# rug-marl-group2/scopa

Hardware: AMD Instinct MI355X
Metric: MiniScopa infoset-traversals/sec (higher is better)
Workload: dtype f64

## Files before the change

include/scopa.h:

```cpp
#ifndef SCOPA_H
#define SCOPA_H
#include <stddef.h>
#include <stdint.h>

#ifdef __cplusplus
extern "C" {
#endif

#define SCOPA_ABI_VERSION 1

enum {
    SCOPA_OK = 0,
    SCOPA_EINVAL = -1,
    SCOPA_ENODEV = -2,
    SCOPA_EHIP = -3,
    SCOPA_ESTATE = -4,
    SCOPA_ENOMEM = -5,
    SCOPA_ELIMIT = -6,
    SCOPA_ETIMEOUT = -7
};

#define SCOPA_N_CARDS 16
#define SCOPA_N_PLIES 8
#define SCOPA_N_DECISION 1653
#define SCOPA_N_TERMINAL 576
#define SCOPA_N_NODES 2229
#define SCOPA_MAX_ACTIONS 4

#define SCOPA_STEP_CLONED 0x80u
#define SCOPA_STEP_COUNT_MASK 0x7Fu
typedef struct scopa_state {
    uint16_t hand[2];
    uint32_t table;
    uint8_t  nh[2];
    uint8_t  nt;
    uint8_t  step;
    uint8_t  ncap[2];
    uint8_t  scopas[2];
} scopa_state;

typedef struct scopa_ctx scopa_ctx;

int32_t     scopa_abi_version(void);
const char *scopa_strerror(int32_t status);
const char *scopa_last_error(const scopa_ctx *ctx);

int32_t scopa_ctx_create(int32_t device_id, void *hip_stream, scopa_ctx **out);
int32_t scopa_ctx_destroy(scopa_ctx *ctx);
int32_t scopa_ctx_synchronize(scopa_ctx *ctx);

int32_t scopa_deal_py_seed(int64_t seed, uint8_t perm16[16]);
int32_t scopa_state_init(const uint8_t perm16[16], scopa_state *out);
int32_t scopa_state_step(scopa_state *s, int32_t action);
int32_t scopa_state_clone(const scopa_state *s, scopa_state *out);
int32_t scopa_state_is_terminal(const scopa_state *s);
int32_t scopa_state_current_player(const scopa_state *s);
int32_t scopa_state_legal(const scopa_state *s, int32_t player , int32_t out[4], int32_t *n);
int32_t scopa_state_rewards_x2(const scopa_state *s, int32_t r2[2]);
int32_t scopa_state_infoset_key(const scopa_state *s, int32_t player, uint64_t *key);
int32_t scopa_key_to_string(uint64_t key, char *buf, int32_t cap);
int32_t scopa_state_infoset_string(const scopa_state *s, int32_t player, char *buf, int32_t cap);

int32_t scopa_step_batch(scopa_ctx *ctx, scopa_state *d_states, const uint8_t *d_actions, int64_t n);
int32_t scopa_step_batch_host(scopa_ctx *ctx, scopa_state *h_states, const uint8_t *h_actions, int64_t n);

int32_t scopa_set_deal(scopa_ctx *ctx, const uint8_t perm16[16]);
int32_t scopa_tree_counts(scopa_ctx *ctx, int32_t *n_nodes, int32_t *n_decision, int32_t *n_infosets);
int32_t scopa_tree_export(scopa_ctx *ctx, scopa_state *h_states, int32_t *h_infoset, int8_t *h_r2,
                          uint64_t *h_infoset_key, int8_t *h_infoset_nlegal, int8_t *h_infoset_legal);

int32_t scopa_tables_reset(scopa_ctx *ctx);
int32_t scopa_tables_get(scopa_ctx *ctx, double *h_regret, double *h_strategy, double *h_local);
int32_t scopa_tables_set(scopa_ctx *ctx, const double *h_regret, const double *h_strategy, const double *h_local);

int32_t scopa_visited_get(scopa_ctx *ctx, uint32_t *h_seq);

int32_t scopa_cfr_exact_iterate(scopa_ctx *ctx, int32_t n_iters, double *h_root_values);
int32_t scopa_cfr_exact_traverse(scopa_ctx *ctx, int32_t traverser, double *h_value);
int32_t scopa_cfr_exact_mode(scopa_ctx *ctx, int32_t sequential);
int32_t scopa_cfr_exact_last_route(scopa_ctx *ctx, int32_t *route);
int32_t scopa_cfr_exact_traverse_from(scopa_ctx *ctx, int32_t traverser, int32_t depth, const int32_t *path,
                                      double reach_p0, double reach_p1, double *h_value);

int32_t scopa_cfr_sync_iterate(scopa_ctx *ctx, int32_t n_iters);
int32_t scopa_cfr_sync_iterate_weighted(scopa_ctx *ctx, int32_t n_iters, const double *h_w , int32_t alternating);

int32_t scopa_mccfr_replay(scopa_ctx *ctx, int32_t n_iters, const double *h_uniforms, int64_t n_uniforms,
                           int64_t *consumed);

int32_t scopa_mccfr_seed(scopa_ctx *ctx, uint64_t seed);
int32_t scopa_mccfr_iterate(scopa_ctx *ctx, uint32_t batch, uint32_t n_iters);
int32_t scopa_mccfr_traverse(scopa_ctx *ctx, uint32_t iteration, uint32_t b0, uint32_t nb);
int32_t scopa_mccfr_delta_buffer(scopa_ctx *ctx, void **d_delta, size_t *bytes);
int32_t scopa_mccfr_bind_delta(scopa_ctx *ctx, void *d_buf, size_t bytes);
int32_t scopa_mccfr_delta_get(scopa_ctx *ctx, double *h_delta);
int32_t scopa_mccfr_delta_set(scopa_ctx *ctx, const double *h_delta);
int32_t scopa_mccfr_apply(scopa_ctx *ctx);
int32_t scopa_mccfr_iteration_counter(scopa_ctx *ctx, uint32_t *iteration);
int32_t scopa_mccfr_graph_mode(scopa_ctx *ctx, int32_t on);
int32_t scopa_debug_lds_limit(scopa_ctx *ctx, int32_t bytes);

int32_t scopa_sdcfr_frontier_width(int32_t traverser, int32_t ply);
int32_t scopa_sdcfr_features(scopa_ctx *ctx, int32_t ply, int64_t n, const int32_t *d_idx, float *d_feats, float *d_mask);
int32_t scopa_sdcfr_expand(scopa_ctx *ctx, int32_t ply, int32_t traverser, int64_t n, const int32_t *d_idx, const float *d_adv,
                           int32_t *d_child_idx, float *d_pol, const double *d_uniforms, uint32_t iteration, uint32_t b0);
int32_t scopa_sdcfr_terminal_values(scopa_ctx *ctx, int32_t traverser, int64_t n, const int32_t *d_idx, float *d_val);
int32_t scopa_sdcfr_backward(scopa_ctx *ctx, int32_t ply, int32_t traverser, int64_t n, const int32_t *d_idx, const float *d_pol,
                             const float *d_child_val, float *d_val, const float *d_feats, const float *d_mask, float *d_mem_feat,
                             float *d_mem_regret, float *d_mem_mask, int64_t capacity, int64_t write_base);
int32_t scopa_sdcfr_visits(scopa_ctx *ctx, uint64_t *decision_visits);
int32_t scopa_sdcfr_policy_get(scopa_ctx *ctx, float *h_policy, uint64_t *h_thr);
#define SCOPA_SDCFR_IMAGE_FLOATS 13520
int32_t scopa_sdcfr_image_floats(void);
int32_t scopa_sdcfr_pack_weights(scopa_ctx *ctx, int32_t player, const float *d_w1, const float *d_b1, const float *d_w2,
                                 const float *d_b2, const float *d_w3, const float *d_b3, float *d_image);
int32_t scopa_sdcfr_traverse_fused(scopa_ctx *ctx, int32_t traverser, int32_t batch, const float *d_image, float *d_mem_feat,
                                   float *d_mem_regret, float *d_mem_mask, int64_t capacity, int64_t write_base,
                                   float *d_root_values, const double *d_uniforms, uint32_t iteration, uint32_t b0);
int32_t scopa_sdcfr_mode(scopa_ctx *ctx, int32_t forward_per_visit);
int32_t scopa_sdcfr_tuning(scopa_ctx *ctx, int32_t traversals_per_task, int32_t wavefronts_per_task);
int32_t scopa_sdcfr_train_params(void);
int32_t scopa_sdcfr_train_steps(scopa_ctx *ctx, const int64_t *d_rows, int32_t n_rows, int32_t n_steps, const float *d_feat, const float *d_regret, const float *d_mask,
                                int64_t capacity, float *d_w1, float *d_b1, float *d_w2, float *d_b2, float *d_w3, float *d_b3, float *d_state,
                                int32_t first_step, float lr, float *d_loss);
int32_t scopa_sdcfr_train_step(scopa_ctx *ctx, const int64_t *d_rows, int32_t n_rows, const float *d_feat, const float *d_regret, const float *d_mask,
                               int64_t capacity, float *d_w1, float *d_b1, float *d_w2, float *d_b2, float *d_w3, float *d_b3, float *d_state,
                               int32_t step, float lr, float *d_loss);
int32_t scopa_sdcfr_average_policy(scopa_ctx *ctx, int32_t player, int32_t n_snap, const float *d_w1, const float *d_b1, const float *d_w2,
                                   const float *d_b2, const float *d_w3, const float *d_b3, int32_t max_size, const int32_t *d_slots,
                                   const float *d_coef, double *d_policy);
int32_t scopa_features_from_states(scopa_ctx *ctx, const scopa_state *d_states, int64_t n, float *d_feats, float *d_mask);
int32_t scopa_eval_init_states(scopa_ctx *ctx, scopa_state *d_states, int64_t n);
int32_t scopa_eval_step(scopa_ctx *ctx, scopa_state *d_states, int64_t n, const float *d_probs, const int32_t *d_trained_seat,
                        uint32_t stream_id, uint32_t ply_tag);

int32_t scopa_eval_tabular_prepare(scopa_ctx *ctx, const double *d_policy);
int32_t scopa_eval_tabular_step(scopa_ctx *ctx, scopa_state *d_states, int32_t *d_node_idx, int64_t n, int32_t ply,
                                const double *d_policy, const int32_t *d_trained_seat, uint32_t stream_id);
int32_t scopa_eval_tabular_match(scopa_ctx *ctx, int64_t n, int64_t n_seat0, uint32_t stream_id, scopa_state *d_states_out, int32_t *d_node_idx_out,
                                 int64_t h_stats[10]);

int32_t scopa_exploitability(scopa_ctx *ctx, const double *h_policy, double *h_out4, double *h_policy_out);

int32_t scopa_cross_play(scopa_ctx *ctx, int32_t n_pol, const double *d_policies , double *d_out );
int32_t scopa_best_response(scopa_ctx *ctx, int32_t n_pol, const double *d_policies , double *d_br ,
                            double *d_out4 );
int32_t scopa_eval_pair_match(scopa_ctx *ctx, const double *d_policy_a, const double *d_policy_b, int64_t n, int64_t n_seat0, uint32_t stream_id,
                              int32_t *d_node_idx_out, int64_t h_stats[10]);

typedef struct scopa_multi scopa_multi;
int32_t scopa_multi_create(scopa_ctx *ctx, int32_t n_deals, scopa_multi **out);
int32_t scopa_multi_destroy(scopa_multi *m);
int32_t scopa_multi_deal_py_seeds(scopa_multi *m, const int64_t *h_seeds);
int32_t scopa_multi_set_perms(scopa_multi *m, const uint8_t *h_perms );
int32_t scopa_multi_perms_get(scopa_multi *m, uint8_t *h_perms);
int32_t scopa_multi_build(scopa_multi *m, int32_t *h_n_infosets);
int32_t scopa_multi_cfr_exact_iterate(scopa_multi *m, int32_t n_iters);
int32_t scopa_multi_cfr_exact_iterate_lanes(scopa_multi *m, int32_t n_iters);
int32_t scopa_multi_cfr_sync_iterate(scopa_multi *m, int32_t n_iters);
int32_t scopa_multi_cfr_sync_iterate_weighted(scopa_multi *m, int32_t n_iters, const double *h_w, int32_t alternating,
                                              const uint8_t *h_active );
int32_t scopa_multi_mccfr_iterate(scopa_multi *m, uint32_t batch, uint32_t n_iters, uint64_t seed);
int32_t scopa_multi_exploitability(scopa_multi *m, double *h_out4);
int32_t scopa_multi_tables_get(scopa_multi *m, int32_t deal, double *h_regret, double *h_strategy, double *h_local, uint64_t *h_keys);
int32_t scopa_multi_tables_set(scopa_multi *m, int32_t deal, const double *h_regret, const double *h_strategy, const double *h_local);
int32_t scopa_multi_counters(scopa_multi *m, uint64_t *decision_visits, uint64_t *terminal_visits);

typedef struct scopa_chance scopa_chance;
int32_t scopa_chance_create(scopa_multi *m, scopa_chance **out);
int32_t scopa_chance_destroy(scopa_chance *g);
int32_t scopa_chance_counts(scopa_chance *g, int32_t *n_deals, int64_t *n_global, int64_t *n_occurrences);
int32_t scopa_chance_index_get(scopa_chance *g, uint64_t *h_keys , int32_t *h_map );
int32_t scopa_chance_tables_reset(scopa_chance *g);
int32_t scopa_chance_tables_get(scopa_chance *g, double *h_regret, double *h_strategy);
int32_t scopa_chance_tables_set(scopa_chance *g, const double *h_regret, const double *h_strategy);
int32_t scopa_chance_cfr_iterate_weighted(scopa_chance *g, int32_t n_iters, const double *h_w , int32_t alternating);
int32_t scopa_chance_cfr_iterate_sampled(scopa_chance *g, int32_t n_iters, int32_t m, const int32_t *h_deals ,
                                         const double *h_w , int32_t alternating);
int32_t scopa_chance_mccfr_iterate(scopa_chance *g, int32_t n_iters, uint32_t batch, uint64_t seed,
                                   int32_t m, const int32_t *h_deals );
int32_t scopa_chance_mccfr_counters(scopa_chance *g, uint64_t *decision_visits, uint64_t *terminal_visits, uint32_t *iteration);
int32_t scopa_chance_exploitability(scopa_chance *g, const double *h_policy , double *h_out4, double *h_policy_out);
int32_t scopa_chance_policy_for_deal(scopa_chance *g, const double *d_policy_G, int32_t deal, double *d_policy_local );
int32_t scopa_chance_cross_play(scopa_chance *g, int32_t n_pol, const double *d_policies , double *d_per_deal ,
                                double *d_out );
int32_t scopa_chance_best_response(scopa_chance *g, int32_t n_pol, const double *d_policies , double *d_br ,
                                   double *d_out4 );
int32_t scopa_chance_debug_scratch_budget(scopa_chance *g, int64_t bytes);
int32_t scopa_chance_match(scopa_chance *g, const double *d_policy_a, const double *d_policy_b, int64_t n, int64_t n_seat0, uint32_t stream_id,
                           int32_t *d_deal_out , int32_t *d_node_idx_out , int64_t h_stats[10]);
int32_t scopa_chance_sdcfr_traverse(scopa_chance *g, int32_t traverser, int32_t batch, int32_t m, const int32_t *h_deals ,
                                    const float *d_image, float *d_mem_feat, float *d_mem_regret, float *d_mem_mask , int64_t capacity,
                                    int64_t write_base, float *d_root_values , uint32_t iteration, uint32_t b0);
int32_t scopa_chance_sdcfr_visits(scopa_chance *g, uint64_t *decision_visits);
int32_t scopa_chance_sdcfr_average_policy(scopa_chance *g, int32_t player, int32_t n_snap, const float *d_w1, const float *d_b1, const float *d_w2,
                                          const float *d_b2, const float *d_w3, const float *d_b3, int32_t max_size, const int32_t *d_slots,
                                          const float *d_coef, double *d_policy_G );

typedef struct scopa_full_state {
    uint64_t table[2];
    uint64_t cap[2];
    uint32_t hand[2];
    uint32_t game;
    uint8_t  nh[2], nt, deck_pos, round, last_capture , scopas[2];
    uint16_t step;
    uint8_t  terminal;
    int8_t   r2_p0;
    uint8_t  flags;
    uint8_t  pad[7];
} scopa_full_state;
int32_t scopa_full_deal_py_seed(int64_t seed, uint8_t perm40[40]);
int32_t scopa_full_state_init(const uint8_t deck40[40], uint32_t game, scopa_full_state *out);
int32_t scopa_full_state_step(scopa_full_state *s, const uint8_t deck40[40], int32_t action);
int32_t scopa_full_state_legal(const scopa_full_state *s, int32_t player, int32_t out[3], int32_t *n);
int32_t scopa_full_state_infoset_string(const scopa_full_state *s, int32_t player, char *buf, int32_t cap);
int32_t scopa_full_step_batch(scopa_ctx *ctx, scopa_full_state *d_states, const uint8_t *d_actions, const uint8_t *d_decks, int64_t n);
int32_t scopa_full_step_batch_host(scopa_ctx *ctx, scopa_full_state *h_states, const uint8_t *h_actions, const uint8_t *h_decks,
                                   int64_t n_decks, int64_t n);
int32_t scopa_full_random_playouts(scopa_ctx *ctx, const int64_t *h_seeds, int64_t n_games, int8_t *h_r2_p0, int16_t *h_plies);

typedef struct scopa_team_state {
    uint64_t history;
    uint32_t table;
    uint16_t hand[4];
    uint16_t cap[4];
    uint8_t  nh[4];
    uint8_t  scopas[4];
    uint8_t  nt, step, last_capture_team , flags ;
} scopa_team_state;
int32_t scopa_team_state_init(const uint8_t perm16[16], scopa_team_state *out);
int32_t scopa_team_state_step(scopa_team_state *s, int32_t action);
int32_t scopa_team_state_legal(const scopa_team_state *s, int32_t out[4], int32_t *n);
int32_t scopa_team_state_rewards_x2(const scopa_team_state *s, int32_t r2_seat[4]);
int32_t scopa_team_state_infoset_string(const scopa_team_state *s, int32_t team, char *buf, int32_t cap);
int32_t scopa_team_step_batch(scopa_ctx *ctx, scopa_team_state *d_states, const uint8_t *d_actions, int64_t n);
int32_t scopa_team_step_batch_host(scopa_ctx *ctx, scopa_team_state *h_states, const uint8_t *h_actions, int64_t n);
int32_t scopa_team_random_playouts(scopa_ctx *ctx, const int64_t *h_seeds, int64_t n_games, int8_t *h_r2_team0, uint8_t *h_scopas);

#define SCOPA_TEAM_N_CHOICE 321365
#define SCOPA_TEAM_N_LEAVES 331776
#define SCOPA_TEAM_N_INFOSETS 1648469
int32_t scopa_team_set_deal(scopa_ctx *ctx, const uint8_t perm16[16]);
int32_t scopa_team_tree_counts(scopa_ctx *ctx, int32_t *n_choice, int32_t *n_leaves, int32_t *n_infosets);
int32_t scopa_team_tree_leaves(scopa_ctx *ctx, int8_t *h_r2);
int32_t scopa_team_tables_reset(scopa_ctx *ctx);
int32_t scopa_team_tables_get(scopa_ctx *ctx, double *h_regret, double *h_strategy, double *h_local, double *h_leaf_reach_sum);
int32_t scopa_team_tables_set(scopa_ctx *ctx, const double *h_regret, const double *h_strategy, const double *h_local, const double *h_leaf_reach_sum);
int32_t scopa_team_cfr_iterate(scopa_ctx *ctx, int32_t n_iters, const double *h_w , double *h_root_values );
int32_t scopa_team_cfr_traverse(scopa_ctx *ctx, int32_t traverser, double *h_value);
int32_t scopa_team_cfr_launch(scopa_ctx *ctx, int32_t traverser, int32_t part);
int32_t scopa_team_exploitability(scopa_ctx *ctx, const double *d_policy , double *h_out4, double *d_br );
int32_t scopa_team_minimax(scopa_ctx *ctx, double *h_value, double *d_policy_out );
int32_t scopa_team_policy_value(scopa_ctx *ctx, const double *d_policy_a, const double *d_policy_b, double *h_out);
// ... 53 lines not shown
```

scopa_amd/_lib.py:

```python
import ctypes as C
import os

import numpy as np

_HERE = os.path.dirname(os.path.abspath(__file__))
LIB_PATH = os.environ.get("SCOPA_HIP_LIBRARY") or os.path.join(_HERE, "libscopa_hip.so")

SCOPA_OK, SCOPA_EINVAL, SCOPA_ENODEV, SCOPA_EHIP, SCOPA_ESTATE, SCOPA_ENOMEM, SCOPA_ELIMIT, SCOPA_ETIMEOUT = 0, -1, -2, -3, -4, -5, -6, -7
N_NODES, N_DECISION, N_TERMINAL = 2229, 1653, 576
TEAM_N_CHOICE, TEAM_N_LEAVES, TEAM_N_INFOSETS = 321365, 331776, 1648469
TEAM_MCCFR_DRAWS = (49381, 20583)

SYMBOLS = [
    "scopa_abi_version", "scopa_strerror", "scopa_last_error", "scopa_ctx_create", "scopa_ctx_destroy",
    "scopa_ctx_synchronize", "scopa_deal_py_seed", "scopa_state_init", "scopa_state_step", "scopa_state_clone", "scopa_state_is_terminal",
    "scopa_state_current_player", "scopa_state_legal", "scopa_state_rewards_x2", "scopa_state_infoset_key",
    "scopa_key_to_string", "scopa_state_infoset_string", "scopa_step_batch", "scopa_step_batch_host", "scopa_set_deal",
    "scopa_tree_counts", "scopa_tree_export", "scopa_tables_reset", "scopa_tables_get", "scopa_tables_set",
    "scopa_visited_get", "scopa_cfr_exact_iterate", "scopa_cfr_exact_traverse", "scopa_cfr_exact_mode", "scopa_cfr_exact_last_route", "scopa_cfr_exact_traverse_from", "scopa_mccfr_replay", "scopa_mccfr_seed",
    "scopa_mccfr_iterate", "scopa_mccfr_traverse", "scopa_mccfr_delta_buffer", "scopa_mccfr_bind_delta", "scopa_mccfr_delta_get", "scopa_mccfr_delta_set", "scopa_mccfr_apply",
    "scopa_mccfr_iteration_counter", "scopa_mccfr_graph_mode", "scopa_debug_lds_limit", "scopa_sdcfr_frontier_width", "scopa_sdcfr_features", "scopa_sdcfr_expand",
    "scopa_sdcfr_terminal_values", "scopa_sdcfr_backward", "scopa_sdcfr_visits", "scopa_sdcfr_policy_get", "scopa_sdcfr_traverse_fused", "scopa_sdcfr_image_floats", "scopa_sdcfr_pack_weights", "scopa_sdcfr_tuning", "scopa_sdcfr_mode", "scopa_sdcfr_train_params", "scopa_sdcfr_train_step", "scopa_sdcfr_train_steps", "scopa_sdcfr_average_policy", "scopa_features_from_states",
    "scopa_eval_init_states", "scopa_eval_step", "scopa_eval_tabular_step", "scopa_eval_tabular_prepare", "scopa_eval_tabular_match", "scopa_cfr_sync_iterate", "scopa_cfr_sync_iterate_weighted", "scopa_multi_create", "scopa_multi_destroy",
    "scopa_multi_deal_py_seeds", "scopa_multi_set_perms", "scopa_multi_perms_get", "scopa_multi_build", "scopa_multi_cfr_exact_iterate",
    "scopa_multi_cfr_exact_iterate_lanes", "scopa_multi_cfr_sync_iterate", "scopa_multi_cfr_sync_iterate_weighted", "scopa_multi_mccfr_iterate", "scopa_multi_exploitability", "scopa_multi_tables_get", "scopa_multi_tables_set", "scopa_multi_counters",
    "scopa_chance_create", "scopa_chance_destroy", "scopa_chance_counts", "scopa_chance_index_get", "scopa_chance_tables_reset", "scopa_chance_tables_get", "scopa_chance_tables_set",
    "scopa_chance_cfr_iterate_weighted", "scopa_chance_cfr_iterate_sampled", "scopa_chance_mccfr_iterate", "scopa_chance_mccfr_counters", "scopa_chance_exploitability", "scopa_chance_policy_for_deal",
    "scopa_chance_cross_play", "scopa_chance_best_response", "scopa_chance_debug_scratch_budget", "scopa_chance_match",
    "scopa_chance_sdcfr_traverse", "scopa_chance_sdcfr_visits", "scopa_chance_sdcfr_average_policy", "scopa_full_deal_py_seed",
    "scopa_full_state_init", "scopa_full_state_step", "scopa_full_state_legal", "scopa_full_state_infoset_string",
    "scopa_full_step_batch", "scopa_full_step_batch_host", "scopa_full_random_playouts",
    "scopa_team_state_init", "scopa_team_state_step", "scopa_team_state_legal", "scopa_team_state_rewards_x2", "scopa_team_state_infoset_string",
    "scopa_team_step_batch", "scopa_team_step_batch_host", "scopa_team_random_playouts",
    "scopa_team_set_deal", "scopa_team_tree_counts", "scopa_team_tree_leaves", "scopa_team_tables_reset", "scopa_team_tables_get", "scopa_team_tables_set",
    "scopa_team_cfr_iterate", "scopa_team_cfr_traverse", "scopa_team_cfr_launch", "scopa_team_exploitability", "scopa_team_minimax", "scopa_team_policy_value",
    "scopa_team_chance_create", "scopa_team_chance_destroy", "scopa_team_chance_debug_image_budget", "scopa_team_chance_counts", "scopa_team_chance_index_get",
    "scopa_team_chance_tables_reset", "scopa_team_chance_tables_get", "scopa_team_chance_tables_set", "scopa_team_chance_sigma_get", "scopa_team_chance_cfr_iterate", "scopa_team_chance_cfr_launch",
    "scopa_team_chance_exploitability", "scopa_team_chance_policy_for_deal",
    "scopa_team_chance_mccfr_traverse", "scopa_team_chance_mccfr_apply", "scopa_team_chance_mccfr_walk", "scopa_team_chance_mccfr_iterate", "scopa_team_chance_mccfr_counters", "scopa_team_chance_mccfr_delta_get",
    "scopa_team_mccfr_replay", "scopa_team_mccfr_traverse", "scopa_team_mccfr_apply", "scopa_team_mccfr_iterate", "scopa_team_mccfr_counters", "scopa_team_mccfr_delta_get", "scopa_team_mccfr_visits_get",
    "scopa_mccfr_iterate_sharded", "scopa_p2p_create", "scopa_p2p_connect", "scopa_p2p_allreduce_delta", "scopa_p2p_set_form", "scopa_p2p_set_budget", "scopa_p2p_status", "scopa_p2p_destroy", "scopa_exploitability", "scopa_cross_play", "scopa_best_response", "scopa_eval_pair_match", "scopa_counters", "scopa_prof_enable", "scopa_prof_read", "scopa_prof_device", "scopa_prof_phases", "scopa_prof_spread",
]


class ScopaError(RuntimeError):
    def __init__(self, status, where, detail=""):
        self.status = status
        msg = f"{where}: status {status}"
        try:
            msg += f" ({lib().scopa_strerror(status).decode()})"
        except Exception:
            pass
        if detail:
            msg += f": {detail}"
        super().__init__(msg)


class State16(C.Structure):
    _fields_ = [("hand", C.c_uint16 * 2), ("table", C.c_uint32), ("nh", C.c_uint8 * 2), ("nt", C.c_uint8),
                ("step", C.c_uint8), ("ncap", C.c_uint8 * 2), ("scopas", C.c_uint8 * 2)]


STEP_CLONED, STEP_COUNT_MASK = 0x80, 0x7F
STATE_DTYPE = np.dtype([("hand", "<u2", (2,)), ("table", "<u4"), ("nh", "u1", (2,)), ("nt", "u1"), ("step", "u1"),
                        ("ncap", "u1", (2,)), ("scopas", "u1", (2,))])
assert STATE_DTYPE.itemsize == 16 and C.sizeof(State16) == 16

_lib = None


def lib():
    global _lib
    if _lib is not None:
        return _lib
    try:
        import torch
    except ImportError:
        pass
    if not os.path.exists(LIB_PATH):
        raise OSError(f"{LIB_PATH} is missing: build it with `python __graft_entry__.py` or `python scopa_amd/build.py` "
                      "(the MiniScopa solver path has no fallback)")
    L = C.CDLL(LIB_PATH)
    vp, i32, i64, u32, u64 = C.c_void_p, C.c_int32, C.c_int64, C.c_uint32, C.c_uint64
    sig = {
        "scopa_abi_version": (i32, []),
        "scopa_strerror": (C.c_char_p, [i32]),
        "scopa_last_error": (C.c_char_p, [vp]),
        "scopa_ctx_create": (i32, [i32, vp, C.POINTER(vp)]),
        "scopa_ctx_destroy": (i32, [vp]),
        "scopa_ctx_synchronize": (i32, [vp]),
        "scopa_deal_py_seed": (i32, [i64, vp]),
        "scopa_state_init": (i32, [vp, C.POINTER(State16)]),
        "scopa_state_step": (i32, [C.POINTER(State16), i32]),
        "scopa_state_clone": (i32, [C.POINTER(State16), C.POINTER(State16)]),
        "scopa_state_is_terminal": (i32, [C.POINTER(State16)]),
        "scopa_state_current_player": (i32, [C.POINTER(State16)]),
        "scopa_state_legal": (i32, [C.POINTER(State16), i32, C.POINTER(i32 * 4), C.POINTER(i32)]),
        "scopa_state_rewards_x2": (i32, [C.POINTER(State16), C.POINTER(i32 * 2)]),
        "scopa_state_infoset_key": (i32, [C.POINTER(State16), i32, C.POINTER(u64)]),
        "scopa_key_to_string": (i32, [u64, C.c_char_p, i32]),
        "scopa_state_infoset_string": (i32, [C.POINTER(State16), i32, C.c_char_p, i32]),
        "scopa_step_batch": (i32, [vp, vp, vp, i64]),
        "scopa_step_batch_host": (i32, [vp, vp, vp, i64]),
        "scopa_set_deal": (i32, [vp, vp]),
        "scopa_tree_counts": (i32, [vp, C.POINTER(i32), C.POINTER(i32), C.POINTER(i32)]),
        "scopa_tree_export": (i32, [vp, vp, vp, vp, vp, vp, vp]),
        "scopa_tables_reset": (i32, [vp]),
        "scopa_tables_get": (i32, [vp, vp, vp, vp]),
        "scopa_tables_set": (i32, [vp, vp, vp, vp]),
        "scopa_cfr_exact_iterate": (i32, [vp, i32, vp]),
        "scopa_cfr_exact_traverse": (i32, [vp, i32, C.POINTER(C.c_double)]),
        "scopa_cfr_exact_mode": (i32, [vp, i32]),
        "scopa_cfr_exact_last_route": (i32, [vp, C.POINTER(i32)]),
        "scopa_cfr_exact_traverse_from": (i32, [vp, i32, i32, vp, C.c_double, C.c_double, C.POINTER(C.c_double)]),
        "scopa_visited_get": (i32, [vp, vp]),
        "scopa_mccfr_replay": (i32, [vp, i32, vp, i64, C.POINTER(i64)]),
        "scopa_mccfr_seed": (i32, [vp, u64]),
        "scopa_mccfr_iterate": (i32, [vp, u32, u32]),
        "scopa_mccfr_traverse": (i32, [vp, u32, u32, u32]),
        "scopa_mccfr_delta_buffer": (i32, [vp, C.POINTER(vp), C.POINTER(C.c_size_t)]),
        "scopa_mccfr_bind_delta": (i32, [vp, vp, C.c_size_t]),
        "scopa_mccfr_delta_get": (i32, [vp, vp]),
        "scopa_mccfr_delta_set": (i32, [vp, vp]),
        "scopa_mccfr_apply": (i32, [vp]),
        "scopa_mccfr_iteration_counter": (i32, [vp, C.POINTER(u32)]),
        "scopa_mccfr_graph_mode": (i32, [vp, i32]),
        "scopa_debug_lds_limit": (i32, [vp, i32]),
        "scopa_exploitability": (i32, [vp, vp, vp, vp]),
        "scopa_sdcfr_frontier_width": (i32, [i32, i32]),
        "scopa_sdcfr_features": (i32, [vp, i32, i64, vp, vp, vp]),
        "scopa_sdcfr_expand": (i32, [vp, i32, i32, i64, vp, vp, vp, vp, vp, u32, u32]),
        "scopa_sdcfr_terminal_values": (i32, [vp, i32, i64, vp, vp]),
        "scopa_sdcfr_backward": (i32, [vp, i32, i32, i64, vp, vp, vp, vp, vp, vp, vp, vp, vp, i64, i64]),
        "scopa_sdcfr_visits": (i32, [vp, C.POINTER(u64)]),
        "scopa_sdcfr_policy_get": (i32, [vp, vp, vp]),
        "scopa_sdcfr_traverse_fused": (i32, [vp, i32, i32, vp, vp, vp, vp, i64, i64, vp, vp, u32, u32]),
        "scopa_sdcfr_image_floats": (i32, []),
        "scopa_sdcfr_pack_weights": (i32, [vp, i32, vp, vp, vp, vp, vp, vp, vp]),
        "scopa_sdcfr_tuning": (i32, [vp, i32, i32]),
        "scopa_sdcfr_train_params": (i32, []),
        "scopa_sdcfr_train_step": (i32, [vp, vp, i32, vp, vp, vp, i64, vp, vp, vp, vp, vp, vp, vp, i32, C.c_float, vp]),
        "scopa_sdcfr_train_steps": (i32, [vp, vp, i32, i32, vp, vp, vp, i64, vp, vp, vp, vp, vp, vp, vp, i32, C.c_float, vp]),
        "scopa_sdcfr_mode": (i32, [vp, i32]),
        "scopa_sdcfr_average_policy": (i32, [vp, i32, i32, vp, vp, vp, vp, vp, vp, i32, vp, vp, vp]),
        "scopa_features_from_states": (i32, [vp, vp, i64, vp, vp]),
        "scopa_eval_init_states": (i32, [vp, vp, i64]),
        "scopa_eval_step": (i32, [vp, vp, i64, vp, vp, u32, u32]),
        "scopa_eval_tabular_step": (i32, [vp, vp, vp, i64, i32, vp, vp, u32]),
        "scopa_eval_tabular_prepare": (i32, [vp, vp]),
        "scopa_eval_tabular_match": (i32, [vp, i64, i64, u32, vp, vp, vp]),
        "scopa_cross_play": (i32, [vp, i32, vp, vp]),
        "scopa_best_response": (i32, [vp, i32, vp, vp, vp]),
        "scopa_eval_pair_match": (i32, [vp, vp, vp, i64, i64, u32, vp, vp]),
        "scopa_cfr_sync_iterate": (i32, [vp, i32]),
        "scopa_cfr_sync_iterate_weighted": (i32, [vp, i32, vp, i32]),
        "scopa_multi_create": (i32, [vp, i32, C.POINTER(vp)]),
        "scopa_multi_destroy": (i32, [vp]),
        "scopa_multi_deal_py_seeds": (i32, [vp, vp]),
        "scopa_multi_set_perms": (i32, [vp, vp]),
        "scopa_multi_perms_get": (i32, [vp, vp]),
        "scopa_multi_build": (i32, [vp, vp]),
        "scopa_multi_cfr_exact_iterate": (i32, [vp, i32]),
        "scopa_multi_cfr_sync_iterate": (i32, [vp, i32]),
        "scopa_multi_cfr_sync_iterate_weighted": (i32, [vp, i32, vp, i32, vp]),
        "scopa_multi_cfr_exact_iterate_lanes": (i32, [vp, i32]),
        "scopa_multi_exploitability": (i32, [vp, vp]),
        "scopa_multi_mccfr_iterate": (i32, [vp, u32, u32, u64]),
        "scopa_multi_tables_get": (i32, [vp, i32, vp, vp, vp, vp]),
        "scopa_multi_tables_set": (i32, [vp, i32, vp, vp, vp]),
        "scopa_multi_counters": (i32, [vp, C.POINTER(u64), C.POINTER(u64)]),
        "scopa_chance_create": (i32, [vp, C.POINTER(vp)]),
        "scopa_chance_destroy": (i32, [vp]),
        "scopa_chance_counts": (i32, [vp, C.POINTER(i32), C.POINTER(i64), C.POINTER(i64)]),
        "scopa_chance_index_get": (i32, [vp, vp, vp]),
        "scopa_chance_tables_reset": (i32, [vp]),
        "scopa_chance_tables_get": (i32, [vp, vp, vp]),
        "scopa_chance_tables_set": (i32, [vp, vp, vp]),
        "scopa_chance_cfr_iterate_weighted": (i32, [vp, i32, vp, i32]),
        "scopa_chance_cfr_iterate_sampled": (i32, [vp, i32, i32, vp, vp, i32]),
        "scopa_chance_mccfr_iterate": (i32, [vp, i32, u32, u64, i32, vp]),
        "scopa_chance_mccfr_counters": (i32, [vp, C.POINTER(u64), C.POINTER(u64), C.POINTER(u32)]),
        "scopa_chance_exploitability": (i32, [vp, vp, vp, vp]),
        "scopa_chance_policy_for_deal": (i32, [vp, vp, i32, vp]),
        "scopa_chance_cross_play": (i32, [vp, i32, vp, vp, vp]),
        "scopa_chance_best_response": (i32, [vp, i32, vp, vp, vp]),
        "scopa_chance_debug_scratch_budget": (i32, [vp, i64]),
        "scopa_chance_match": (i32, [vp, vp, vp, i64, i64, u32, vp, vp, vp]),
        "scopa_chance_sdcfr_traverse": (i32, [vp, i32, i32, i32, vp, vp, vp, vp, vp, i64, i64, vp, u32, u32]),
        "scopa_chance_sdcfr_visits": (i32, [vp, C.POINTER(u64)]),
        "scopa_chance_sdcfr_average_policy": (i32, [vp, i32, i32, vp, vp, vp, vp, vp, vp, i32, vp, vp, vp]),
        "scopa_full_deal_py_seed": (i32, [i64, vp]),
        "scopa_full_state_init": (i32, [vp, u32, vp]),
        "scopa_full_state_step": (i32, [vp, vp, i32]),
        "scopa_full_state_legal": (i32, [vp, i32, C.POINTER(i32 * 3), C.POINTER(i32)]),
        "scopa_full_state_infoset_string": (i32, [vp, i32, C.c_char_p, i32]),
        "scopa_full_step_batch": (i32, [vp, vp, vp, vp, i64]),
        "scopa_full_step_batch_host": (i32, [vp, vp, vp, vp, i64, i64]),
        "scopa_full_random_playouts": (i32, [vp, vp, i64, vp, vp]),
        "scopa_mccfr_iterate_sharded": (i32, [vp, u32, u32, u32]),
        "scopa_p2p_create": (i32, [vp, i32, i32, vp]),
        "scopa_p2p_connect": (i32, [vp, vp]),
        "scopa_p2p_allreduce_delta": (i32, [vp]),
        "scopa_p2p_set_form": (i32, [vp, i32]),
        "scopa_p2p_set_budget": (i32, [vp, C.c_double]),
        "scopa_p2p_status": (i32, [vp, C.POINTER(i32), C.POINTER(u64)]),
        "scopa_p2p_destroy": (i32, [vp]),
        "scopa_team_state_init": (i32, [vp, vp]),
        "scopa_team_state_step": (i32, [vp, i32]),
        "scopa_team_state_legal": (i32, [vp, C.POINTER(i32 * 4), C.POINTER(i32)]),
        "scopa_team_state_rewards_x2": (i32, [vp, C.POINTER(i32 * 4)]),
        "scopa_team_state_infoset_string": (i32, [vp, i32, C.c_char_p, i32]),
        "scopa_team_step_batch": (i32, [vp, vp, vp, i64]),
        "scopa_team_step_batch_host": (i32, [vp, vp, vp, i64]),
        "scopa_team_random_playouts": (i32, [vp, vp, i64, vp, vp]),
        "scopa_team_set_deal": (i32, [vp, vp]),
        "scopa_team_tree_counts": (i32, [vp, C.POINTER(i32), C.POINTER(i32), C.POINTER(i32)]),
        "scopa_team_tree_leaves": (i32, [vp, vp]),
        "scopa_team_tables_reset": (i32, [vp]),
        "scopa_team_tables_get": (i32, [vp, vp, vp, vp, vp]),
        "scopa_team_tables_set": (i32, [vp, vp, vp, vp, vp]),
        "scopa_team_cfr_iterate": (i32, [vp, i32, vp, vp]),
        "scopa_team_cfr_traverse": (i32, [vp, i32, C.POINTER(C.c_double)]),
        "scopa_team_cfr_launch": (i32, [vp, i32, i32]),
        "scopa_team_exploitability": (i32, [vp, vp, C.POINTER(C.c_double * 4), vp]),
        "scopa_team_minimax": (i32, [vp, C.POINTER(C.c_double), vp]),
        "scopa_team_policy_value": (i32, [vp, vp, vp, C.POINTER(C.c_double)]),
        "scopa_team_chance_create": (i32, [vp, i32, vp, C.POINTER(vp)]),
        "scopa_team_chance_destroy": (i32, [vp]),
        "scopa_team_chance_debug_image_budget": (i32, [vp, i64]),
        "scopa_team_chance_counts": (i32, [vp, C.POINTER(i32), C.POINTER(i64), C.POINTER(i64)]),
        "scopa_team_chance_index_get": (i32, [vp, vp, vp]),
        "scopa_team_chance_tables_reset": (i32, [vp]),
        "scopa_team_chance_tables_get": (i32, [vp, vp, vp]),
        "scopa_team_chance_tables_set": (i32, [vp, vp, vp]),
        "scopa_team_chance_sigma_get": (i32, [vp, vp]),
        "scopa_team_chance_cfr_iterate": (i32, [vp, i32, vp, vp]),
        "scopa_team_chance_cfr_launch": (i32, [vp, i32, i32]),
        "scopa_team_chance_exploitability": (i32, [vp, vp, C.POINTER(C.c_double * 4), vp, vp]),
        "scopa_team_chance_policy_for_deal": (i32, [vp, vp, i32, vp]),
        "scopa_team_chance_mccfr_traverse": (i32, [vp, C.c_uint32, i32, C.c_uint32, C.c_uint32]),
        "scopa_team_chance_mccfr_apply": (i32, [vp]),
        "scopa_team_chance_mccfr_walk": (i32, [vp, C.c_uint32, C.c_uint32, i32, vp]),
        "scopa_team_chance_mccfr_iterate": (i32, [vp, i32, C.c_uint32, i32, vp]),
        "scopa_team_chance_mccfr_counters": (i32, [vp, C.POINTER(C.c_uint64), C.POINTER(C.c_uint64), C.POINTER(C.c_uint32)]),
        "scopa_team_chance_mccfr_delta_get": (i32, [vp, vp]),
        "scopa_team_mccfr_replay": (i32, [vp, i32, vp, i64, C.POINTER(i64)]),
        "scopa_team_mccfr_traverse": (i32, [vp, C.c_uint32, C.c_uint32, C.c_uint32]),
        "scopa_team_mccfr_apply": (i32, [vp]),
        "scopa_team_mccfr_iterate": (i32, [vp, C.c_uint32, C.c_uint32]),
        "scopa_team_mccfr_counters": (i32, [vp, C.POINTER(C.c_uint64), C.POINTER(C.c_uint64), C.POINTER(C.c_uint32)]),
        "scopa_team_mccfr_delta_get": (i32, [vp, vp]),
        "scopa_team_mccfr_visits_get": (i32, [vp, vp, vp]),
        "scopa_counters": (i32, [vp, C.POINTER(u64), C.POINTER(u64)]),
        "scopa_prof_enable": (i32, [vp, i32]),
        "scopa_prof_read": (i32, [vp, C.POINTER(i64), C.POINTER(C.c_double)]),
        "scopa_prof_device": (i32, [vp, C.POINTER(i64), C.POINTER(C.c_double)]),
        "scopa_prof_phases": (i32, [vp, C.POINTER(C.c_double * 3)]),
        "scopa_prof_spread": (i32, [vp, C.POINTER(C.c_double * 3)]),
    }
    lenient = bool(os.environ.get("SCOPA_HIP_LIBRARY")) and os.environ.get("SCOPA_AB_OLD_LIBRARY") == "1"
    for name, (res, args) in sig.items():
        if lenient and not hasattr(L, name):
            continue
        fn = getattr(L, name)
        fn.restype, fn.argtypes = res, args
    if L.scopa_abi_version() != 1:
        raise OSError("libscopa_hip.so ABI version mismatch")
    _lib = L
    return L


def _ptr(a):
    return a.ctypes.data_as(C.c_void_p) if a is not None else None


def _weights(weights):
    w = np.ascontiguousarray(weights, np.float64).reshape(-1, 3)
    return (w if w.size else np.ones((1, 3))), w.shape[0]


# ... 20 lines not shown
        self._L = lib()
        rc = self._L.scopa_ctx_create(int(device), C.c_void_p(stream) if stream else None, C.byref(self._h))
        if rc:
            self._h = None
            raise ScopaError(rc, "scopa_ctx_create", "a GPU is required: the solver path has no CPU fallback")
        self.device = device
        self.stream = stream
        self.n_infosets = 0
        self._children = []

    def close(self):
        if getattr(self, "_h", None):
            for ref in getattr(self, "_children", []):
                child = ref()
                if child is not None:
                    child.close()
            self._L.scopa_ctx_destroy(self._h)
            self._h = None

    def __del__(self):
        try:
            self.close()
        except Exception:
            pass

    def _ck(self, rc, where):
        if rc:
            raise ScopaError(rc, where, self._L.scopa_last_error(self._h).decode())

    def synchronize(self):
        self._ck(self._L.scopa_ctx_synchronize(self._h), "scopa_ctx_synchronize")

    def step_batch_host(self, states, actions):
        assert states.dtype == STATE_DTYPE and states.flags.c_contiguous
        actions = np.ascontiguousarray(actions, np.uint8)
        assert actions.size == states.size
        self._ck(self._L.scopa_step_batch_host(self._h, _ptr(states), _ptr(actions), states.size), "scopa_step_batch_host")
        return states

    def step_batch(self, d_states_ptr, d_actions_ptr, n):
        self._ck(self._L.scopa_step_batch(self._h, C.c_void_p(d_states_ptr), C.c_void_p(d_actions_ptr), int(n)), "scopa_step_batch")

    def set_deal(self, perm16):
        perm = np.ascontiguousarray(perm16, np.uint8)
        assert perm.size == 16
        self._ck(self._L.scopa_set_deal(self._h, _ptr(perm)), "scopa_set_deal")
        a, b, c = C.c_int32(), C.c_int32(), C.c_int32()
        self._ck(self._L.scopa_tree_counts(self._h, C.byref(a), C.byref(b), C.byref(c)), "scopa_tree_counts")
        self.n_infosets = c.value
        self.perm = perm
        return self.n_infosets

    def tree_export(self):
        I = self.n_infosets
        out = dict(states=np.zeros(N_NODES, STATE_DTYPE), infoset=np.zeros(N_NODES, np.int32), r2=np.zeros((N_NODES, 2), np.int8),
                   infoset_key=np.zeros(I, np.uint64), infoset_nlegal=np.zeros(I, np.int8), infoset_legal=np.zeros((I, 4), np.int8))
        self._ck(self._L.scopa_tree_export(self._h, _ptr(out["states"]), _ptr(out["infoset"]), _ptr(out["r2"]),
                                           _ptr(out["infoset_key"]), _ptr(out["infoset_nlegal"]), _ptr(out["infoset_legal"])),
                 "scopa_tree_export")
        return out

    def tables_reset(self):
        self._ck(self._L.scopa_tables_reset(self._h), "scopa_tables_reset")

    def tables_get(self, regret=True, strategy=True, local=True):
        I = self.n_infosets
        R = np.zeros((I, 4)) if regret else None
        S = np.zeros((I, 4)) if strategy else None
        Lc = np.zeros((I, 4)) if local else None
        self._ck(self._L.scopa_tables_get(self._h, _ptr(R), _ptr(S), _ptr(Lc)), "scopa_tables_get")
        return R, S, Lc

    def tables_set(self, regret=None, strategy=None, local=None):
        arrs = []
        for a in (regret, strategy, local):
            if a is not None:
                a = np.ascontiguousarray(a, np.float64)
                assert a.shape == (self.n_infosets, 4)
            arrs.append(a)
        self._ck(self._L.scopa_tables_set(self._h, _ptr(arrs[0]), _ptr(arrs[1]), _ptr(arrs[2])), "scopa_tables_set")

    def cfr_exact_iterate(self, n_iters):
        rv = np.zeros((max(int(n_iters), 0), 2))
        self._ck(self._L.scopa_cfr_exact_iterate(self._h, int(n_iters), _ptr(rv)), "scopa_cfr_exact_iterate")
        return rv

    def cfr_exact_mode(self, sequential):
        self._ck(self._L.scopa_cfr_exact_mode(self._h, 1 if sequential else 0), "scopa_cfr_exact_mode")

    def cfr_exact_last_route(self):
        r = C.c_int32()
        self._ck(self._L.scopa_cfr_exact_last_route(self._h, C.byref(r)), "scopa_cfr_exact_last_route")
        return r.value

    def cfr_exact_traverse(self, traverser):
        v = C.c_double()
        self._ck(self._L.scopa_cfr_exact_traverse(self._h, int(traverser), C.byref(v)), "scopa_cfr_exact_traverse")
        return v.value

    def cfr_exact_traverse_from(self, traverser, path, reach_p0=1.0, reach_p1=1.0):
        pa = np.ascontiguousarray(path, np.int32)
        v = C.c_double()
        self._ck(self._L.scopa_cfr_exact_traverse_from(self._h, int(traverser), pa.size, _ptr(pa), float(reach_p0), float(reach_p1),
                                                       C.byref(v)), "scopa_cfr_exact_traverse_from")
        return v.value

    def visited_get(self):
        seq = np.zeros(self.n_infosets, np.uint32)
        self._ck(self._L.scopa_visited_get(self._h, _ptr(seq)), "scopa_visited_get")
        return seq

    def mccfr_replay(self, n_iters, uniforms):
        u = np.ascontiguousarray(uniforms, np.float64)
        used = C.c_int64()
        self._ck(self._L.scopa_mccfr_replay(self._h, int(n_iters), _ptr(u), u.size, C.byref(used)), "scopa_mccfr_replay")
        return used.value

    def mccfr_seed(self, seed):
        self._ck(self._L.scopa_mccfr_seed(self._h, int(seed)), "scopa_mccfr_seed")

    def mccfr_iterate(self, batch, n_iters):
        self._ck(self._L.scopa_mccfr_iterate(self._h, int(batch), int(n_iters)), "scopa_mccfr_iterate")

    def mccfr_traverse(self, iteration, b0, nb):
        self._ck(self._L.scopa_mccfr_traverse(self._h, int(iteration), int(b0), int(nb)), "scopa_mccfr_traverse")

    def mccfr_delta_buffer(self):
        p, n = C.c_void_p(), C.c_size_t()
        self._ck(self._L.scopa_mccfr_delta_buffer(self._h, C.byref(p), C.byref(n)), "scopa_mccfr_delta_buffer")
        return p.value, n.value

    def mccfr_bind_delta(self, d_ptr, nbytes):
        self._ck(self._L.scopa_mccfr_bind_delta(self._h, C.c_void_p(d_ptr) if d_ptr else None, int(nbytes)), "scopa_mccfr_bind_delta")

    def mccfr_delta_get(self):
        d = np.zeros((self.n_infosets, 5))
        self._ck(self._L.scopa_mccfr_delta_get(self._h, _ptr(d)), "scopa_mccfr_delta_get")
        return d

    def mccfr_delta_set(self, d):
        d = np.ascontiguousarray(d, np.float64)
        assert d.shape == (self.n_infosets, 5)
        self._ck(self._L.scopa_mccfr_delta_set(self._h, _ptr(d)), "scopa_mccfr_delta_set")

    def mccfr_apply(self):
        self._ck(self._L.scopa_mccfr_apply(self._h), "scopa_mccfr_apply")

    def mccfr_graph_mode(self, on):
        self._ck(self._L.scopa_mccfr_graph_mode(self._h, 1 if on else 0), "scopa_mccfr_graph_mode")

    def debug_lds_limit(self, nbytes):
        self._ck(self._L.scopa_debug_lds_limit(self._h, int(nbytes)), "scopa_debug_lds_limit")

    def mccfr_iteration(self):
        v = C.c_uint32()
        self._ck(self._L.scopa_mccfr_iteration_counter(self._h, C.byref(v)), "scopa_mccfr_iteration_counter")
        return v.value

    def exploitability(self, policy=None, return_policy=False):
        pin = None if policy is None else np.ascontiguousarray(policy, np.float64)
        out = np.zeros(4)
        pout = np.zeros((self.n_infosets, 4)) if return_policy else None
        self._ck(self._L.scopa_exploitability(self._h, _ptr(pin), _ptr(out), _ptr(pout)), "scopa_exploitability")
        res = dict(exploitability=out[0], br0=out[1], br1=out[2], value_p0=out[3])
        if return_policy:
            res["policy"] = pout
        return res

    def sdcfr_features(self, ply, n, idx_ptr, feats_ptr, mask_ptr):
        self._ck(self._L.scopa_sdcfr_features(self._h, ply, n, C.c_void_p(idx_ptr), C.c_void_p(feats_ptr), C.c_void_p(mask_ptr)), "scopa_sdcfr_features")

    def sdcfr_expand(self, ply, traverser, n, idx_ptr, adv_ptr, child_ptr, pol_ptr, uniforms_ptr, iteration, b0):
        self._ck(self._L.scopa_sdcfr_expand(self._h, ply, traverser, n, C.c_void_p(idx_ptr), C.c_void_p(adv_ptr), C.c_void_p(child_ptr),
                                            C.c_void_p(pol_ptr), C.c_void_p(uniforms_ptr) if uniforms_ptr else None, iteration, b0), "scopa_sdcfr_expand")

    def sdcfr_terminal_values(self, traverser, n, idx_ptr, val_ptr):
        self._ck(self._L.scopa_sdcfr_terminal_values(self._h, traverser, n, C.c_void_p(idx_ptr), C.c_void_p(val_ptr)), "scopa_sdcfr_terminal_values")

    def sdcfr_backward(self, ply, traverser, n, idx_ptr, pol_ptr, child_val_ptr, val_ptr, feats_ptr, mask_ptr, mem_feat_ptr, mem_regret_ptr,
                       mem_mask_ptr, capacity, write_base):
        vp = lambda x: C.c_void_p(x) if x else None
        self._ck(self._L.scopa_sdcfr_backward(self._h, ply, traverser, n, vp(idx_ptr), vp(pol_ptr), vp(child_val_ptr), vp(val_ptr), vp(feats_ptr),
                                              vp(mask_ptr), vp(mem_feat_ptr), vp(mem_regret_ptr), vp(mem_mask_ptr), capacity, write_base),
                 "scopa_sdcfr_backward")

    def sdcfr_pack_weights(self, player, w1_ptr, b1_ptr, w2_ptr, b2_ptr, w3_ptr, b3_ptr, image_ptr):
        self._ck(self._L.scopa_sdcfr_pack_weights(self._h, player, *(C.c_void_p(x) for x in (w1_ptr, b1_ptr, w2_ptr, b2_ptr, w3_ptr, b3_ptr, image_ptr))),
                 "scopa_sdcfr_pack_weights")

    def sdcfr_mode(self, forward_per_visit):
        self._ck(self._L.scopa_sdcfr_mode(self._h, 1 if forward_per_visit else 0), "scopa_sdcfr_mode")

    def sdcfr_tuning(self, traversals_per_task=0, wavefronts_per_task=0):
        self._ck(self._L.scopa_sdcfr_tuning(self._h, traversals_per_task, wavefronts_per_task), "scopa_sdcfr_tuning")

    def sdcfr_train_steps(self, rows_ptr, n_rows, n_steps, feat_ptr, regret_ptr, mask_ptr, capacity, param_ptrs, state_ptr, first_step, lr, loss_ptr):
        self._ck(self._L.scopa_sdcfr_train_steps(self._h, C.c_void_p(rows_ptr), int(n_rows), int(n_steps), C.c_void_p(feat_ptr), C.c_void_p(regret_ptr), C.c_void_p(mask_ptr),
                                                 int(capacity), *(C.c_void_p(p) for p in param_ptrs), C.c_void_p(state_ptr), int(first_step), float(lr),
                                                 C.c_void_p(loss_ptr)), "scopa_sdcfr_train_steps")

    def sdcfr_train_step(self, rows_ptr, n_rows, feat_ptr, regret_ptr, mask_ptr, capacity, param_ptrs, state_ptr, step, lr, loss_ptr):
        self._ck(self._L.scopa_sdcfr_train_step(self._h, C.c_void_p(rows_ptr), int(n_rows), C.c_void_p(feat_ptr), C.c_void_p(regret_ptr), C.c_void_p(mask_ptr),
                                                int(capacity), *(C.c_void_p(p) for p in param_ptrs), C.c_void_p(state_ptr), int(step), float(lr),
                                                C.c_void_p(loss_ptr)), "scopa_sdcfr_train_step")

    def sdcfr_traverse_fused(self, traverser, batch, weights_ptr, mem_feat_ptr, mem_regret_ptr, mem_mask_ptr, capacity, write_base,
                             root_values_ptr, uniforms_ptr, iteration, b0):
        self._ck(self._L.scopa_sdcfr_traverse_fused(self._h, traverser, batch, C.c_void_p(weights_ptr), C.c_void_p(mem_feat_ptr),
                                                    C.c_void_p(mem_regret_ptr), C.c_void_p(mem_mask_ptr), capacity, write_base,
                                                    C.c_void_p(root_values_ptr), C.c_void_p(uniforms_ptr) if uniforms_ptr else None,
                                                    iteration, b0), "scopa_sdcfr_traverse_fused")

    def sdcfr_average_policy(self, player, n_snap, param_ptrs, max_size, slots_ptr, coef_ptr, policy_ptr):
        vp = lambda x: C.c_void_p(x) if x else None
        self._ck(self._L.scopa_sdcfr_average_policy(self._h, int(player), int(n_snap), *(vp(p) for p in param_ptrs), int(max_size), vp(slots_ptr),
                                                    vp(coef_ptr), vp(policy_ptr)), "scopa_sdcfr_average_policy")

    def sdcfr_visits(self):
        v = C.c_uint64()
        self._ck(self._L.scopa_sdcfr_visits(self._h, C.byref(v)), "scopa_sdcfr_visits")
        return v.value

    def sdcfr_policy_get(self):
        pol, thr = np.zeros((N_DECISION, 4), np.float32), np.zeros((N_DECISION, 3), np.uint64)
        self._ck(self._L.scopa_sdcfr_policy_get(self._h, _ptr(pol), _ptr(thr)), "scopa_sdcfr_policy_get")
        return pol, thr

    def features_from_states(self, states_ptr, n, feats_ptr, mask_ptr):
        self._ck(self._L.scopa_features_from_states(self._h, C.c_void_p(states_ptr), n, C.c_void_p(feats_ptr), C.c_void_p(mask_ptr)), "scopa_features_from_states")

    def eval_init_states(self, states_ptr, n):
        self._ck(self._L.scopa_eval_init_states(self._h, C.c_void_p(states_ptr), n), "scopa_eval_init_states")

    def eval_step(self, states_ptr, n, probs_ptr, seat_ptr, stream_id, ply_tag):
        self._ck(self._L.scopa_eval_step(self._h, C.c_void_p(states_ptr), n, C.c_void_p(probs_ptr) if probs_ptr else None, C.c_void_p(seat_ptr),
                                         stream_id, ply_tag), "scopa_eval_step")

    def eval_tabular_prepare(self, policy_ptr):
        self._ck(self._L.scopa_eval_tabular_prepare(self._h, C.c_void_p(policy_ptr)), "scopa_eval_tabular_prepare")

    def eval_tabular_step(self, states_ptr, idx_ptr, n, ply, policy_ptr, seat_ptr, stream_id):
        self._ck(self._L.scopa_eval_tabular_step(self._h, C.c_void_p(states_ptr), C.c_void_p(idx_ptr), n, ply, C.c_void_p(policy_ptr) if policy_ptr else None,
                                                 C.c_void_p(seat_ptr), stream_id), "scopa_eval_tabular_step")

    def eval_tabular_match(self, n, n_seat0, stream_id, states_ptr=0, idx_ptr=0):
        st = np.zeros((2, 5), np.int64)
        self._ck(self._L.scopa_eval_tabular_match(self._h, int(n), int(n_seat0), stream_id, C.c_void_p(states_ptr) if states_ptr else None,
                                                  C.c_void_p(idx_ptr) if idx_ptr else None, _ptr(st)), "scopa_eval_tabular_match")
        return st

    def cross_play(self, n_pol, policies_ptr, out_ptr):
        self._ck(self._L.scopa_cross_play(self._h, int(n_pol), C.c_void_p(policies_ptr) if policies_ptr else None, C.c_void_p(out_ptr) if out_ptr else None),
                 "scopa_cross_play")

    def best_response(self, n_pol, policies_ptr, br_ptr, out4_ptr):
        self._ck(self._L.scopa_best_response(self._h, int(n_pol), C.c_void_p(policies_ptr) if policies_ptr else None, C.c_void_p(br_ptr) if br_ptr else None,
                                             C.c_void_p(out4_ptr) if out4_ptr else None), "scopa_best_response")

    def eval_pair_match(self, policy_a_ptr, policy_b_ptr, n, n_seat0, stream_id, idx_ptr=0):
        st = np.zeros((2, 5), np.int64)
        self._ck(self._L.scopa_eval_pair_match(self._h, C.c_void_p(policy_a_ptr) if policy_a_ptr else None, C.c_void_p(policy_b_ptr) if policy_b_ptr else None,
                                               int(n), int(n_seat0), stream_id, C.c_void_p(idx_ptr) if idx_ptr else None, _ptr(st)), "scopa_eval_pair_match")
        return st

    def cfr_sync_iterate(self, n_iters):
        self._ck(self._L.scopa_cfr_sync_iterate(self._h, int(n_iters)), "scopa_cfr_sync_iterate")

    def cfr_sync_iterate_weighted(self, weights, alternating=False):
        w, n = _weights(weights)
        self._ck(self._L.scopa_cfr_sync_iterate_weighted(self._h, n, _ptr(w), int(alternating)), "scopa_cfr_sync_iterate_weighted")

    def full_step_batch_host(self, states, actions, decks):
        assert states.dtype == FULL_STATE_DTYPE
        actions = np.ascontiguousarray(actions, np.uint8)
        decks = np.ascontiguousarray(decks, np.uint8).reshape(-1, 40)
        self._ck(self._L.scopa_full_step_batch_host(self._h, _ptr(states), _ptr(actions), _ptr(decks), decks.shape[0], states.size),
                 "scopa_full_step_batch_host")
        return states

    def full_step_batch(self, states_ptr, actions_ptr, decks_ptr, n):
        self._ck(self._L.scopa_full_step_batch(self._h, C.c_void_p(states_ptr), C.c_void_p(actions_ptr), C.c_void_p(decks_ptr), int(n)), "scopa_full_step_batch")

    def full_random_playouts(self, seeds):
        seeds = np.ascontiguousarray(seeds, np.int64)
        r2, plies = np.zeros(seeds.size, np.int8), np.zeros(seeds.size, np.int16)
        self._ck(self._L.scopa_full_random_playouts(self._h, _ptr(seeds), seeds.size, _ptr(r2), _ptr(plies)), "scopa_full_random_playouts")
        return r2, plies

    def p2p_create(self, rank, world):
        h = np.zeros(64, np.uint8)
        self._ck(self._L.scopa_p2p_create(self._h, int(rank), int(world), _ptr(h)), "scopa_p2p_create")
        return h

    def p2p_connect(self, handles):
        handles = np.ascontiguousarray(handles, np.uint8).reshape(-1, 64)
        self._ck(self._L.scopa_p2p_connect(self._h, _ptr(handles)), "scopa_p2p_connect")

    def p2p_allreduce_delta(self):
        self._ck(self._L.scopa_p2p_allreduce_delta(self._h), "scopa_p2p_allreduce_delta")

    def mccfr_iterate_sharded(self, b0, nb, n_iters=1):
        self._ck(self._L.scopa_mccfr_iterate_sharded(self._h, int(b0), int(nb), int(n_iters)), "scopa_mccfr_iterate_sharded")

    def p2p_status(self):
        t, n = C.c_int32(), C.c_uint64()
        self._ck(self._L.scopa_p2p_status(self._h, C.byref(t), C.byref(n)), "scopa_p2p_status")
# ... 664 lines not shown
```

scopa_amd/csrc/scopa_ctx.h:

```cpp
#pragma once
#include <hip/hip_runtime.h>
#include <stdint.h>
#include <stdio.h>

#include <vector>

#include "../../include/scopa.h"
#include "scopa_rules.h"

struct scopa_p2p;
struct scopa_team_solver;

struct scopa_ctx {
    int device = -1;
    hipStream_t stream = nullptr;
    bool own_stream = false;
    char err[512] = {0};

    bool has_deal = false;
    uint8_t perm[16] = {0};
    int n_infosets = 0;

    scopa_state *d_states = nullptr;
    uint16_t *d_infoset = nullptr;
    int8_t *d_payoff = nullptr;
    uint64_t *d_key = nullptr;
    int32_t *d_meta = nullptr;
    uint32_t *d_visit = nullptr;

    double *d_regret = nullptr, *d_strat = nullptr, *d_local = nullptr;
    double *d_delta = nullptr;
    double *d_delta_own = nullptr;
    double *d_scratch = nullptr;
    double *d_sigcdf = nullptr;
    bool sigcdf_valid = false;
    bool mccfr_all_seen = false;
    uint32_t mccfr_seen_wait = 0;
    double *d_groups = nullptr;
    unsigned long long *d_clock = nullptr;
    uint16_t clock_grid[2048] = {0};
    double prof_phase_us[3] = {0.0, 0.0, 0.0};
    double prof_spread_us[3] = {0.0, 0.0, 0.0};
    size_t scratch_bytes = 0;

    unsigned long long *d_counters = nullptr;

    uint64_t seed = 0x5C09A;
    uint64_t sdcfr_visits = 0;
    void *d_sdnode = nullptr;
    bool sdnode_valid = false;
    void *d_eval_thr = nullptr;
    bool eval_thr_valid = false;
    void *d_pair_thr = nullptr;
    void *d_train_partial = nullptr;
    void *d_sdpol = nullptr;
    bool sdpol_valid = false;
    void *d_sdavg = nullptr;
    size_t sdavg_bytes = 0;
    int sdcfr_mode = 0;
    uint32_t iteration = 0;

    bool prof_on = false;
    int prof_stride = 1;
    long long prof_tick = 0;
    std::vector<hipEvent_t> ev_pool;
    size_t ev_used = 0;
    int64_t prof_launches = 0;
    double prof_ms = 0.0;

    uint32_t *d_lane_tab = nullptr;
    uint16_t *d_sched = nullptr;
    int sched_steps = 0;
    bool sched_valid = false;
    int exact_last_route = -1;
    bool exact_sequential = false;

    scopa_p2p *p2p = nullptr;
    scopa_team_solver *team = nullptr;

    struct GraphEntry { uint32_t batch, k, track; void *exec; };
    std::vector<GraphEntry> mccfr_graphs;
    bool mccfr_graph_mode = false;

    int lds_limit = 160 * 1024;
    int n_cus = 256;
    uint32_t lds_attr_done = 0;
    long long team_chance_budget = 0;
};

namespace scopa {

#ifndef SCOPA_GROUPS
#define SCOPA_GROUPS 16
#endif
#ifndef SCOPA_GROUP_PERM
#define SCOPA_GROUP_PERM 0
#endif
constexpr int kDeltaGroups = SCOPA_GROUPS;
constexpr int kGroupRows = 1664;
constexpr size_t kDeltaTable = (size_t)kGroupRows * 5;
__host__ __device__ inline size_t group_cell(int k, int r) {
#if SCOPA_GROUP_PERM == 1
    return (size_t)k * kGroupRows + (size_t)((r & 63) * 26 + (r >> 6));
#elif SCOPA_GROUP_PERM == 2
    return (size_t)k * kGroupRows + (size_t)((r & 7) * 208 + (r >> 3));
#else
    return (size_t)k * kGroupRows + (size_t)r;
#endif
}
constexpr int kClockSamples = 2048, kClockStride = 2048;

inline int32_t fail(scopa_ctx *ctx, int32_t code, const char *what, hipError_t e = hipSuccess) {
    if (ctx) {
        if (e != hipSuccess) snprintf(ctx->err, sizeof ctx->err, "%s: %s", what, hipGetErrorString(e));
        else snprintf(ctx->err, sizeof ctx->err, "%s", what);
    }
    return code;
}

#define SC_HIP(ctx, call)                                                         \
    do {                                                                          \
        hipError_t e__ = (call);                                                  \
        if (e__ != hipSuccess) return scopa::fail((ctx), SCOPA_EHIP, #call, e__); \
    } while (0)

#define SC_REQUIRE(ctx, cond, code, msg)                        \
    do {                                                        \
        if (!(cond)) return scopa::fail((ctx), (code), (msg)); \
    } while (0)

int32_t ensure_scratch(scopa_ctx *ctx, size_t bytes);

void range_push(const char *name);
void range_pop();
struct Range { explicit Range(const char *n) { range_push(n); } ~Range() { range_pop(); } };

enum LdsAttrKernel : uint32_t { kLdsTraverse = 1u, kLdsReplay = 8u, kLdsCfrExact = 16u, kLdsCfrSched = 512u, kLdsExploit = 32u, kLdsCfrSync = 64u, kLdsSdcfr = 128u, kLdsMulti = 256u, kLdsSdcfrReplay = 1024u, kLdsSdPolicy = 2048u, kLdsSdWalk0 = 4096u, kLdsSdWalk1 = 8192u, kLdsCfrSyncW = 16384u, kLdsCrossPlay = 32768u, kLdsBestResponse = 65536u, kLdsMccfrChance = 131072u, kLdsChanceSdWalk0 = 262144u, kLdsChanceSdWalk1 = 524288u, kLdsChanceCrossPlay = 1048576u, kLdsTeamCfr = 2097152u, kLdsTeamChance = 4194304u };
inline bool cfr_weights_ok(const double *h_w, int32_t n_iters) {
    for (size_t k = 0; k < (size_t)n_iters * 3; k++) if (!(h_w[k] >= 0.0 && h_w[k] <= 1.0)) return false;
    return true;
}
inline int32_t ensure_lds_attr(scopa_ctx *ctx, uint32_t kernel_bit, const void *fn, int bytes) {
    if (ctx->lds_attr_done & kernel_bit) return SCOPA_OK;
    SC_HIP(ctx, hipFuncSetAttribute(fn, hipFuncAttributeMaxDynamicSharedMemorySize, bytes));
    ctx->lds_attr_done |= kernel_bit;
    return SCOPA_OK;
}
#define SC_LDS_ATTR(ctx, bit, kernel, bytes)                                                                     \
    do {                                                                                                         \
        const int32_t rc__ = scopa::ensure_lds_attr((ctx), (bit), reinterpret_cast<const void *>(kernel), (bytes)); \
        if (rc__ != SCOPA_OK) return rc__;                                                                       \
    } while (0)
bool prof_events(scopa_ctx *ctx, hipEvent_t *start, hipEvent_t *stop);
void p2p_release(scopa_ctx *ctx);
void team_release(scopa_ctx *ctx);
void mccfr_graphs_clear(scopa_ctx *ctx);

}
```

scopa_amd/csrc/scopa_host.hip:

```cpp
#include <string.h>

#include <new>

#include "scopa_ctx.h"

using namespace scopa;

namespace scopa {

int32_t ensure_scratch(scopa_ctx *ctx, size_t bytes) {
    if (bytes <= ctx->scratch_bytes) return SCOPA_OK;
    if (ctx->d_scratch) SC_HIP(ctx, hipFree(ctx->d_scratch));
    ctx->d_scratch = nullptr;
    ctx->scratch_bytes = 0;
    SC_HIP(ctx, hipMalloc(&ctx->d_scratch, bytes));
    ctx->scratch_bytes = bytes;
    return SCOPA_OK;
}

static void prof_pool_fill(scopa_ctx *ctx) {
    while (ctx->ev_pool.size() < 4096) {
        hipEvent_t e;
        if (hipEventCreate(&e) != hipSuccess) break;
        ctx->ev_pool.push_back(e);
    }
}

bool prof_events(scopa_ctx *ctx, hipEvent_t *start, hipEvent_t *stop) {
    if (!ctx->prof_on) return false;
    if ((ctx->prof_tick++ % ctx->prof_stride) != 0) return false;
    if (ctx->ev_used + 2 > ctx->ev_pool.size()) {
        if (ctx->ev_used) {
            (void)hipEventSynchronize(ctx->ev_pool[ctx->ev_used - 1]);
            for (size_t i = 0; i + 1 < ctx->ev_used; i += 2) {
                float ms = 0.f;
                if (hipEventElapsedTime(&ms, ctx->ev_pool[i], ctx->ev_pool[i + 1]) == hipSuccess) ctx->prof_ms += ms;
            }
            ctx->ev_used = 0;
        }
        if (ctx->ev_pool.empty()) prof_pool_fill(ctx);
    }
    if (ctx->ev_used + 2 > ctx->ev_pool.size()) return false;
    *start = ctx->ev_pool[ctx->ev_used];
    *stop = ctx->ev_pool[ctx->ev_used + 1];
    ctx->ev_used += 2;
    ctx->prof_launches++;
    return true;
}

}

#include <dlfcn.h>
namespace scopa {
namespace {
int (*g_roctx_push)(const char *) = nullptr;
int (*g_roctx_pop)() = nullptr;
int g_roctx_state = 0;
void roctx_resolve() {
    g_roctx_state = -1;
    const char *on = getenv("SCOPA_ROCTX");
    if (!on || on[0] != '1') return;
    for (const char *lib : {"librocprofiler-sdk-roctx.so", "libroctx64.so"}) {
        void *h = dlopen(lib, RTLD_NOW | RTLD_GLOBAL);
        if (!h) continue;
        g_roctx_push = reinterpret_cast<int (*)(const char *)>(dlsym(h, "roctxRangePushA"));
        g_roctx_pop = reinterpret_cast<int (*)()>(dlsym(h, "roctxRangePop"));
        if (g_roctx_push && g_roctx_pop) { g_roctx_state = 1; return; }
    }
}
}
void range_push(const char *name) {
    if (g_roctx_state == 0) roctx_resolve();
    if (g_roctx_state == 1) (void)g_roctx_push(name);
}
void range_pop() {
    if (g_roctx_state == 1) (void)g_roctx_pop();
}
}

extern "C" {

int32_t scopa_abi_version(void) { return SCOPA_ABI_VERSION; }

const char *scopa_strerror(int32_t status) {
    switch (status) {
        case SCOPA_OK: return "ok";
        case SCOPA_EINVAL: return "invalid argument";
        case SCOPA_ENODEV: return "no usable HIP device (the solver path has no CPU fallback)";
        case SCOPA_EHIP: return "HIP runtime error";
        case SCOPA_ESTATE: return "call order violated";
        case SCOPA_ENOMEM: return "out of memory";
        case SCOPA_ELIMIT: return "problem exceeds a compiled-in capacity";
        case SCOPA_ETIMEOUT: return "a peer did not answer within the wait budget";
        default: return "unknown status";
    }
}

const char *scopa_last_error(const scopa_ctx *ctx) { return ctx ? ctx->err : "null context"; }

int32_t scopa_ctx_create(int32_t device_id, void *hip_stream, scopa_ctx **out) {
    if (!out || device_id < 0) return SCOPA_EINVAL;
    *out = nullptr;
    int count = 0;
    if (hipGetDeviceCount(&count) != hipSuccess || count <= 0) return SCOPA_ENODEV;
    if (device_id >= count) return SCOPA_ENODEV;
    scopa_ctx *ctx = new (std::nothrow) scopa_ctx();
    if (!ctx) return SCOPA_ENOMEM;
    ctx->device = device_id;
    hipError_t e = hipSetDevice(device_id);
    if (e != hipSuccess) { delete ctx; return SCOPA_ENODEV; }
    hipDeviceProp_t prop;
    if (hipGetDeviceProperties(&prop, device_id) == hipSuccess) {
        ctx->n_cus = prop.multiProcessorCount;
        ctx->lds_limit = (int)prop.sharedMemPerBlock;
    }
    if (hip_stream) ctx->stream = (hipStream_t)hip_stream;
    else {
        e = hipStreamCreateWithFlags(&ctx->stream, hipStreamNonBlocking);
        if (e != hipSuccess) { delete ctx; return SCOPA_EHIP; }
        ctx->own_stream = true;
    }
    const size_t rows = (size_t)kDecision;
    bool ok = hipMalloc(&ctx->d_states, sizeof(scopa_state) * kNodes) == hipSuccess &&
              hipMalloc(&ctx->d_infoset, sizeof(uint16_t) * kDecision) == hipSuccess &&
              hipMalloc(&ctx->d_payoff, kTerminal) == hipSuccess &&
              hipMalloc(&ctx->d_key, sizeof(uint64_t) * kDecision) == hipSuccess &&
              hipMalloc(&ctx->d_meta, sizeof(int32_t) * 8) == hipSuccess &&
              hipMalloc(&ctx->d_visit, sizeof(uint32_t) * kDecision) == hipSuccess &&
              hipMalloc(&ctx->d_sigcdf, (size_t)kDecision * 6 * sizeof(double)) == hipSuccess &&
              hipMalloc(&ctx->d_groups, scopa::kDeltaGroups * scopa::kDeltaTable * sizeof(double)) == hipSuccess &&
              hipMalloc(&ctx->d_regret, rows * 4 * sizeof(double)) == hipSuccess &&
              hipMalloc(&ctx->d_strat, rows * 4 * sizeof(double)) == hipSuccess &&
              hipMalloc(&ctx->d_local, rows * 4 * sizeof(double)) == hipSuccess &&
              hipMalloc(&ctx->d_delta_own, rows * 5 * sizeof(double)) == hipSuccess &&
              hipMalloc(&ctx->d_counters, (8 + 2 * 1024) * sizeof(unsigned long long)) == hipSuccess;
    ctx->d_delta = ctx->d_delta_own;
    if (ok) ok = hipMemsetAsync(ctx->d_counters, 0, (8 + 2 * 1024) * sizeof(unsigned long long), ctx->stream) == hipSuccess &&
                 hipMemsetAsync(ctx->d_delta, 0, rows * 5 * sizeof(double), ctx->stream) == hipSuccess &&
                 hipMemsetAsync(ctx->d_groups, 0, scopa::kDeltaGroups * scopa::kDeltaTable * sizeof(double), ctx->stream) == hipSuccess;
    if (!ok) { scopa_ctx_destroy(ctx); return SCOPA_ENOMEM; }
    *out = ctx;
    return SCOPA_OK;
}

int32_t scopa_ctx_destroy(scopa_ctx *ctx) {
    if (!ctx) return SCOPA_EINVAL;
    (void)hipSetDevice(ctx->device);
    (void)hipStreamSynchronize(ctx->stream);
    scopa::p2p_release(ctx);
    scopa::team_release(ctx);
    scopa::mccfr_graphs_clear(ctx);
    for (hipEvent_t e : ctx->ev_pool) (void)hipEventDestroy(e);
    void *bufs[] = {ctx->d_states, ctx->d_infoset, ctx->d_payoff, ctx->d_key, ctx->d_meta, ctx->d_regret, ctx->d_strat,
                    ctx->d_local, ctx->d_delta_own, ctx->d_scratch, ctx->d_counters, ctx->d_visit, ctx->d_sigcdf, ctx->d_groups, ctx->d_clock, ctx->d_sched, ctx->d_lane_tab, ctx->d_sdnode, ctx->d_sdpol, ctx->d_train_partial, ctx->d_eval_thr, ctx->d_pair_thr, ctx->d_sdavg};
    for (void *b : bufs) if (b) (void)hipFree(b);
    if (ctx->own_stream) (void)hipStreamDestroy(ctx->stream);
    delete ctx;
    return SCOPA_OK;
}

int32_t scopa_debug_lds_limit(scopa_ctx *ctx, int32_t bytes) {
    if (!ctx || bytes < 0) return SCOPA_EINVAL;
    hipDeviceProp_t prop;
    SC_HIP(ctx, hipGetDeviceProperties(&prop, ctx->device));
    SC_REQUIRE(ctx, bytes == 0 || (bytes >= 64 * 1024 && (size_t)bytes <= prop.sharedMemPerBlock), SCOPA_EINVAL, "scopa_debug_lds_limit: 0 or 64 KB .. the device's limit");
    ctx->lds_limit = bytes ? bytes : (int)prop.sharedMemPerBlock;
    ctx->lds_attr_done = 0;
    scopa::mccfr_graphs_clear(ctx);
    return SCOPA_OK;
}

int32_t scopa_ctx_synchronize(scopa_ctx *ctx) {
    if (!ctx) return SCOPA_EINVAL;
    SC_HIP(ctx, hipStreamSynchronize(ctx->stream));
    return SCOPA_OK;
}

namespace {
struct Mt19937 {
    uint32_t mt[624];
    int at = 624;
    void seed_u32(uint32_t s) {
        mt[0] = s;
        for (int i = 1; i < 624; i++) mt[i] = 1812433253u * (mt[i - 1] ^ (mt[i - 1] >> 30)) + (uint32_t)i;
        at = 624;
    }
    void seed_array(const uint32_t *key, int n) {
        seed_u32(19650218u);
        int i = 1, j = 0;
        for (int k = n > 624 ? n : 624; k > 0; k--) {
            mt[i] = (mt[i] ^ ((mt[i - 1] ^ (mt[i - 1] >> 30)) * 1664525u)) + key[j] + (uint32_t)j;
            if (++i >= 624) { mt[0] = mt[623]; i = 1; }
            if (++j >= n) j = 0;
        }
        for (int k = 623; k > 0; k--) {
            mt[i] = (mt[i] ^ ((mt[i - 1] ^ (mt[i - 1] >> 30)) * 1566083941u)) - (uint32_t)i;
            if (++i >= 624) { mt[0] = mt[623]; i = 1; }
        }
        mt[0] = 0x80000000u;
    }
    void refill() {
        for (int k = 0; k < 624; k++) {
            const uint32_t y = (mt[k] & 0x80000000u) | (mt[(k + 1) % 624] & 0x7fffffffu);
            mt[k] = mt[(k + 397) % 624] ^ (y >> 1) ^ ((y & 1u) ? 0x9908b0dfu : 0u);
        }
        at = 0;
    }
    uint32_t next() {
        if (at >= 624) refill();
        uint32_t y = mt[at++];
        y ^= y >> 11;
        y ^= (y << 7) & 0x9d2c5680u;
        y ^= (y << 15) & 0xefc60000u;
        y ^= y >> 18;
        return y;
    }
    uint32_t below(uint32_t n) {
        int bits = 32 - __builtin_clz(n);
        uint32_t r;
        do r = next() >> (32 - bits); while (r >= n);
        return r;
    }
};
}

int32_t scopa_deal_py_seed(int64_t seed, uint8_t perm16[16]) {
    if (!perm16) return SCOPA_EINVAL;
    const uint64_t a = seed < 0 ? (uint64_t)0 - (uint64_t)seed : (uint64_t)seed;
    const uint32_t key[2] = {(uint32_t)a, (uint32_t)(a >> 32)};
    Mt19937 g;
    g.seed_array(key, key[1] ? 2 : 1);
    for (int i = 0; i < 16; i++) perm16[i] = (uint8_t)i;
    for (uint32_t i = 15; i >= 1; i--) {
        const uint32_t j = g.below(i + 1);
        const uint8_t t = perm16[i]; perm16[i] = perm16[j]; perm16[j] = t;
    }
    return SCOPA_OK;
}

static bool perm_ok(const uint8_t *p) {
    uint32_t seen = 0;
    for (int i = 0; i < 16; i++) { if (p[i] > 15) return false; seen |= 1u << p[i]; }
    return seen == 0xFFFFu;
}

int32_t scopa_state_init(const uint8_t perm16[16], scopa_state *out) {
    if (!perm16 || !out || !perm_ok(perm16)) return SCOPA_EINVAL;
    state_init(*out, perm16);
    return SCOPA_OK;
}

int32_t scopa_state_step(scopa_state *s, int32_t action) {
    if (!s || action < 0 || action > 15) return SCOPA_EINVAL;
    step(*s, action);
    return SCOPA_OK;
}

int32_t scopa_state_clone(const scopa_state *s, scopa_state *out) {
    if (!s || !out) return SCOPA_EINVAL;
    scopa_state c = *s;
    if (!is_terminal(c)) c.step = (uint8_t)(c.step | SCOPA_STEP_CLONED);
    *out = c;
    return SCOPA_OK;
}

int32_t scopa_state_is_terminal(const scopa_state *s) { return s ? (is_terminal(*s) ? 1 : 0) : SCOPA_EINVAL; }

int32_t scopa_state_current_player(const scopa_state *s) { return s ? current_player(*s) : SCOPA_EINVAL; }

int32_t scopa_state_legal(const scopa_state *s, int32_t player, int32_t out[4], int32_t *n) {
    if (!s || !out || !n || player > 1) return SCOPA_EINVAL;
    int tmp[4];
    *n = legal(*s, player, tmp);
    for (int i = 0; i < *n; i++) out[i] = tmp[i];
    return SCOPA_OK;
}

int32_t scopa_state_rewards_x2(const scopa_state *s, int32_t r2[2]) {
    if (!s || !r2) return SCOPA_EINVAL;
    int a, b;
    rewards_x2(*s, a, b);
    r2[0] = a; r2[1] = b;
    return SCOPA_OK;
}

int32_t scopa_state_infoset_key(const scopa_state *s, int32_t player, uint64_t *key) {
    if (!s || !key || player > 1) return SCOPA_EINVAL;
    if (player < 0) player = s->step & 1;
    *key = infoset_key(*s, player);
    return SCOPA_OK;
}

int32_t scopa_key_to_string(uint64_t key, char *buf, int32_t cap) {
    if (!buf || cap < 64) return SCOPA_EINVAL;
    static const char suit[4] = {'c', 'f', 'p', 'b'};
    const int player = (int)(key & 1), nh = (int)((key >> 1) & 7), nt = (int)((key >> 20) & 15);
    const uint32_t hand = (uint32_t)((key >> 4) & 0xFFFF), table = (uint32_t)(key >> 24);
    char *w = buf;
    w += sprintf(w, "P%d:H[", player);
    for (int i = 0; i < nh; i++) w += sprintf(w, "%s%d%c", i ? "-" : "", card_rank(nib(hand, i)), suit[nib(hand, i) >> 2]);
    w += sprintf(w, "]_T[");
    for (int i = 0; i < nt; i++) w += sprintf(w, "%s%d%c", i ? "-" : "", card_rank(nib(table, i)), suit[nib(table, i) >> 2]);
    w += sprintf(w, "]");
    return (int32_t)(w - buf);
}

int32_t scopa_state_infoset_string(const scopa_state *s, int32_t player, char *buf, int32_t cap) {
    if (!s || !buf || cap < 64 || player > 1) return SCOPA_EINVAL;
    if (player < 0) player = current_player(*s);
    if (is_terminal(*s) || player < 0) return (int32_t)sprintf(buf, "TERMINAL");
    return scopa_key_to_string(infoset_key(*s, player), buf, cap);
}

int32_t scopa_tables_get(scopa_ctx *ctx, double *h_regret, double *h_strategy, double *h_local) {
    if (!ctx) return SCOPA_EINVAL;
    SC_REQUIRE(ctx, ctx->has_deal, SCOPA_ESTATE, "scopa_tables_get: no deal set");
    const size_t bytes = (size_t)ctx->n_infosets * 4 * sizeof(double);
    if (h_regret) SC_HIP(ctx, hipMemcpyAsync(h_regret, ctx->d_regret, bytes, hipMemcpyDeviceToHost, ctx->stream));
    if (h_strategy) SC_HIP(ctx, hipMemcpyAsync(h_strategy, ctx->d_strat, bytes, hipMemcpyDeviceToHost, ctx->stream));
    if (h_local) SC_HIP(ctx, hipMemcpyAsync(h_local, ctx->d_local, bytes, hipMemcpyDeviceToHost, ctx->stream));
    SC_HIP(ctx, hipStreamSynchronize(ctx->stream));
// ... 140 lines not shown
```

scopa_amd/csrc/scopa_mccfr.hip:

```cpp
#include <hip/hip_ext.h>

#include "scopa_ctx.h"
#include "scopa_mccfr_sigma.h"
#include "scopa_p2p.h"
#include "scopa_philox.h"

using namespace scopa;

namespace {


__device__ __forceinline__ void choice_cdf(const double *sigma, int n, uint32_t *thr) {
    double cdf[4];
    double c = sigma[0];
    cdf[0] = c;
#pragma unroll
    for (int i = 1; i < 4; i++) { if (i < n) c += sigma[i]; cdf[i] = c; }
    const double last = c;
#pragma unroll
    for (int i = 0; i < 4; i++) thr[i] = i < n ? (uint32_t)ceil((cdf[i] / last) * 2147483648.0) : 0xFFFFFFFFu;
}
__device__ __forceinline__ void row_store(double *__restrict__ row, const double *sg, const uint32_t *thr) {
    double2 *out = reinterpret_cast<double2 *>(row);
    out[0] = make_double2(sg[0], sg[1]);
    out[1] = make_double2(sg[2], sg[3]);
    out[2] = make_double2(__longlong_as_double((long long)(((unsigned long long)thr[1] << 32) | thr[0])),
                          __longlong_as_double((long long)(((unsigned long long)thr[3] << 32) | thr[2])));
}
__device__ __forceinline__ void choice_cdf_f64(const double *sigma, int n, double *cdf) {
    double c = sigma[0];
    cdf[0] = c;
    for (int i = 1; i < n; i++) { c += sigma[i]; cdf[i] = c; }
    const double last = cdf[n - 1];
    for (int i = 0; i < 4; i++) cdf[i] = i < n ? cdf[i] / last : 2.0;
}

__host__ __device__ constexpr int ntl_at(int trav, int d) { return trav == 0 ? (d + 1) >> 1 : d >> 1; }
__host__ __device__ constexpr int task_nodes(int trav, int d) {
    return ntl_at(trav, d) == 0 ? 1 : ntl_at(trav, d) == 1 ? 5 : ntl_at(trav, d) == 2 ? 20 : 60;
}

constexpr int kRow = 6;
constexpr int kUpd = 26;
constexpr unsigned int kPairDecisionVisits = (1 + 5 + 5 + 20 + 20 + 60 + 60 + 120) + (1 + 1 + 5 + 5 + 20 + 20 + 60 + 60), kPairTerminalVisits = 120 + 120;
static_assert(kPairDecisionVisits == 463, "291 + 172");

}

__global__ void __launch_bounds__(256)
k_mccfr_prepare(const uint64_t *__restrict__ g_key, const double *__restrict__ g_regret, double *__restrict__ g_sigcdf, int n_infosets) {
    const int r = blockIdx.x * blockDim.x + threadIdx.x;
    if (r >= n_infosets) return;
    const int n = (int)((g_key[r] >> 1) & 7);
    double R[4], sg[4];
    uint32_t thr[4];
    for (int c = 0; c < 4; c++) R[c] = g_regret[r * 4 + c];
    mc_sigma(R, n, sg);
    choice_cdf(sg, n, thr);
    row_store(g_sigcdf + r * kRow, sg, thr);
}

constexpr int kIdentSlot = 166;
struct WaveScratch {
    uint32_t npk[168];
    int8_t p6[128];
    uint32_t kdraw[64][4];
};
static_assert(sizeof(WaveScratch) % 16 == 0, "WaveScratch must keep 16-byte alignment");

__device__ __forceinline__ void wave_lds_sync() {
    __builtin_amdgcn_fence(__ATOMIC_RELEASE, "wavefront");
    __builtin_amdgcn_s_waitcnt(0xc07f);
    __builtin_amdgcn_wave_barrier();
    __builtin_amdgcn_fence(__ATOMIC_ACQUIRE, "wavefront");
}

__device__ __forceinline__ uint32_t lds_addr(const void *p) { return (uint32_t)(uintptr_t)(__attribute__((address_space(3))) const void *)p; }
__device__ __forceinline__ uint32_t lds_read_u32(uint32_t a) { return *(__attribute__((address_space(3))) const uint32_t *)(uintptr_t)a; }
__device__ __forceinline__ int lds_read_i8(uint32_t a) { return *(__attribute__((address_space(3))) const int8_t *)(uintptr_t)a; }
__device__ __forceinline__ double lds_read_f64(uint32_t a) { return *(__attribute__((address_space(3))) const double *)(uintptr_t)a; }
typedef uint32_t u32x4 __attribute__((ext_vector_type(4)));
__device__ __forceinline__ uint4 lds_read_u4(uint32_t a) {
    const u32x4 v = *(__attribute__((address_space(3))) const u32x4 *)(uintptr_t)a;
    return make_uint4(v.x, v.y, v.z, v.w);
}
__device__ __forceinline__ void lds_write_u4(uint32_t a, uint32_t x, uint32_t y, uint32_t z, uint32_t w) {
    *(__attribute__((address_space(3))) u32x4 *)(uintptr_t)a = u32x4{x, y, z, w};
}

constexpr int kLaneSlotVecs = 15;
constexpr int kStaticLds = 64 + kLaneSlotVecs * 1024;
constexpr int kStaticLdsMulti = kStaticLds;

template <int NP>
__device__ __forceinline__ void draw_pairs(uint32_t wsb, int lane, const uint32_t (&b)[NP], uint32_t iteration, uint32_t seed_lo, uint32_t seed_hi) {
    const int trav = lane < 44 ? 0 : 1, p = trav ? lane - 44 : lane;
    philox_out x[NP];
#pragma unroll
    for (int i = 0; i < NP; i++) x[i] = philox4x32_10((uint32_t)p, b[i], iteration, (uint32_t)trav, seed_lo, seed_hi);
#pragma unroll
    for (int i = 0; i < NP; i++)
        lds_write_u4(wsb + (uint32_t)(i * sizeof(WaveScratch) + offsetof(WaveScratch, kdraw)) + 16u * (uint32_t)lane, x[i].x0 >> 1, x[i].x1 >> 1, x[i].x2 >> 1, x[i].x3 >> 1);
    wave_lds_sync();
}

struct NodeRegs {
    uint32_t pk;
};

__host__ __device__ constexpr int npk_offset(int d) { return d == 0 ? 0 : d == 1 ? 2 : d == 2 ? 8 : d == 3 ? 18 : d == 4 ? 43 : 86; }
__host__ __device__ constexpr int npk_slot(int trav, int d, int j) { return npk_offset(d) + (trav ? task_nodes(0, d) : 0) + j; }
static_assert(npk_offset(1) == task_nodes(0, 0) + task_nodes(1, 0) && npk_offset(2) == npk_offset(1) + task_nodes(0, 1) + task_nodes(1, 1) &&
              npk_offset(3) == npk_offset(2) + task_nodes(0, 2) + task_nodes(1, 2) && npk_offset(4) == npk_offset(3) + task_nodes(0, 3) + task_nodes(1, 3) &&
              npk_offset(4) + task_nodes(0, 4) + task_nodes(1, 4) <= npk_offset(5) && npk_offset(5) + task_nodes(0, 5) + task_nodes(1, 5) == kIdentSlot,
              "record slots of plies 0..5 tile WaveScratch::npk");

constexpr int kLvLeaf = 7, kLvUpd = 9;
struct LaneTabRow { uint4 v[kLaneSlotVecs]; };

template <int D, int ROUND>
__device__ __forceinline__ void lane_slot_build(LaneTabRow &row, int lane) {
    constexpr int S = D + ROUND;
    constexpr int c0 = task_nodes(0, D), c1 = task_nodes(1, D);
    const int t = lane + 64 * ROUND;
    const bool valid = t < c0 + c1;
    const int trav = t < c0 ? 0 : 1;
    const int j = valid ? (trav ? t - c0 : t) : 0;
    const bool is_trav = (D & 1) == trav;
    const int ntl = trav == 0 ? (D + 1) >> 1 : D >> 1;
    uint32_t plane4 = 0u, amask = valid ? ~0u : 0u, aforce = 0u;
    if constexpr (D > 0) {
        constexpr int pd = D > 0 ? D - 1 : 0, pn = 4 - (pd >> 1);
        const bool p_trav = (pd & 1) == trav;
        int pj = j, br = 0;
        if (p_trav) { pj = j / (pn + 1); br = j - pj * (pn + 1); }
        if (valid) plane4 = 4u * (uint32_t)((trav ? task_nodes(0, pd) : 0) + pj);
        if (valid && p_trav && br > 0) { amask = 0u; aforce = (uint32_t)(br - 1); }
    }
    const int blk = (ntl == 0 ? 0 : ntl == 1 ? 1 : ntl == 2 ? 4 : 14) + (j >> 1);
    const uint32_t kword = valid ? (uint32_t)(offsetof(WaveScratch, kdraw) + 16 * ((trav ? 44 : 0) + blk) + 4 * ((j & 1) * 2 + (is_trav ? 1 : 0)))
                                 : (uint32_t)offsetof(WaveScratch, kdraw);
    row.v[S] = make_uint4(plane4, amask, aforce, kword);
}

__device__ __forceinline__ void upd_build(LaneTabRow &row, int x) {
    const uint32_t ident = (uint32_t)(offsetof(WaveScratch, npk) + 4 * kIdentSlot);
    uint32_t rec[5] = {ident, ident, ident, ident, ident}, am[5] = {24u, 24u, 24u, 24u, 24u}, af[5] = {0u, 0u, 0u, 0u, 0u};
    uint32_t own = ident, nX = 1u, p6o[4] = {(uint32_t)offsetof(WaveScratch, p6), (uint32_t)offsetof(WaveScratch, p6), (uint32_t)offsetof(WaveScratch, p6), (uint32_t)offsetof(WaveScratch, p6)};
    if (x < 2 * kUpd) {
        const int trav = x < kUpd ? 0 : 1, xx = trav ? x - kUpd : x;
        const int m = xx == 0 ? 0 : xx < 6 ? 1 : 2;
        int j = xx - (m == 0 ? 0 : m == 1 ? 1 : 6);
        const int d = 2 * m + trav;
        nX = (uint32_t)(4 - m);
        const int stride = m == 0 ? 12 : m == 1 ? 3 : 1;
        const int base = m == 0 ? 0 : m == 1 ? j * 12 : j * 3;
        for (int c = 0; c < 4; c++) p6o[c] = (uint32_t)(offsetof(WaveScratch, p6) + trav * 60 + base + ((c < (int)nX ? c : (int)nX - 1) + 1) * stride);
        own = (uint32_t)(offsetof(WaveScratch, npk) + 4 * npk_slot(trav, d, j));
        for (int c = d; c > 0; c--) {
            const int pd = c - 1, pn = 4 - (pd >> 1);
            int forced = 0;
            if ((pd & 1) == trav) { const int pj = j / (pn + 1), br = j - pj * (pn + 1); forced = br; j = pj; }
            rec[pd] = (uint32_t)(offsetof(WaveScratch, npk) + 4 * npk_slot(trav, pd, j));
            if (forced) { am[pd] = 0u; af[pd] = 8u * (uint32_t)(forced - 1); }
        }
    }
    row.v[kLvUpd + 0] = make_uint4(rec[0], rec[1], rec[2], rec[3]);
    row.v[kLvUpd + 1] = make_uint4(rec[4], own, nX, 0u);
    row.v[kLvUpd + 2] = make_uint4(p6o[0], p6o[1], p6o[2], p6o[3]);
    row.v[kLvUpd + 3] = make_uint4(am[0], am[1], am[2], am[3]);
    row.v[kLvUpd + 4] = make_uint4(am[4], af[0], af[1], af[2]);
    row.v[kLvUpd + 5] = make_uint4(af[3], af[4], 0u, 0u);
}

struct WalkEnv {
    uint32_t wsb;
    uint32_t tab;
    const uint16_t *s_inf;
    const int8_t *s_pay;
    const double *s_sigcdf;
    double *s_dR;
    uint8_t *s_seen;
    unsigned int *s_cnt;
};

template <int D, int NP>
__device__ __forceinline__ void ply_step(const WalkEnv &e, int lane, NodeRegs (&st)[NP]) {
    constexpr int n = 4 - (D >> 1);
    constexpr int c0 = task_nodes(0, D), c1 = task_nodes(1, D);
    constexpr int NR = c0 + c1 > 64 ? 2 : 1;
    struct Pre {
        int idx, In;
        uint32_t k, thr0, thr1, thr2;
    };
    Pre g[NP][NR];
    uint4 sl[NR];
#pragma unroll
    for (int r = 0; r < NR; r++) sl[r] = lds_read_u4(e.tab + 1024u * (uint32_t)(D + r));
#pragma unroll
    for (int i = 0; i < NP; i++)
#pragma unroll
        for (int r = 0; r < NR; r++) {
            Pre &q = g[i][r];
            q.idx = 0;
            if constexpr (D > 0) {
                constexpr int pn = 4 - ((D > 0 ? D - 1 : 0) >> 1);
                const uint32_t ppk = (uint32_t)__builtin_amdgcn_ds_bpermute((int)sl[r].x, (int)st[i].pk);
                const uint32_t act = ((ppk >> 21) & sl[r].y) | sl[r].z;
                q.idx = (int)((ppk & 1023u) * pn + act);
            }
            q.In = e.s_inf[level_offset(D) + q.idx];
            q.k = lds_read_u32(e.wsb + sl[r].w + (uint32_t)(i * sizeof(WaveScratch)));
            const uint32_t *thr = reinterpret_cast<const uint32_t *>(e.s_sigcdf + q.In * kRow + 4);
            q.thr0 = thr[0];
            q.thr1 = n > 2 ? thr[1] : 0xFFFFFFFFu;
            q.thr2 = n > 3 ? thr[2] : 0xFFFFFFFFu;
        }
#pragma unroll
    for (int i = 0; i < NP; i++)
#pragma unroll
        for (int r = 0; r < NR; r++) {
            const Pre &q = g[i][r];
            const int t = 64 * r + lane;
            if (t < c0 + c1) {
                const int a = (q.thr0 <= q.k) + (q.thr1 <= q.k) + (q.thr2 <= q.k);
                if ((D & 1) == (t < c0 ? 0 : 1)) atomicAdd(&e.s_cnt[q.In], 1u);
                else if (e.s_seen) e.s_seen[q.In] = 1;
                const uint32_t pk = (uint32_t)q.idx | ((uint32_t)q.In << 10) | ((uint32_t)a << 21);
                *(__attribute__((address_space(3))) uint32_t *)(uintptr_t)(e.wsb + (uint32_t)(i * sizeof(WaveScratch) + offsetof(WaveScratch, npk) + 4 * npk_offset(D)) + 4u * (uint32_t)t) = pk;
                if constexpr (D < 5) st[i].pk = pk;
            }
        }
    if constexpr (D == 5) wave_lds_sync();
}

#ifdef SCOPA_WALK_STAMPS
__device__ unsigned long long g_walk_stamps[16];
__device__ unsigned long long g_wave_clocks[3 * 16];
__device__ unsigned long long g_wave_phases[4 * 16];
#define WALK_STAMP(i) do { const unsigned long long now_ = clock64(); if (blockIdx.x == 0 && threadIdx.x == 0) { g_walk_stamps[i] += now_ - t_prev_; } t_prev_ = now_; } while (0)
#else
#define WALK_STAMP(i) do { } while (0)
#endif

template <int NP>
__device__ __forceinline__ void walk_pairs(const WalkEnv &e, int lane, const uint32_t (&b)[NP], uint32_t iteration, uint32_t seed_lo,
                                           uint32_t seed_hi, unsigned int &my_pairs) {
#ifdef SCOPA_WALK_STAMPS
    const unsigned long long w_start_ = wall_clock64();
    unsigned long long t_prev_ = clock64();
#endif
    draw_pairs<NP>(e.wsb, lane, b, iteration, seed_lo, seed_hi);
    WALK_STAMP(0);
    NodeRegs st[NP];
#pragma unroll
    for (int i = 0; i < NP; i++) st[i].pk = 0u;
    ply_step<0, NP>(e, lane, st); WALK_STAMP(1);
    ply_step<1, NP>(e, lane, st); WALK_STAMP(2);
    ply_step<2, NP>(e, lane, st); WALK_STAMP(3);
    ply_step<3, NP>(e, lane, st); WALK_STAMP(4);
    ply_step<4, NP>(e, lane, st); WALK_STAMP(5);
    ply_step<5, NP>(e, lane, st); WALK_STAMP(6);
    my_pairs += NP;
    {
        uint4 lf[2];
#pragma unroll
        for (int q = 0; q < 2; q++) lf[q] = lds_read_u4(e.tab + 1024u * (uint32_t)(kLvLeaf + q));
        uint32_t ppk[NP][2];
#pragma unroll
        for (int i = 0; i < NP; i++)
#pragma unroll
            for (int q = 0; q < 2; q++) ppk[i][q] = lds_read_u32(e.wsb + lf[q].x + (uint32_t)(i * sizeof(WaveScratch)));
        int I6[NP][2], I7[NP][2], pay[NP][2];
#pragma unroll
        for (int i = 0; i < NP; i++)
#pragma unroll
            for (int q = 0; q < 2; q++) {
                const uint32_t act = ((ppk[i][q] >> 21) & lf[q].y) | lf[q].z;
                const int idx6 = (int)((ppk[i][q] & 1023u) * 2 + act);
                I6[i][q] = e.s_inf[level_offset(6) + idx6];
                I7[i][q] = e.s_inf[level_offset(7) + idx6];
                pay[i][q] = e.s_pay[idx6];
            }
#pragma unroll
        for (int i = 0; i < NP; i++)
#pragma unroll
            for (int q = 0; q < 2; q++) {
                const int t = lane + 64 * q;
                if (t < 2 * 60) {
                    const int trv = t < 60 ? 0 : 1;
                    if (e.s_seen) e.s_seen[trv == 0 ? I7[i][q] : I6[i][q]] = 1;
                    atomicAdd(&e.s_cnt[trv == 0 ? I6[i][q] : I7[i][q]], 1u);
                    *(__attribute__((address_space(3))) int8_t *)(uintptr_t)(e.wsb + (uint32_t)(i * sizeof(WaveScratch) + offsetof(WaveScratch, p6)) + (uint32_t)t) =
                        (int8_t)(trv == 0 ? pay[i][q] : -pay[i][q]);
                }
            }
    }
    wave_lds_sync();
    WALK_STAMP(7);
    if (lane < 2 * kUpd) {
        const bool trav1 = lane >= kUpd;
        uint4 u[6];
#pragma unroll
        for (int q = 0; q < 6; q++) u[q] = lds_read_u4(e.tab + 1024u * (uint32_t)(kLvUpd + q));
        const uint32_t ro[5] = {u[0].x, u[0].y, u[0].z, u[0].w, u[1].x}, own = u[1].y;
        const int nX = (int)u[1].z;
        const uint32_t p6o[4] = {u[2].x, u[2].y, u[2].z, u[2].w};
        const uint32_t am[5] = {u[3].x, u[3].y, u[3].z, u[3].w, u[4].x}, af[5] = {u[4].y, u[4].z, u[4].w, u[5].x, u[5].y};
        uint32_t rec[NP][5];
        int IX[NP], pv[NP][4];
#pragma unroll
        for (int i = 0; i < NP; i++) {
            const uint32_t wi = e.wsb + (uint32_t)(i * sizeof(WaveScratch));
#pragma unroll
            for (int q = 0; q < 5; q++) rec[i][q] = lds_read_u32(wi + ro[q]);
            IX[i] = (int)((lds_read_u32(wi + own) >> 10) & 2047u);
#pragma unroll
            for (int c = 0; c < 4; c++) pv[i][c] = lds_read_i8(wi + p6o[c]);
        }
        double fq[NP][5], sg[NP][4];
        const uint32_t sig = lds_addr(e.s_sigcdf);
#pragma unroll
        for (int i = 0; i < NP; i++) {
#pragma unroll
            for (int q = 0; q < 5; q++)
                fq[i][q] = lds_read_f64(sig + ((rec[i][q] >> 10) & 2047u) * (uint32_t)(kRow * 8) + (((rec[i][q] >> 18) & am[q]) | af[q]));
            const double2 s01 = *reinterpret_cast<const double2 *>(e.s_sigcdf + IX[i] * kRow), s23 = *reinterpret_cast<const double2 *>(e.s_sigcdf + IX[i] * kRow + 2);
            sg[i][0] = s01.x; sg[i][1] = s01.y; sg[i][2] = s23.x; sg[i][3] = s23.y;
        }
#pragma unroll
        for (int i = 0; i < NP; i++) {
            const double even = (fq[i][0] * fq[i][2]) * fq[i][4], odd = fq[i][1] * fq[i][3];
            const double sX = trav1 ? odd : even, rX = trav1 ? even : odd;
            const double w = sX > 0.0 ? rX / sX : 0.0;
            double cfv[4], v = 0.0;
#pragma unroll
            for (int c = 0; c < 4; c++) {
                cfv[c] = 0.5 * (double)pv[i][c];
                const double t = fma(sg[i][c], cfv[c], v);
                v = c < nX ? t : v;
            }
#pragma unroll
            for (int c = 0; c < 4; c++) {
                const double delta = w * (cfv[c] - v);
                if (c < nX && delta != 0.0) atomicAdd(&e.s_dR[IX[i] * 4 + c], delta);
            }
        }
    }
    wave_lds_sync();
    WALK_STAMP(8);
#ifdef SCOPA_WALK_STAMPS
    if (blockIdx.x == 0 && threadIdx.x == 0) { g_walk_stamps[15] += NP; g_walk_stamps[14] += wall_clock64() - w_start_; }
#endif
}

__global__ void __launch_bounds__(64) k_lane_table(uint4 *__restrict__ g_tab) {
    const int lane = threadIdx.x;
    LaneTabRow row;
    for (int i = 0; i < kLaneSlotVecs; i++) row.v[i] = make_uint4(0u, 0u, 0u, 0u);
    lane_slot_build<0, 0>(row, lane);
    lane_slot_build<1, 0>(row, lane);
    lane_slot_build<2, 0>(row, lane);
    lane_slot_build<3, 0>(row, lane);
    lane_slot_build<4, 0>(row, lane);
    lane_slot_build<5, 0>(row, lane);
    lane_slot_build<5, 1>(row, lane);
    for (int q = 0; q < 2; q++) {
        const int t = lane + 64 * q;
        const bool on = t < 2 * 60;
        const int tt = on ? t : 0, trv = tt < 60 ? 0 : 1, j = trv ? tt - 60 : tt;
        int pj = j, kk = 0;
        if (trv == 1) { pj = j / 3; kk = j - pj * 3; }
        row.v[kLvLeaf + q] = make_uint4((uint32_t)(offsetof(WaveScratch, npk) + 4 * (npk_offset(5) + (trv ? 60 : 0) + pj)),
                                        (trv == 1 && kk > 0) ? 0u : ~0u, (trv == 1 && kk > 0) ? (uint32_t)(kk - 1) : 0u, 0u);
    }
    upd_build(row, lane);
    for (int i = 0; i < kLaneSlotVecs; i++) g_tab[i * 64 + lane] = row.v[i];
}

__device__ __forceinline__ void wave_scratch_init(WaveScratch *ws, int n_scratch, int lane, int n_infosets) {
    if (lane == 0)
        for (int i = 0; i < n_scratch; i++) ws[i].npk[kIdentSlot] = (uint32_t)n_infosets << 10;
}

__device__ __forceinline__ int group_of(unsigned int b) { return (int)((b >> 3) % kDeltaGroups); }

__global__ void __launch_bounds__(1024)
k_mccfr_traverse(const uint16_t *__restrict__ g_infoset, const int8_t *__restrict__ g_payoff,
                 const double *__restrict__ g_sigcdf, double *__restrict__ g_groups,
                 int n_infosets, uint32_t seed_lo, uint32_t seed_hi, uint32_t iteration, uint32_t b0, uint32_t nb,
                 unsigned long long *__restrict__ g_wg_counts, uint32_t *__restrict__ g_visit, unsigned long long *__restrict__ g_clock,
                 const uint4 *__restrict__ g_lane_tab, const uint32_t *__restrict__ g_iter, uint32_t track_seen) {
    extern __shared__ __align__(16) unsigned char smem[];
    __shared__ unsigned int s_vis[2];
    if (g_iter) iteration = *g_iter;
    __shared__ uint32_t s_next[1];
    __shared__ uint32_t s_slice[1];
    __shared__ uint4 s_lane_tab[kLaneSlotVecs * 64];
    const unsigned long long t_start = wall_clock64();
#ifdef SCOPA_WALK_STAMPS
    const unsigned long long c_entry_ = clock64();
#endif
    const int I = n_infosets;
    double *s_sigcdf = reinterpret_cast<double *>(smem);
    double *s_dR = s_sigcdf + (size_t)(I + 1) * kRow;
    WaveScratch *s_wave = reinterpret_cast<WaveScratch *>(s_dR + (size_t)I * 4);
    unsigned int *s_cnt = reinterpret_cast<unsigned int *>(s_wave + 2 * (blockDim.x >> 6));
    uint16_t *s_inf = reinterpret_cast<uint16_t *>(reinterpret_cast<unsigned char *>(s_cnt) + (((size_t)I * 4 + 15) & ~(size_t)15));
    int8_t *s_pay = reinterpret_cast<int8_t *>(s_inf + 1656);
    uint8_t *s_seen = reinterpret_cast<uint8_t *>(s_pay + kTerminal);

    const int tid = threadIdx.x, lane = tid & 63, wave = tid >> 6, n_waves = blockDim.x >> 6, nthr = blockDim.x;
    if (tid < 2) s_vis[tid] = 0u;
    const uint4 lane_piece = tid < kLaneSlotVecs * 64 ? g_lane_tab[tid] : make_uint4(0u, 0u, 0u, 0u);
    if (tid == 0) {
        s_slice[0] = 0u;
        const uint32_t per_wg = (nb + gridDim.x - 1) / gridDim.x, W = blockDim.x >> 6;
        const uint32_t first = blockIdx.x * per_wg, count = first < nb ? (nb - first < per_wg ? nb - first : per_wg) : 0u;
        s_next[0] = count >= 2 * W ? 2 * W : W;
    }
    const uint32_t *gi = reinterpret_cast<const uint32_t *>(g_infoset), *gp = reinterpret_cast<const uint32_t *>(g_payoff);
    {
        constexpr int kSig = 5;
        const double2 *g2 = reinterpret_cast<const double2 *>(g_sigcdf);
        double2 *s2 = reinterpret_cast<double2 *>(s_sigcdf);
        double2 v[kSig];
#pragma unroll
        for (int j = 0; j < kSig; j++) {
            const int idx = tid + j * nthr;
            v[j] = idx < I * 3 ? g2[idx] : make_double2(0.0, 0.0);
        }
        const uint32_t wi = tid < kDecision / 2 ? gi[tid] : 0u;
        const uint32_t wp = tid < kTerminal / 4 ? gp[tid] : 0u;
        const uint16_t last_inf = g_infoset[kDecision - 1];
        for (int i = tid; i < I * 2; i += nthr) reinterpret_cast<double2 *>(s_dR)[i] = make_double2(0.0, 0.0);
        for (int r = tid; r < I; r += nthr) s_cnt[r] = 0u;
        if (track_seen) for (int r = tid; r < I; r += nthr) s_seen[r] = 0;
        if (tid < 4) s_sigcdf[(size_t)I * kRow + tid] = 1.0;
#pragma unroll
        for (int j = 0; j < kSig; j++) {
            const int idx = tid + j * nthr;
            if (idx < I * 3) s2[idx] = v[j];
        }
        for (int idx = tid + kSig * nthr; idx < I * 3; idx += nthr) s2[idx] = g2[idx];
        if (tid < kLaneSlotVecs * 64) s_lane_tab[tid] = lane_piece;
        if (tid < kDecision / 2) reinterpret_cast<uint32_t *>(s_inf)[tid] = wi;
        if (tid == 0) s_inf[kDecision - 1] = last_inf;
        if (tid < kTerminal / 4) reinterpret_cast<uint32_t *>(s_pay)[tid] = wp;
    }
    for (int i = tid + nthr; i < kLaneSlotVecs * 64; i += nthr) s_lane_tab[i] = g_lane_tab[i];
    for (int i = tid + nthr; i < kDecision / 2; i += nthr) reinterpret_cast<uint32_t *>(s_inf)[i] = gi[i];
    for (int i = tid + nthr; i < kTerminal / 4; i += nthr) reinterpret_cast<uint32_t *>(s_pay)[i] = gp[i];
    __syncthreads();
    const unsigned long long t_pro = wall_clock64();
#ifdef SCOPA_WALK_STAMPS
    const unsigned long long c_barrier_ = clock64();
    unsigned long long c_loop0_ = 0, c_loop1_ = 0;
#endif

    WaveScratch *ws = s_wave + 2 * wave;
    wave_scratch_init(ws, 2, lane, I);
    WalkEnv env;
    env.wsb = lds_addr(ws); env.tab = lds_addr(s_lane_tab) + 16u * (uint32_t)lane;
    env.s_inf = s_inf; env.s_pay = s_pay; env.s_sigcdf = s_sigcdf; env.s_dR = s_dR; env.s_seen = track_seen ? s_seen : nullptr; env.s_cnt = s_cnt;
    unsigned int my_pairs = 0;
    {
#ifdef SCOPA_WALK_STAMPS
        const unsigned long long loop_start_ = clock64();
        c_loop0_ = loop_start_;
#endif
        const uint32_t per_wg = (nb + gridDim.x - 1) / gridDim.x;
        const uint32_t first = blockIdx.x * per_wg, count = first < nb ? (nb - first < per_wg ? nb - first : per_wg) : 0u;
        const uint32_t W = (uint32_t)n_waves;
        const bool start_two = count >= 2 * W;
        uint32_t c = start_two ? 2 * (uint32_t)wave : (uint32_t)wave, g = start_two ? 2u : 1u;
        for (;;) {
            if (g == 2 && c + 1 < count) {
                const uint32_t two[2] = {b0 + first + c, b0 + first + c + 1};
                walk_pairs<2>(env, lane, two, iteration, seed_lo, seed_hi, my_pairs);
            } else if (c < count) {
                const uint32_t one[1] = {b0 + first + c};
                walk_pairs<1>(env, lane, one, iteration, seed_lo, seed_hi, my_pairs);
            }
            if (count <= W || c + g >= count) break;
            g = count - c > 4 * W ? 2u : 1u;
            uint32_t got = 0;
            if (lane == 0) got = atomicAdd(s_next, g);
            c = (uint32_t)__builtin_amdgcn_readfirstlane((int)got);
            if (c >= count) break;
        }
#ifdef SCOPA_WALK_STAMPS
        c_loop1_ = clock64();
        if (lane == 0 && (blockIdx.x == 0 || blockIdx.x == 100)) g_wave_clocks[(blockIdx.x == 0 ? 0 : 16) + wave] += c_loop1_ - loop_start_;
        if (lane == 0 && blockIdx.x == 0) { unsigned int hw; asm volatile("s_getreg_b32 %0, hwreg(HW_REG_HW_ID)" : "=s"(hw)); g_wave_clocks[32 + wave] = hw; }
#endif
    }
    {
        uint32_t sl = 0;
        if (lane == 0) sl = atomicAdd(s_slice, 1u);
        sl = (uint32_t)__builtin_amdgcn_readfirstlane((int)sl);
        const int W = n_waves;
        if ((int)sl < W - W / 4) {
            const int per = (I + W - 1) / W, r0 = (W - 1 - (int)sl) * per, r1 = r0 + per < I ? r0 + per : I;
            double *tab = g_groups + (size_t)group_of(blockIdx.x) * kDeltaTable;
            for (int r = r0 + lane; r < r1; r += 64) {
#pragma unroll
                for (int k = 0; k < 4; k++) {
                    const double v = __longlong_as_double((long long)atomicExch(reinterpret_cast<unsigned long long *>(&s_dR[r * 4 + k]), 0ull));
                    if (v != 0.0) atomicAdd(&tab[group_cell(k, r)], v);
                }
                const unsigned int c = atomicExch(&s_cnt[r], 0u);
                if (c != 0u) { atomicAdd(&tab[group_cell(4, r)], (double)c); if (track_seen) s_seen[r] = 1; }
            }
        }
    }
    __syncthreads();

    const unsigned long long t_walk = wall_clock64();
    {
        const bool first0 = track_seen && tid < I && (s_seen[tid] || s_cnt[tid]) && g_visit[tid] == 0u;
        const bool first1 = track_seen && tid + nthr < I && (s_seen[tid + nthr] || s_cnt[tid + nthr]) && g_visit[tid + nthr] == 0u;
        double *tab = g_groups + (size_t)group_of(blockIdx.x) * kDeltaTable;
        for (int r = tid; r < I; r += nthr) {
            const double2 a = reinterpret_cast<const double2 *>(s_dR)[r * 2], b = reinterpret_cast<const double2 *>(s_dR)[r * 2 + 1];
            const unsigned int c = s_cnt[r];
            if (a.x != 0.0) atomicAdd(&tab[group_cell(0, r)], a.x);
            if (a.y != 0.0) atomicAdd(&tab[group_cell(1, r)], a.y);
            if (b.x != 0.0) atomicAdd(&tab[group_cell(2, r)], b.x);
            if (b.y != 0.0) atomicAdd(&tab[group_cell(3, r)], b.y);
            if (c != 0u) atomicAdd(&tab[group_cell(4, r)], (double)c);
        }
        if (first0) g_visit[tid] = 0x40000000u + (uint32_t)tid;
        if (first1) g_visit[tid + nthr] = 0x40000000u + (uint32_t)(tid + nthr);
        if (track_seen)
            for (int r = tid + 2 * nthr; r < I; r += nthr)
                if ((s_seen[r] || s_cnt[r]) && g_visit[r] == 0u) g_visit[r] = 0x40000000u + (uint32_t)r;
    }
    if (lane == 0) { atomicAdd(&s_vis[0], my_pairs * kPairDecisionVisits); atomicAdd(&s_vis[1], my_pairs * kPairTerminalVisits); }
    __syncthreads();
    if (tid < 2) atomicAdd(&g_wg_counts[blockIdx.x * 2 + tid], (unsigned long long)s_vis[tid]);
#ifdef SCOPA_WALK_STAMPS
    if (blockIdx.x == 0 && (tid & 63) == 0) {
        g_wave_phases[(tid >> 6)] += c_barrier_ - c_entry_; g_wave_phases[16 + (tid >> 6)] += c_loop0_ - c_barrier_;
        g_wave_phases[32 + (tid >> 6)] += c_loop1_ - c_loop0_; g_wave_phases[48 + (tid >> 6)] += clock64() - c_loop1_;
    }
#endif
    if (g_clock && tid == 0) {
        g_clock[blockIdx.x * 4] = t_start; g_clock[blockIdx.x * 4 + 1] = t_pro; g_clock[blockIdx.x * 4 + 2] = t_walk; g_clock[blockIdx.x * 4 + 3] = wall_clock64();
    }
}

__global__ void __launch_bounds__(1024)
k_mccfr_multi(const uint16_t *__restrict__ g_infoset, const int8_t *__restrict__ g_payoff, const uint64_t *__restrict__ g_key,
              double *__restrict__ g_regret, double *__restrict__ g_strat, const int32_t *__restrict__ g_meta, uint32_t *__restrict__ g_visit,
              unsigned long long *__restrict__ g_counters, uint32_t seed_lo, uint32_t seed_hi, uint32_t iter0, uint32_t n_iters,
              uint32_t batch, const uint4 *__restrict__ g_lane_tab) {
    extern __shared__ __align__(16) unsigned char smem[];
    __shared__ unsigned long long s_pairs;
    __shared__ uint4 s_lane_tab[kLaneSlotVecs * 64];
    for (int i = threadIdx.x; i < kLaneSlotVecs * 64; i += blockDim.x) s_lane_tab[i] = g_lane_tab[i];
    {
        const size_t deal = blockIdx.x;
        g_infoset += deal * kDecision; g_payoff += deal * kTerminal; g_key += deal * kDecision; g_regret += deal * kDecision * 4;
        g_strat += deal * kDecision * 4; g_meta += deal * 8; g_visit += deal * kDecision; g_counters += deal * 8;
    }
    const int I = g_meta[0];
    double *s_sigcdf = reinterpret_cast<double *>(smem);
    double *s_R = s_sigcdf + (size_t)(I + 1) * kRow;
    WaveScratch *s_wave = reinterpret_cast<WaveScratch *>(s_R + (size_t)I * 4);
    unsigned int *s_cnt = reinterpret_cast<unsigned int *>(s_wave + (blockDim.x >> 6));
    uint16_t *s_inf = reinterpret_cast<uint16_t *>(reinterpret_cast<unsigned char *>(s_cnt) + (((size_t)I * 4 + 15) & ~(size_t)15));
    int8_t *s_pay = reinterpret_cast<int8_t *>(s_inf + 1656);
    uint8_t *s_seen = reinterpret_cast<uint8_t *>(s_pay + kTerminal);
    const int tid = threadIdx.x, lane = tid & 63, wave = tid >> 6, n_waves = blockDim.x >> 6;
    if (tid == 0) s_pairs = 0ull;
    for (int i = tid; i < I * 4; i += blockDim.x) s_R[i] = g_regret[i];
    for (int r = tid; r < I; r += blockDim.x) { s_cnt[r] = 0u; s_seen[r] = 0; }
    for (int i = tid; i < kDecision; i += blockDim.x) s_inf[i] = g_infoset[i];
    for (int i = tid; i < kTerminal; i += blockDim.x) s_pay[i] = g_payoff[i];
    if (tid < 4) s_sigcdf[(size_t)I * kRow + tid] = 1.0;
    __syncthreads();
    WaveScratch *ws = s_wave + wave;
    wave_scratch_init(ws, 1, lane, I);
    WalkEnv env;
    env.wsb = lds_addr(ws); env.tab = lds_addr(s_lane_tab) + 16u * (uint32_t)lane;
    env.s_inf = s_inf; env.s_pay = s_pay; env.s_sigcdf = s_sigcdf; env.s_dR = s_R; env.s_seen = s_seen; env.s_cnt = s_cnt;
    unsigned int my_pairs = 0;
    unsigned long long my_total = 0ull;
    for (uint32_t it = 0; it < n_iters; it++) {
        for (int r = tid; r < I; r += blockDim.x) {
            const int n = (int)((g_key[r] >> 1) & 7);
            double sg[4];
            uint32_t thr[4];
            mc_sigma(s_R + r * 4, n, sg);
            choice_cdf(sg, n, thr);
            for (int c = 0; c < 4; c++) { s_sigcdf[r * kRow + c] = sg[c]; reinterpret_cast<uint32_t *>(s_sigcdf + r * kRow + 4)[c] = thr[c]; }
        }
        __syncthreads();
        for (uint32_t pg = (uint32_t)wave; pg < batch; pg += (uint32_t)n_waves) {
            const uint32_t one[1] = {pg};
            walk_pairs<1>(env, lane, one, iter0 + it, seed_lo, seed_hi, my_pairs);
        }
        my_total += my_pairs;
        my_pairs = 0u;
        __syncthreads();
        for (int r = tid; r < I; r += blockDim.x) {
            const unsigned int c = s_cnt[r];
            if (c) {
                s_seen[r] = 1;
                const int n = (int)((g_key[r] >> 1) & 7);
                for (int k = 0; k < n; k++) g_strat[r * 4 + k] += (double)c * s_sigcdf[r * kRow + k];
                s_cnt[r] = 0u;
            }
        }
        __syncthreads();
    }
    for (int i = tid; i < I * 4; i += blockDim.x) g_regret[i] = s_R[i];
    for (int r = tid; r < I; r += blockDim.x) if (s_seen[r] && g_visit[r] == 0u) g_visit[r] = 0x40000000u + (uint32_t)r;
    if (lane == 0) atomicAdd(&s_pairs, my_total);
    __syncthreads();
    if (tid < 2) g_counters[tid] += s_pairs * (tid == 0 ? kPairDecisionVisits : kPairTerminalVisits);
}

__global__ void __launch_bounds__(1024)
k_mccfr_chance(const uint16_t *__restrict__ g_infoset, const int8_t *__restrict__ g_payoff, const uint64_t *__restrict__ g_key,
               const int32_t *__restrict__ g_map, const int32_t *__restrict__ g_meta, const double *__restrict__ g_R ,
               double *__restrict__ g_delta , const int32_t *__restrict__ list ,
               long long *__restrict__ stamp , long long serial, unsigned long long *__restrict__ g_counters ,
               uint32_t seed_lo, uint32_t seed_hi, uint32_t iteration, uint32_t batch, const uint4 *__restrict__ g_lane_tab) {
    extern __shared__ __align__(16) unsigned char smem[];
    __shared__ unsigned int s_vis[2];
    __shared__ uint4 s_lane_tab[kLaneSlotVecs * 64];
    for (int i = threadIdx.x; i < kLaneSlotVecs * 64; i += blockDim.x) s_lane_tab[i] = g_lane_tab[i];
    const size_t slot = blockIdx.x, deal = list ? (size_t)list[slot] : slot;
    g_infoset += deal * kDecision; g_payoff += deal * kTerminal; g_key += deal * kDecision; g_map += deal * kDecision; g_meta += deal * 8;
    g_delta += slot * kDecision * 8; g_counters += deal * 2;
    const int I = g_meta[0];
    double *s_sigcdf = reinterpret_cast<double *>(smem);
    double *s_dR = s_sigcdf + (size_t)(I + 1) * kRow;
    WaveScratch *s_wave = reinterpret_cast<WaveScratch *>(s_dR + (size_t)I * 4);
    unsigned int *s_cnt = reinterpret_cast<unsigned int *>(s_wave + (blockDim.x >> 6));
    uint16_t *s_inf = reinterpret_cast<uint16_t *>(reinterpret_cast<unsigned char *>(s_cnt) + (((size_t)I * 4 + 15) & ~(size_t)15));
    int8_t *s_pay = reinterpret_cast<int8_t *>(s_inf + 1656);
    const int tid = threadIdx.x, lane = tid & 63, wave = tid >> 6, n_waves = blockDim.x >> 6;
    if (tid < 2) s_vis[tid] = 0u;
    if (tid == 0) stamp[deal] = (serial << 20) | (long long)slot;
    for (int r = tid; r < I; r += blockDim.x) {
        const int n = (int)((g_key[r] >> 1) & 7);
        const double *Rg = g_R + (size_t)g_map[r] * 4;
        const double R[4] = {Rg[0], Rg[1], Rg[2], Rg[3]};
        double sg[4];
        uint32_t thr[4];
        mc_sigma(R, n, sg);
        choice_cdf(sg, n, thr);
        for (int c = 0; c < 4; c++) { s_sigcdf[r * kRow + c] = sg[c]; reinterpret_cast<uint32_t *>(s_sigcdf + r * kRow + 4)[c] = thr[c]; }
        s_cnt[r] = 0u;
    }
    for (int i = tid; i < I * 4; i += blockDim.x) s_dR[i] = 0.0;
    for (int i = tid; i < kDecision; i += blockDim.x) s_inf[i] = g_infoset[i];
    for (int i = tid; i < kTerminal; i += blockDim.x) s_pay[i] = g_payoff[i];
    if (tid < 4) s_sigcdf[(size_t)I * kRow + tid] = 1.0;
    __syncthreads();
    WaveScratch *ws = s_wave + wave;
    wave_scratch_init(ws, 1, lane, I);
    WalkEnv env;
    env.wsb = lds_addr(ws); env.tab = lds_addr(s_lane_tab) + 16u * (uint32_t)lane;
    env.s_inf = s_inf; env.s_pay = s_pay; env.s_sigcdf = s_sigcdf; env.s_dR = s_dR; env.s_seen = nullptr; env.s_cnt = s_cnt;
    unsigned int my_pairs = 0;
    const uint32_t id0 = (uint32_t)deal * batch;
    for (uint32_t pg = (uint32_t)wave; pg < batch; pg += (uint32_t)n_waves) {
        const uint32_t one[1] = {id0 + pg};
        walk_pairs<1>(env, lane, one, iteration, seed_lo, seed_hi, my_pairs);
    }
    __syncthreads();
    for (int i = tid; i < I * 8; i += blockDim.x) {
        const int r = i >> 3, k = i & 7;
        g_delta[i] = k < 4 ? s_dR[r * 4 + k] : k == 4 ? (double)s_cnt[r] : 0.0;
    }
    if (lane == 0) atomicAdd(&s_vis[0], my_pairs);
    __syncthreads();
    if (tid < 2) g_counters[tid] += (unsigned long long)s_vis[0] * (tid == 0 ? kPairDecisionVisits : kPairTerminalVisits);
}

__global__ void __launch_bounds__(256)
k_mccfr_fold(double *__restrict__ g_groups, double *__restrict__ g_delta, int n_infosets) {
    const int r = blockIdx.x * blockDim.x + threadIdx.x;
    if (r >= n_infosets) return;
    double d[5] = {0.0, 0.0, 0.0, 0.0, 0.0};
    for (int g = 0; g < kDeltaGroups; g++)
        for (int k = 0; k < 5; k++) {
            double *q = g_groups + (size_t)g * kDeltaTable + group_cell(k, r);
            d[k] += *q;
            *q = 0.0;
        }
    for (int k = 0; k < 5; k++) g_delta[r * 5 + k] += d[k];
}

struct ApplyRow { double R[4], S[4], sg[4]; int n; };

__device__ __forceinline__ ApplyRow apply_row_load(int r, const uint64_t *__restrict__ g_key, const double *__restrict__ g_regret,
                                                   const double *__restrict__ g_strat, const double *__restrict__ g_sigcdf) {
    ApplyRow a;
    const double2 r0 = *reinterpret_cast<const double2 *>(g_regret + r * 4), r1 = *reinterpret_cast<const double2 *>(g_regret + r * 4 + 2);
    const double2 s0 = *reinterpret_cast<const double2 *>(g_strat + r * 4), s1 = *reinterpret_cast<const double2 *>(g_strat + r * 4 + 2);
    const double2 g0 = *reinterpret_cast<const double2 *>(g_sigcdf + r * kRow), g1 = *reinterpret_cast<const double2 *>(g_sigcdf + r * kRow + 2);
    a.n = (int)((g_key[r] >> 1) & 7);
    a.R[0] = r0.x; a.R[1] = r0.y; a.R[2] = r1.x; a.R[3] = r1.y;
    a.S[0] = s0.x; a.S[1] = s0.y; a.S[2] = s1.x; a.S[3] = s1.y;
    a.sg[0] = g0.x; a.sg[1] = g0.y; a.sg[2] = g1.x; a.sg[3] = g1.y;
    return a;
}

__device__ __forceinline__ void apply_row_store(int r, ApplyRow &a, const double (&d)[5], double *__restrict__ g_regret,
                                                double *__restrict__ g_strat, double *__restrict__ g_sigcdf) {
#pragma unroll
    for (int c = 0; c < 4; c++)
        if (c < a.n) { a.R[c] += d[c]; a.S[c] += d[4] * a.sg[c]; }
    *reinterpret_cast<double2 *>(g_regret + r * 4) = make_double2(a.R[0], a.R[1]);
    *reinterpret_cast<double2 *>(g_regret + r * 4 + 2) = make_double2(a.R[2], a.R[3]);
    *reinterpret_cast<double2 *>(g_strat + r * 4) = make_double2(a.S[0], a.S[1]);
    *reinterpret_cast<double2 *>(g_strat + r * 4 + 2) = make_double2(a.S[2], a.S[3]);
    double sg[4];
    uint32_t thr[4];
    mc_sigma(a.R, a.n, sg);
    choice_cdf(sg, a.n, thr);
    row_store(g_sigcdf + r * kRow, sg, thr);
}

__device__ __forceinline__ double groups_cell_take(double *__restrict__ g_groups, int r, int k) {
    double v[kDeltaGroups];
#pragma unroll
    for (int g = 0; g < kDeltaGroups; g++) v[g] = g_groups[(size_t)g * kDeltaTable + group_cell(k, r)];
    double d = 0.0;
#pragma unroll
    for (int g = 0; g < kDeltaGroups; g++) {
        d += v[g];
        if (v[g] != 0.0) g_groups[(size_t)g * kDeltaTable + group_cell(k, r)] = 0.0;
    }
    return d;
}

constexpr int kApplyLanes = 8, kApplyThreads = 64;

__global__ void __launch_bounds__(kApplyThreads)
k_mccfr_apply_groups(const uint64_t *__restrict__ g_key, double *__restrict__ g_regret, double *__restrict__ g_strat,
                     double *__restrict__ g_groups, int n_infosets, double *__restrict__ g_sigcdf, uint32_t *__restrict__ g_iter) {
    if (g_iter && blockIdx.x == 0 && threadIdx.x == 0) *g_iter += 1u;
    const int lane = threadIdx.x & 63, k = lane & (kApplyLanes - 1);
    const int r = (int)(blockIdx.x * blockDim.x + threadIdx.x) / kApplyLanes;
    const bool valid = r < n_infosets;
    ApplyRow a{};
    if (valid && k == 0) a = apply_row_load(r, g_key, g_regret, g_strat, g_sigcdf);
    const double mine = (valid && k < 5) ? groups_cell_take(g_groups, r, k) : 0.0;
    double d[5];
#pragma unroll
    for (int j = 0; j < 5; j++) d[j] = __shfl(mine, (lane & ~(kApplyLanes - 1)) + j);
    if (valid && k == 0) apply_row_store(r, a, d, g_regret, g_strat, g_sigcdf);
}

__global__ void __launch_bounds__(64)
k_mccfr_apply(const uint64_t *__restrict__ g_key, double *__restrict__ g_regret, double *__restrict__ g_strat,
              double *__restrict__ g_delta, int n_infosets, double *__restrict__ g_sigcdf) {
    const int r = blockIdx.x * blockDim.x + threadIdx.x;
    if (r >= n_infosets) return;
    double d[5];
    for (int k = 0; k < 5; k++) d[k] = g_delta[r * 5 + k];
    ApplyRow a = apply_row_load(r, g_key, g_regret, g_strat, g_sigcdf);
    for (int k = 0; k < 5; k++) g_delta[r * 5 + k] = 0.0;
    apply_row_store(r, a, d, g_regret, g_strat, g_sigcdf);
}

__global__ void __launch_bounds__(64)
k_mccfr_exchange_apply(scopa::P2PArgs xa, double *__restrict__ g_groups, const uint64_t *__restrict__ g_key, double *__restrict__ g_regret,
                       double *__restrict__ g_strat, double *__restrict__ g_sigcdf, int n_infosets) {
    __shared__ double xch[4][scopa::kP2PMaxWorld][5];
    const int rl = threadIdx.x >> 4, q = threadIdx.x & 15;
    const int r = blockIdx.x * 4 + rl;
    const bool valid = r < n_infosets;
    const double mine = (valid && q < 5) ? groups_cell_take(g_groups, r, q) : 0.0;
    double d[5];
#pragma unroll
    for (int j = 0; j < 5; j++) d[j] = __shfl(mine, (int)(threadIdx.x & ~15u) + j);
    ApplyRow a{};
    if (valid && q == 0) a = apply_row_load(r, g_key, g_regret, g_strat, g_sigcdf);
    scopa::p2p_exchange_wave4(xa, r, valid, q, d, xch[rl]);
    if (valid && q == 0) apply_row_store(r, a, d, g_regret, g_strat, g_sigcdf);
}

namespace {
struct ReplayWalk {
    double *R, *S;
    const uint16_t *inf;
    const int8_t *pay;
    uint32_t *visit;
    const double *uniforms;
    long long upos, n_uniforms;
    uint32_t seq;
    unsigned long long dvis, tvis;
};

template <int D, int TRAV>
__device__ __forceinline__ double replay_rec(ReplayWalk &w, int idx, double reach_opp, double samp_trav) {
    if constexpr (D == kPlies) {
        w.tvis++;
        const int p0 = w.pay[idx];
        return 0.5 * (double)(TRAV == 0 ? p0 : -p0);
    } else {
        constexpr int n = 4 - (D >> 1);
        constexpr bool is_trav = (D & 1) == TRAV;
        w.dvis++;
        const int I = w.inf[level_offset(D) + idx];
        if (w.visit[I] == 0u) w.visit[I] = ++w.seq;
        double R[4], sigma[4], cdf[4];
        for (int c = 0; c < 4; c++) R[c] = w.R[I * 4 + c];
        mc_sigma(R, n, sigma);
        choice_cdf_f64(sigma, n, cdf);
        const double u = w.upos < w.n_uniforms ? w.uniforms[w.upos] : 0.0;
        w.upos++;
        int a = (cdf[0] <= u) + (cdf[1] <= u) + (cdf[2] <= u) + (cdf[3] <= u);
        a = a < n - 1 ? a : n - 1;
        double sa = sigma[0];
        for (int i = 1; i < n; i++) sa = a == i ? sigma[i] : sa;
        if constexpr (!is_trav) {
            return replay_rec<D + 1, TRAV>(w, idx * n + a, reach_opp * sa, samp_trav);
        } else {
            const double util = replay_rec<D + 1, TRAV>(w, idx * n + a, reach_opp, samp_trav * sa);
            double cfv[4] = {0.0, 0.0, 0.0, 0.0};
#pragma unroll 1
            for (int i = 0; i < n; i++)
                cfv[i] = replay_rec<D + 1, TRAV>(w, idx * n + i, reach_opp, samp_trav * sigma[i]);
            double v = 0.0;
            for (int i = 0; i < n; i++) v = fma(sigma[i], cfv[i], v);
            const double wt = samp_trav > 0.0 ? reach_opp / samp_trav : 0.0;
            for (int i = 0; i < n; i++) {
                w.R[I * 4 + i] += wt * (cfv[i] - v);
                w.S[I * 4 + i] += 1.0 * sigma[i];
            }
            return util;
        }
    }
}
}

__global__ void __launch_bounds__(256)
k_mccfr_replay(const uint16_t *__restrict__ g_infoset, const int8_t *__restrict__ g_payoff, const uint64_t *__restrict__ g_key,
               double *__restrict__ g_regret, double *__restrict__ g_strat, const double *__restrict__ uniforms,
               long long n_uniforms, int n_iters, unsigned long long *__restrict__ g_counters, long long *__restrict__ consumed,
               uint32_t *__restrict__ g_visit, int32_t *__restrict__ g_meta) {
    extern __shared__ __align__(16) unsigned char smem[];
    __shared__ uint16_t s_inf[1656];
    __shared__ int8_t s_pay[kTerminal];
    __shared__ uint32_t s_visit[kDecision];
    const int tid = threadIdx.x, I = g_meta[0], cells = I * 4;
    double *R = reinterpret_cast<double *>(smem), *S = R + cells;
    for (int i = tid; i < cells; i += blockDim.x) { R[i] = g_regret[i]; S[i] = g_strat[i]; }
    for (int i = tid; i < kDecision; i += blockDim.x) s_inf[i] = g_infoset[i];
    for (int i = tid; i < kTerminal; i += blockDim.x) s_pay[i] = g_payoff[i];
    for (int i = tid; i < I; i += blockDim.x) s_visit[i] = g_visit[i];
    __syncthreads();
    if (tid == 0) {
        ReplayWalk w;
        w.R = R; w.S = S; w.inf = s_inf; w.pay = s_pay; w.visit = s_visit; w.uniforms = uniforms; w.upos = 0; w.n_uniforms = n_uniforms;
        w.seq = (uint32_t)g_meta[1]; w.dvis = 0; w.tvis = 0;
#pragma unroll 1
        for (int it = 0; it < n_iters; it++) {
            replay_rec<0, 0>(w, 0, 1.0, 1.0);
            replay_rec<0, 1>(w, 0, 1.0, 1.0);
        }
        g_counters[0] += w.dvis;
        g_counters[1] += w.tvis;
        g_meta[1] = (int32_t)w.seq;
        *consumed = w.upos;
    }
    __syncthreads();
    for (int i = tid; i < cells; i += blockDim.x) { g_regret[i] = R[i]; g_strat[i] = S[i]; }
    for (int i = tid; i < I; i += blockDim.x) g_visit[i] = s_visit[i];
}


static size_t traverse_lds_bytes(int n_infosets, int waves) {
    size_t b = ((size_t)(n_infosets + 1) * kRow + (size_t)n_infosets * 4) * sizeof(double);
    b += (size_t)waves * 2 * sizeof(WaveScratch);
    b += (((size_t)n_infosets * 4 + 15) & ~(size_t)15);
    b += 1656 * 2 + 576;
    b += (size_t)n_infosets;
    return (b + 15) & ~(size_t)15;
}

static int32_t ensure_lane_table(scopa_ctx *ctx) {
    if (ctx->d_lane_tab) return SCOPA_OK;
    SC_HIP(ctx, hipMalloc(&ctx->d_lane_tab, (size_t)kLaneSlotVecs * 64 * sizeof(uint4)));
    hipLaunchKernelGGL(k_lane_table, dim3(1), dim3(64), 0, ctx->stream, (uint4 *)ctx->d_lane_tab);
    SC_HIP(ctx, hipGetLastError());
    return SCOPA_OK;
}

struct TraverseGeom { int threads; size_t lds; uint32_t grid; };

static int32_t refresh_all_seen(scopa_ctx *ctx, bool now) {
    if (ctx->mccfr_all_seen) return SCOPA_OK;
    if (!now && ++ctx->mccfr_seen_wait < 16u) return SCOPA_OK;
    ctx->mccfr_seen_wait = 0;
    uint32_t h[kDecision];
    SC_HIP(ctx, hipMemcpyAsync(h, ctx->d_visit, (size_t)ctx->n_infosets * sizeof(uint32_t), hipMemcpyDeviceToHost, ctx->stream));
    SC_HIP(ctx, hipStreamSynchronize(ctx->stream));
    bool all = true;
    for (int r = 0; r < ctx->n_infosets; r++) all = all && h[r] != 0u;
    ctx->mccfr_all_seen = all;
    return SCOPA_OK;
}

static int32_t prepare_traverse(scopa_ctx *ctx, uint32_t nb, TraverseGeom *g) {
    int waves = 16;
    while (waves > 1 && traverse_lds_bytes(ctx->n_infosets, waves) + kStaticLds > (size_t)ctx->lds_limit) waves = waves > 2 ? waves - 2 : 1;
    g->threads = waves * 64;
    g->lds = traverse_lds_bytes(ctx->n_infosets, waves);
    SC_REQUIRE(ctx, g->lds + kStaticLds <= (size_t)ctx->lds_limit, SCOPA_ELIMIT, "mccfr traverse: infoset tables do not fit in LDS");
    SC_LDS_ATTR(ctx, scopa::kLdsTraverse, k_mccfr_traverse, ctx->lds_limit - kStaticLds);
    const uint32_t n_passes = (nb + waves - 1) / waves;
    g->grid = n_passes < (uint32_t)ctx->n_cus ? n_passes : (uint32_t)ctx->n_cus;
    SC_REQUIRE(ctx, g->grid <= 1024u, SCOPA_ELIMIT, "mccfr traverse: more than 1024 compute units");
    static_assert(kClockStride >= 4 * 512, "clock sample stride");
    if (int32_t rc = ensure_lane_table(ctx)) return rc;
    if (int32_t rc = refresh_all_seen(ctx, false)) return rc;
    if (!ctx->sigcdf_valid) {
        hipLaunchKernelGGL(k_mccfr_prepare, dim3((ctx->n_infosets + 255) / 256), dim3(256), 0, ctx->stream, ctx->d_key,
                           ctx->d_regret, ctx->d_sigcdf, ctx->n_infosets);
        SC_HIP(ctx, hipGetLastError());
        ctx->sigcdf_valid = true;
    }
    return SCOPA_OK;
}

static int32_t launch_traverse(scopa_ctx *ctx, uint32_t iteration, uint32_t b0, uint32_t nb) {
    TraverseGeom g;
    if (int32_t rc = prepare_traverse(ctx, nb, &g)) return rc;
    const int threads = g.threads;
    const size_t lds = g.lds;
    const uint32_t grid = g.grid;
    hipEvent_t ev0 = nullptr, ev1 = nullptr;
    const bool sampled = prof_events(ctx, &ev0, &ev1);
    unsigned long long *clock = sampled && ctx->d_clock && grid <= 512u ? ctx->d_clock + (size_t)((ctx->prof_launches - 1) % kClockSamples) * kClockStride : nullptr;
    if (sampled) ctx->clock_grid[(ctx->prof_launches - 1) % kClockSamples] = clock ? (uint16_t)grid : (uint16_t)0;
    if (sampled)
        hipExtLaunchKernelGGL(k_mccfr_traverse, dim3(grid), dim3(threads), lds, ctx->stream, ev0, ev1, 0, ctx->d_infoset, ctx->d_payoff,
                              ctx->d_sigcdf, ctx->d_groups, ctx->n_infosets, (uint32_t)ctx->seed, (uint32_t)(ctx->seed >> 32),
                              iteration, b0, nb, ctx->d_counters + 8, ctx->d_visit, clock, (const uint4 *)ctx->d_lane_tab, (const uint32_t *)nullptr,
                              ctx->mccfr_all_seen ? 0u : 1u);
    else
        hipLaunchKernelGGL(k_mccfr_traverse, dim3(grid), dim3(threads), lds, ctx->stream, ctx->d_infoset, ctx->d_payoff,
                           ctx->d_sigcdf, ctx->d_groups, ctx->n_infosets, (uint32_t)ctx->seed, (uint32_t)(ctx->seed >> 32),
                           iteration, b0, nb, ctx->d_counters + 8, ctx->d_visit, clock, (const uint4 *)ctx->d_lane_tab, (const uint32_t *)nullptr,
                           ctx->mccfr_all_seen ? 0u : 1u);
    SC_HIP(ctx, hipGetLastError());
    return SCOPA_OK;
}

void scopa::mccfr_graphs_clear(scopa_ctx *ctx) {
    for (auto &e : ctx->mccfr_graphs) (void)hipGraphExecDestroy((hipGraphExec_t)e.exec);
    ctx->mccfr_graphs.clear();
}

static int32_t graph_for(scopa_ctx *ctx, uint32_t batch, uint32_t k, hipGraphExec_t *out) {
    const uint32_t track = ctx->mccfr_all_seen ? 0u : 1u;
    for (auto &e : ctx->mccfr_graphs)
        if (e.batch == batch && e.k == k && e.track == track) { *out = (hipGraphExec_t)e.exec; return SCOPA_OK; }
    TraverseGeom g;
    if (int32_t rc = prepare_traverse(ctx, batch, &g)) return rc;
    uint32_t *d_iter = reinterpret_cast<uint32_t *>(ctx->d_meta + 2);
    hipGraph_t graph = nullptr;
    SC_HIP(ctx, hipStreamBeginCapture(ctx->stream, hipStreamCaptureModeThreadLocal));
    for (uint32_t i = 0; i < k; i++) {
        hipLaunchKernelGGL(k_mccfr_traverse, dim3(g.grid), dim3(g.threads), g.lds, ctx->stream, ctx->d_infoset, ctx->d_payoff,
                           ctx->d_sigcdf, ctx->d_groups, ctx->n_infosets, (uint32_t)ctx->seed, (uint32_t)(ctx->seed >> 32),
                           0u, 0u, batch, ctx->d_counters + 8, ctx->d_visit, (unsigned long long *)nullptr, (const uint4 *)ctx->d_lane_tab, (const uint32_t *)d_iter, track);
        hipLaunchKernelGGL(k_mccfr_apply_groups, dim3((ctx->n_infosets * kApplyLanes + kApplyThreads - 1) / kApplyThreads), dim3(kApplyThreads), 0, ctx->stream, ctx->d_key,
                           ctx->d_regret, ctx->d_strat, ctx->d_groups, ctx->n_infosets, ctx->d_sigcdf, d_iter);
    }
    const hipError_t e_end = hipStreamEndCapture(ctx->stream, &graph);
    if (e_end != hipSuccess || !graph) return scopa::fail(ctx, SCOPA_EHIP, "mccfr graph: stream capture", e_end);
    hipGraphExec_t exec = nullptr;
    const hipError_t e_inst = hipGraphInstantiate(&exec, graph, nullptr, nullptr, 0);
    (void)hipGraphDestroy(graph);
    if (e_inst != hipSuccess) return scopa::fail(ctx, SCOPA_EHIP, "mccfr graph: instantiate", e_inst);
    if (ctx->mccfr_graphs.size() >= 16) { (void)hipGraphExecDestroy((hipGraphExec_t)ctx->mccfr_graphs.front().exec); ctx->mccfr_graphs.erase(ctx->mccfr_graphs.begin()); }
    ctx->mccfr_graphs.push_back({batch, k, track, (void *)exec});
    *out = exec;
    return SCOPA_OK;
}

static size_t multi_lds_bytes(int max_infosets, int waves) {
    size_t b = ((size_t)(max_infosets + 1) * kRow + (size_t)max_infosets * 4) * sizeof(double) + (size_t)waves * sizeof(WaveScratch);
    b += (((size_t)max_infosets * 4 + 15) & ~(size_t)15) + 1656 * 2 + 576 + (size_t)max_infosets;
    return (b + 15) & ~(size_t)15;
}

namespace scopa {
int32_t launch_mccfr_multi(scopa_ctx *ctx, int n_deals, int max_infosets, const uint16_t *d_infoset, const int8_t *d_payoff,
                           const uint64_t *d_key, double *d_regret, double *d_strat, const int32_t *d_meta, uint32_t *d_visit,
                           unsigned long long *d_counters, uint64_t seed, uint32_t iter0, uint32_t n_iters, uint32_t batch) {
    int waves = 16;
    while (waves > 2 && multi_lds_bytes(max_infosets, waves) + kStaticLdsMulti > (size_t)ctx->lds_limit) waves -= 2;
    SC_REQUIRE(ctx, multi_lds_bytes(max_infosets, waves) + kStaticLdsMulti <= (size_t)ctx->lds_limit, SCOPA_ELIMIT, "mccfr multi: infoset tables do not fit in LDS");
    SC_LDS_ATTR(ctx, scopa::kLdsMulti, k_mccfr_multi, ctx->lds_limit - kStaticLdsMulti);
    if (int32_t rc = ensure_lane_table(ctx)) return rc;
    hipLaunchKernelGGL(k_mccfr_multi, dim3(n_deals), dim3(waves * 64), multi_lds_bytes(max_infosets, waves), ctx->stream, d_infoset, d_payoff, d_key, d_regret, d_strat,
                       d_meta, d_visit, d_counters, (uint32_t)seed, (uint32_t)(seed >> 32), iter0, n_iters, batch, (const uint4 *)ctx->d_lane_tab);
    SC_HIP(ctx, hipGetLastError());
    return SCOPA_OK;
}

int32_t launch_mccfr_chance(scopa_ctx *ctx, int n_slots, int max_infosets, const uint16_t *d_infoset, const int8_t *d_payoff, const uint64_t *d_key,
                            const int32_t *d_map, const int32_t *d_meta, const double *d_R, double *d_delta, const int32_t *d_list, long long *d_stamp,
                            long long serial, unsigned long long *d_counters, uint64_t seed, uint32_t iteration, uint32_t batch) {
    int waves = 16;
    while (waves > 2 && multi_lds_bytes(max_infosets, waves) + kStaticLdsMulti > (size_t)ctx->lds_limit) waves -= 2;
    SC_REQUIRE(ctx, multi_lds_bytes(max_infosets, waves) + kStaticLdsMulti <= (size_t)ctx->lds_limit, SCOPA_ELIMIT, "mccfr chance: infoset tables do not fit in LDS");
    SC_LDS_ATTR(ctx, scopa::kLdsMccfrChance, k_mccfr_chance, ctx->lds_limit - kStaticLdsMulti);
    if (int32_t rc = ensure_lane_table(ctx)) return rc;
    hipLaunchKernelGGL(k_mccfr_chance, dim3(n_slots), dim3(waves * 64), multi_lds_bytes(max_infosets, waves), ctx->stream, d_infoset, d_payoff, d_key, d_map,
                       d_meta, d_R, d_delta, d_list, d_stamp, serial, d_counters, (uint32_t)seed, (uint32_t)(seed >> 32), iteration, batch,
                       (const uint4 *)ctx->d_lane_tab);
    SC_HIP(ctx, hipGetLastError());
    return SCOPA_OK;
}
}

extern "C" {

int32_t scopa_mccfr_seed(scopa_ctx *ctx, uint64_t seed) {
    if (!ctx) return SCOPA_EINVAL;
    if (seed != ctx->seed) scopa::mccfr_graphs_clear(ctx);
    ctx->seed = seed;
    return SCOPA_OK;
}

int32_t scopa_mccfr_traverse(scopa_ctx *ctx, uint32_t iteration, uint32_t b0, uint32_t nb) {
    if (!ctx) return SCOPA_EINVAL;
    SC_REQUIRE(ctx, ctx->has_deal, SCOPA_ESTATE, "scopa_mccfr_traverse: no deal set");
    SC_REQUIRE(ctx, nb <= (1u << 30), SCOPA_EINVAL, "scopa_mccfr_traverse: batch too large");
    if (nb == 0) return SCOPA_OK;
    SC_HIP(ctx, hipSetDevice(ctx->device));
    scopa::Range r("scopa mccfr traverse (split path)");
    const int32_t rc = launch_traverse(ctx, iteration, b0, nb);
    if (rc != SCOPA_OK) return rc;
    hipLaunchKernelGGL(k_mccfr_fold, dim3((ctx->n_infosets + 255) / 256), dim3(256), 0, ctx->stream, ctx->d_groups, ctx->d_delta, ctx->n_infosets);
    SC_HIP(ctx, hipGetLastError());
    return SCOPA_OK;
}

int32_t scopa_mccfr_delta_buffer(scopa_ctx *ctx, void **d_delta, size_t *bytes) {
    if (!ctx || !d_delta || !bytes) return SCOPA_EINVAL;
    SC_REQUIRE(ctx, ctx->has_deal, SCOPA_ESTATE, "scopa_mccfr_delta_buffer: no deal set");
    *d_delta = ctx->d_delta;
    *bytes = (size_t)ctx->n_infosets * 5 * sizeof(double);
    return SCOPA_OK;
}

int32_t scopa_mccfr_bind_delta(scopa_ctx *ctx, void *d_buf, size_t bytes) {
    if (!ctx) return SCOPA_EINVAL;
    SC_REQUIRE(ctx, ctx->has_deal, SCOPA_ESTATE, "scopa_mccfr_bind_delta: no deal set");
    const size_t need = (size_t)ctx->n_infosets * 5 * sizeof(double);
    if (d_buf) {
        SC_REQUIRE(ctx, bytes >= need, SCOPA_EINVAL, "scopa_mccfr_bind_delta: buffer smaller than n_infosets*5 float64");
        SC_REQUIRE(ctx, ((uintptr_t)d_buf & 15) == 0, SCOPA_EINVAL, "scopa_mccfr_bind_delta: buffer must be 16-byte aligned");
        ctx->d_delta = static_cast<double *>(d_buf);
    } else {
        ctx->d_delta = ctx->d_delta_own;
    }
    SC_HIP(ctx, hipSetDevice(ctx->device));
    SC_HIP(ctx, hipMemsetAsync(ctx->d_delta, 0, need, ctx->stream));
    return SCOPA_OK;
}

int32_t scopa_mccfr_delta_get(scopa_ctx *ctx, double *h_delta) {
    if (!ctx || !h_delta) return SCOPA_EINVAL;
    SC_REQUIRE(ctx, ctx->has_deal, SCOPA_ESTATE, "scopa_mccfr_delta_get: no deal set");
    SC_HIP(ctx, hipMemcpyAsync(h_delta, ctx->d_delta, (size_t)ctx->n_infosets * 5 * sizeof(double), hipMemcpyDeviceToHost, ctx->stream));
    SC_HIP(ctx, hipStreamSynchronize(ctx->stream));
    return SCOPA_OK;
}

int32_t scopa_mccfr_delta_set(scopa_ctx *ctx, const double *h_delta) {
    if (!ctx || !h_delta) return SCOPA_EINVAL;
    SC_REQUIRE(ctx, ctx->has_deal, SCOPA_ESTATE, "scopa_mccfr_delta_set: no deal set");
    SC_HIP(ctx, hipMemcpyAsync(ctx->d_delta, h_delta, (size_t)ctx->n_infosets * 5 * sizeof(double), hipMemcpyHostToDevice, ctx->stream));
    SC_HIP(ctx, hipStreamSynchronize(ctx->stream));
    return SCOPA_OK;
}

int32_t scopa_mccfr_apply(scopa_ctx *ctx) {
    if (!ctx) return SCOPA_EINVAL;
    SC_REQUIRE(ctx, ctx->has_deal, SCOPA_ESTATE, "scopa_mccfr_apply: no deal set");
    SC_HIP(ctx, hipSetDevice(ctx->device));
    scopa::Range r("scopa mccfr apply (split path)");
    if (!ctx->sigcdf_valid) {
        hipLaunchKernelGGL(k_mccfr_prepare, dim3((ctx->n_infosets + 255) / 256), dim3(256), 0, ctx->stream, ctx->d_key,
                           ctx->d_regret, ctx->d_sigcdf, ctx->n_infosets);
        SC_HIP(ctx, hipGetLastError());
    }
    hipLaunchKernelGGL(k_mccfr_apply, dim3((ctx->n_infosets + 63) / 64), dim3(64), 0, ctx->stream, ctx->d_key,
                       ctx->d_regret, ctx->d_strat, ctx->d_delta, ctx->n_infosets, ctx->d_sigcdf);
    SC_HIP(ctx, hipGetLastError());
    ctx->sigcdf_valid = true;
    ctx->iteration++;
    return SCOPA_OK;
}

int32_t scopa_mccfr_iteration_counter(scopa_ctx *ctx, uint32_t *iteration) {
    if (!ctx || !iteration) return SCOPA_EINVAL;
    *iteration = ctx->iteration;
    return SCOPA_OK;
}

int32_t scopa_mccfr_iterate(scopa_ctx *ctx, uint32_t batch, uint32_t n_iters) {
    if (!ctx) return SCOPA_EINVAL;
    SC_REQUIRE(ctx, ctx->has_deal, SCOPA_ESTATE, "scopa_mccfr_iterate: no deal set");
    SC_REQUIRE(ctx, batch > 0 && batch <= (1u << 30), SCOPA_EINVAL, "scopa_mccfr_iterate: bad batch");
    SC_HIP(ctx, hipSetDevice(ctx->device));
    if (ctx->mccfr_graph_mode && !ctx->prof_on && n_iters > 1) {
        TraverseGeom g;
        if (int32_t rc = prepare_traverse(ctx, batch, &g)) return rc;
        SC_HIP(ctx, hipMemsetD32Async(reinterpret_cast<hipDeviceptr_t>(ctx->d_meta + 2), (int)ctx->iteration, 1, ctx->stream));
        for (uint32_t left = n_iters; left > 0;) {
            const uint32_t k = left >= 64u ? 64u : left;
            if (int32_t rc = refresh_all_seen(ctx, true)) return rc;
            hipGraphExec_t exec = nullptr;
            if (int32_t rc = graph_for(ctx, batch, k, &exec)) return rc;
            SC_HIP(ctx, hipGraphLaunch(exec, ctx->stream));
            ctx->iteration += k;
            left -= k;
        }
        ctx->sigcdf_valid = true;
        return SCOPA_OK;
    }
    for (uint32_t it = 0; it < n_iters; it++) {
        int32_t rc;
        { scopa::Range r("scopa mccfr traverse"); rc = launch_traverse(ctx, ctx->iteration, 0, batch); }
        if (rc != SCOPA_OK) return rc;
        scopa::Range r("scopa mccfr apply");
        hipLaunchKernelGGL(k_mccfr_apply_groups, dim3((ctx->n_infosets * kApplyLanes + kApplyThreads - 1) / kApplyThreads), dim3(kApplyThreads), 0, ctx->stream, ctx->d_key,
                           ctx->d_regret, ctx->d_strat, ctx->d_groups, ctx->n_infosets, ctx->d_sigcdf, (uint32_t *)nullptr);
        SC_HIP(ctx, hipGetLastError());
        ctx->sigcdf_valid = true;
        ctx->iteration++;
    }
    return SCOPA_OK;
}

int32_t scopa_mccfr_graph_mode(scopa_ctx *ctx, int32_t on) {
    if (!ctx) return SCOPA_EINVAL;
    ctx->mccfr_graph_mode = on != 0;
    if (!on) scopa::mccfr_graphs_clear(ctx);
    return SCOPA_OK;
}

int32_t scopa_mccfr_iterate_sharded(scopa_ctx *ctx, uint32_t b0, uint32_t nb, uint32_t n_iters) {
    if (!ctx) return SCOPA_EINVAL;
    SC_REQUIRE(ctx, ctx->has_deal, SCOPA_ESTATE, "scopa_mccfr_iterate_sharded: no deal set");
    SC_REQUIRE(ctx, nb > 0 && nb <= (1u << 30), SCOPA_EINVAL, "scopa_mccfr_iterate_sharded: bad slice");
    SC_HIP(ctx, hipSetDevice(ctx->device));
    for (uint32_t it = 0; it < n_iters; it++) {
        scopa::P2PArgs xa{};
        SC_REQUIRE(ctx, scopa::p2p_next_args(ctx, &xa), SCOPA_ESTATE, "mccfr sharded iteration: peer exchange not connected");
        int32_t rc;
        { scopa::Range r("scopa mccfr traverse"); rc = launch_traverse(ctx, ctx->iteration, b0, nb); }
        if (rc != SCOPA_OK) return rc;
        scopa::Range r("scopa mccfr exchange + apply");
        hipLaunchKernelGGL(k_mccfr_exchange_apply, dim3((ctx->n_infosets + 3) / 4), dim3(64), 0, ctx->stream, xa, ctx->d_groups, ctx->d_key,
                           ctx->d_regret, ctx->d_strat, ctx->d_sigcdf, ctx->n_infosets);
        SC_HIP(ctx, hipGetLastError());
        ctx->sigcdf_valid = true;
        ctx->iteration++;
    }
    SC_HIP(ctx, hipStreamSynchronize(ctx->stream));
    return scopa::p2p_check(ctx, "scopa_mccfr_iterate_sharded");
}

int32_t scopa_mccfr_replay(scopa_ctx *ctx, int32_t n_iters, const double *h_uniforms, int64_t n_uniforms, int64_t *consumed) {
    if (!ctx || n_iters < 0 || n_uniforms < 0 || (n_uniforms > 0 && !h_uniforms)) return SCOPA_EINVAL;
    SC_REQUIRE(ctx, ctx->has_deal, SCOPA_ESTATE, "scopa_mccfr_replay: no deal set");
    SC_HIP(ctx, hipSetDevice(ctx->device));
    const size_t ubytes = (size_t)n_uniforms * sizeof(double);
    { const int32_t rc = ensure_scratch(ctx, ubytes + 64); if (rc != SCOPA_OK) return rc; }
    long long *d_consumed = reinterpret_cast<long long *>(ctx->d_scratch);
    double *d_u = ctx->d_scratch + 8;
    if (n_uniforms) SC_HIP(ctx, hipMemcpyAsync(d_u, h_uniforms, ubytes, hipMemcpyHostToDevice, ctx->stream));
    SC_LDS_ATTR(ctx, scopa::kLdsReplay, k_mccfr_replay, ctx->lds_limit - 12 * 1024);
    hipLaunchKernelGGL(k_mccfr_replay, dim3(1), dim3(256), (size_t)ctx->n_infosets * 64, ctx->stream, ctx->d_infoset, ctx->d_payoff, ctx->d_key,
                       ctx->d_regret, ctx->d_strat, d_u, (long long)n_uniforms, (int)n_iters, ctx->d_counters, d_consumed,
                       ctx->d_visit, ctx->d_meta);
    SC_HIP(ctx, hipGetLastError());
    long long used = 0;
    SC_HIP(ctx, hipMemcpyAsync(&used, d_consumed, sizeof used, hipMemcpyDeviceToHost, ctx->stream));
    SC_HIP(ctx, hipStreamSynchronize(ctx->stream));
    ctx->sigcdf_valid = false;
    if (consumed) *consumed = used;
    return SCOPA_OK;
}

}

#ifdef SCOPA_WALK_STAMPS
extern "C" int scopa_debug_wave_phases(unsigned long long *out64) {
    return hipMemcpyFromSymbol(out64, HIP_SYMBOL(g_wave_phases), sizeof(unsigned long long) * 64) == hipSuccess ? 0 : -1;
}
extern "C" int scopa_debug_wave_clocks(unsigned long long *out48) {
    return hipMemcpyFromSymbol(out48, HIP_SYMBOL(g_wave_clocks), sizeof(unsigned long long) * 48) == hipSuccess ? 0 : -1;
}
extern "C" int scopa_debug_walk_stamps(unsigned long long *out16, int reset) {
    if (hipMemcpyFromSymbol(out16, HIP_SYMBOL(g_walk_stamps), sizeof(unsigned long long) * 16) != hipSuccess) return -1;
    if (reset) { unsigned long long z[16] = {0}; if (hipMemcpyToSymbol(HIP_SYMBOL(g_walk_stamps), z, sizeof(z)) != hipSuccess) return -1; }
    return 0;
}
#endif
```

scopa_amd/csrc/scopa_tree.hip:

```cpp
#include <string.h>

#include <vector>

#include "scopa_ctx.h"

using namespace scopa;

#ifndef SCOPA_STEP_UNROLL
#define SCOPA_STEP_UNROLL 2
#endif
__global__ void __launch_bounds__(256) k_step_batch(scopa_state *__restrict__ states,
                                                     const uint8_t *__restrict__ actions, int64_t n) {
    constexpr int U = SCOPA_STEP_UNROLL;
    const int64_t stride = (int64_t)gridDim.x * blockDim.x;
    uint4 *st = reinterpret_cast<uint4 *>(states);
    for (int64_t i = (int64_t)blockIdx.x * blockDim.x + threadIdx.x; i < n; i += U * stride) {
        uint4 v[U];
        int act[U];
#pragma unroll
        for (int u = 0; u < U; u++) {
            const int64_t j = i + u * stride;
            v[u] = j < n ? st[j] : make_uint4(0u, 0u, 0u, 0u);
            act[u] = j < n ? actions[j] & 15 : 0;
        }
#pragma unroll
        for (int u = 0; u < U; u++) {
            const int64_t j = i + u * stride;
            if (j < n) {
                step_words(v[u].x, v[u].y, v[u].z, v[u].w, act[u]);
                st[j] = v[u];
            }
        }
    }
}

__device__ __forceinline__ int dfs_index(int d, int j) {
    int dfs = 0;
    for (int k = d - 1; k >= 0; k--) {
        const int n = nlegal_at(k);
        const int a = j % n;
        j /= n;
        dfs += 1 + a * subtree_size(k + 1);
    }
    return dfs;
}

__global__ void __launch_bounds__(1024) k_tree_build(const uint8_t *__restrict__ perm16, scopa_state *__restrict__ states,
                                                      uint16_t *__restrict__ infoset_of, int8_t *__restrict__ payoff,
                                                      uint64_t *__restrict__ key_of_infoset, int32_t *__restrict__ meta) {
    __shared__ uint64_t s_key[576];
    __shared__ int s_dfs[576];
    __shared__ int s_first[kDecision];
    __shared__ int s_scan[kNodes + 1];
    const int tid = threadIdx.x, nt = blockDim.x;
    {
        const size_t deal = blockIdx.x;
        perm16 += deal * 16; states += deal * kNodes; infoset_of += deal * kDecision; payoff += deal * kTerminal;
        key_of_infoset += deal * kDecision; meta += deal * 8;
    }

    for (int i = tid; i <= kNodes; i += nt) s_scan[i] = 0;
    if (tid == 0) {
        uint8_t p[16];
        for (int i = 0; i < 16; i++) p[i] = perm16[i];
        scopa_state root;
        state_init(root, p);
        states[0] = root;
    }
    __syncthreads();
    for (int d = 0; d < kPlies; d++) {
        const int n = nlegal_at(d), w1 = level_width(d + 1);
        for (int j = tid; j < w1; j += nt) {
            scopa_state s = states[level_offset(d) + j / n];
            const int action = nib(s.hand[s.step & 1], j % n);
            step(s, action);
            states[level_offset(d + 1) + j] = s;
        }
        __syncthreads();
    }
    for (int j = tid; j < kTerminal; j += nt) {
        int r0, r1;
        rewards_x2(states[level_offset(8) + j], r0, r1);
        payoff[j] = (int8_t)r0;
    }
    for (int d = 0; d < kPlies; d++) {
        const int w = level_width(d), off = level_offset(d);
        for (int j = tid; j < w; j += nt) { s_key[j] = infoset_key(states[off + j], d & 1); s_dfs[j] = dfs_index(d, j); }
        __syncthreads();
        for (int j = tid; j < w; j += nt) {
            const uint64_t k = s_key[j];
            int first = s_dfs[j];
            for (int m = 0; m < w; m++) {
                if (s_key[m] == k) { first = s_dfs[m]; break; }
            }
            s_first[off + j] = first;
            if (first == s_dfs[j]) s_scan[first + 1] = 1;
        }
        __syncthreads();
    }
    {
        __shared__ int s_wsum[16];
        const int lane = tid & 63, wave = tid >> 6, base = tid * 4;
        int v[4], sum = 0;
        for (int q = 0; q < 4; q++) { v[q] = base + q <= kNodes ? s_scan[base + q] : 0; sum += v[q]; }
        int x = sum;
        for (int o = 1; o < 64; o <<= 1) { const int y = __shfl_up(x, o); if (lane >= o) x += y; }
        if (lane == 63) s_wsum[wave] = x;
        __syncthreads();
        if (tid == 0) {
            int acc = 0;
            for (int w = 0; w < 16; w++) { const int t = s_wsum[w]; s_wsum[w] = acc; acc += t; }
            meta[0] = acc;
        }
        __syncthreads();
        int run = x - sum + s_wsum[wave];
        for (int q = 0; q < 4; q++) { run += v[q]; if (base + q <= kNodes) s_scan[base + q] = run; }
    }
    __syncthreads();
    for (int d = 0; d < kPlies; d++) {
        const int w = level_width(d), off = level_offset(d);
        for (int j = tid; j < w; j += nt) {
            const int first = s_first[off + j];
            const int id = s_scan[first];
            infoset_of[off + j] = (uint16_t)id;
            if (first == dfs_index(d, j)) key_of_infoset[id] = infoset_key(states[off + j], d & 1);
        }
    }
}

__global__ void k_tables_reset(double *regret, double *strat, double *local, const uint64_t *key_of_infoset,
                               const int32_t *meta) {
    {
        const size_t deal = blockIdx.y;
        regret += deal * kDecision * 4; strat += deal * kDecision * 4; local += deal * kDecision * 4;
        key_of_infoset += deal * kDecision; meta += deal * 8;
    }
    const int I = meta[0];
    for (int i = blockIdx.x * blockDim.x + threadIdx.x; i < kDecision * 4; i += gridDim.x * blockDim.x) {
        const int row = i >> 2, col = i & 3;
        regret[i] = 0.0;
        strat[i] = 0.0;
        double l = 0.0;
        if (row < I) {
            const int n = (int)((key_of_infoset[row] >> 1) & 7);
            if (col < n) l = 1.0 / (double)n;
        }
        local[i] = l;
    }
}

extern "C" {

int32_t scopa_step_batch(scopa_ctx *ctx, scopa_state *d_states, const uint8_t *d_actions, int64_t n) {
    if (!ctx || n < 0 || (n > 0 && (!d_states || !d_actions))) return SCOPA_EINVAL;
    if (n == 0) return SCOPA_OK;
    SC_REQUIRE(ctx, ((uintptr_t)d_states & 15) == 0, SCOPA_EINVAL, "scopa_step_batch: states must be 16-byte aligned");
    SC_HIP(ctx, hipSetDevice(ctx->device));
    int64_t blocks = (n + 255) / 256;
#ifndef SCOPA_STEP_BLOCKS_PER_CU
#define SCOPA_STEP_BLOCKS_PER_CU 128
#endif
    const int64_t cap = (int64_t)ctx->n_cus * SCOPA_STEP_BLOCKS_PER_CU;
    if (blocks > cap) blocks = cap;
    hipLaunchKernelGGL(k_step_batch, dim3((unsigned)blocks), dim3(256), 0, ctx->stream, d_states, d_actions, n);
    SC_HIP(ctx, hipGetLastError());
    return SCOPA_OK;
}

int32_t scopa_step_batch_host(scopa_ctx *ctx, scopa_state *h_states, const uint8_t *h_actions, int64_t n) {
    if (!ctx || n < 0 || (n > 0 && (!h_states || !h_actions))) return SCOPA_EINVAL;
    if (n == 0) return SCOPA_OK;
    SC_HIP(ctx, hipSetDevice(ctx->device));
    scopa_state *d_s = nullptr;
    uint8_t *d_a = nullptr;
    SC_HIP(ctx, hipMalloc(&d_s, (size_t)n * sizeof(scopa_state)));
    hipError_t e = hipMalloc(&d_a, (size_t)n);
    if (e != hipSuccess) { (void)hipFree(d_s); return fail(ctx, SCOPA_EHIP, "hipMalloc(actions)", e); }
    int32_t rc = SCOPA_OK;
    if ((e = hipMemcpyAsync(d_s, h_states, (size_t)n * sizeof(scopa_state), hipMemcpyHostToDevice, ctx->stream)) != hipSuccess ||
        (e = hipMemcpyAsync(d_a, h_actions, (size_t)n, hipMemcpyHostToDevice, ctx->stream)) != hipSuccess)
        rc = fail(ctx, SCOPA_EHIP, "hipMemcpyAsync(H2D)", e);
    if (rc == SCOPA_OK) rc = scopa_step_batch(ctx, d_s, d_a, n);
    if (rc == SCOPA_OK && (e = hipMemcpyAsync(h_states, d_s, (size_t)n * sizeof(scopa_state), hipMemcpyDeviceToHost, ctx->stream)) != hipSuccess)
        rc = fail(ctx, SCOPA_EHIP, "hipMemcpyAsync(D2H)", e);
    e = hipStreamSynchronize(ctx->stream);
    if (rc == SCOPA_OK && e != hipSuccess) rc = fail(ctx, SCOPA_EHIP, "hipStreamSynchronize", e);
    (void)hipFree(d_s);
    (void)hipFree(d_a);
    return rc;
}

int32_t scopa_tables_reset(scopa_ctx *ctx) {
    if (!ctx) return SCOPA_EINVAL;
    SC_REQUIRE(ctx, ctx->has_deal, SCOPA_ESTATE, "scopa_tables_reset: no deal set");
    SC_HIP(ctx, hipSetDevice(ctx->device));
    hipLaunchKernelGGL(k_tables_reset, dim3(8), dim3(1024), 0, ctx->stream, ctx->d_regret, ctx->d_strat, ctx->d_local,
                       ctx->d_key, ctx->d_meta);
    SC_HIP(ctx, hipGetLastError());
    SC_HIP(ctx, hipMemsetAsync(ctx->d_visit, 0, sizeof(uint32_t) * kDecision, ctx->stream));
    SC_HIP(ctx, hipMemsetAsync(ctx->d_meta + 1, 0, sizeof(int32_t), ctx->stream));
    SC_HIP(ctx, hipMemsetAsync(ctx->d_delta, 0, (size_t)(ctx->d_delta == ctx->d_delta_own ? kDecision : ctx->n_infosets) * 5 * sizeof(double), ctx->stream));
    ctx->iteration = 0;
    ctx->sigcdf_valid = false;
    ctx->mccfr_all_seen = false;
    ctx->mccfr_seen_wait = 0;
    return SCOPA_OK;
}

int32_t scopa_set_deal(scopa_ctx *ctx, const uint8_t perm16[16]) {
    if (!ctx || !perm16) return SCOPA_EINVAL;
    uint32_t seen = 0;
    for (int i = 0; i < 16; i++) { if (perm16[i] > 15) return fail(ctx, SCOPA_EINVAL, "scopa_set_deal: card id > 15"); seen |= 1u << perm16[i]; }
    SC_REQUIRE(ctx, seen == 0xFFFFu, SCOPA_EINVAL, "scopa_set_deal: not a permutation of the 16 cards");
    SC_HIP(ctx, hipSetDevice(ctx->device));
    { const int32_t rc = ensure_scratch(ctx, 4096); if (rc != SCOPA_OK) return rc; }
    memcpy(ctx->perm, perm16, 16);
    SC_HIP(ctx, hipMemcpyAsync(ctx->d_scratch, ctx->perm, 16, hipMemcpyHostToDevice, ctx->stream));
    hipLaunchKernelGGL(k_tree_build, dim3(1), dim3(1024), 0, ctx->stream, (const uint8_t *)ctx->d_scratch, ctx->d_states,
                       ctx->d_infoset, ctx->d_payoff, ctx->d_key, ctx->d_meta);
    SC_HIP(ctx, hipGetLastError());
    int32_t n_inf = 0;
    SC_HIP(ctx, hipMemcpyAsync(&n_inf, ctx->d_meta, sizeof n_inf, hipMemcpyDeviceToHost, ctx->stream));
    SC_HIP(ctx, hipStreamSynchronize(ctx->stream));
    SC_REQUIRE(ctx, n_inf > 0 && n_inf <= kDecision, SCOPA_EHIP, "scopa_set_deal: tree build produced a bad infoset count");
    ctx->n_infosets = n_inf;
    ctx->has_deal = true;
    ctx->d_delta = ctx->d_delta_own;
    ctx->sched_valid = false;
    ctx->sdnode_valid = false;
    ctx->eval_thr_valid = false;
    ctx->sdpol_valid = false;
    ctx->exact_last_route = -1;
    scopa::mccfr_graphs_clear(ctx);
    return scopa_tables_reset(ctx);
}

int32_t scopa_tree_counts(scopa_ctx *ctx, int32_t *n_nodes, int32_t *n_decision, int32_t *n_infosets) {
    if (!ctx) return SCOPA_EINVAL;
    SC_REQUIRE(ctx, ctx->has_deal, SCOPA_ESTATE, "scopa_tree_counts: no deal set");
    if (n_nodes) *n_nodes = kNodes;
    if (n_decision) *n_decision = kDecision;
    if (n_infosets) *n_infosets = ctx->n_infosets;
    return SCOPA_OK;
}

int32_t scopa_tree_export(scopa_ctx *ctx, scopa_state *h_states, int32_t *h_infoset, int8_t *h_r2, uint64_t *h_infoset_key,
                          int8_t *h_infoset_nlegal, int8_t *h_infoset_legal) {
    if (!ctx) return SCOPA_EINVAL;
    SC_REQUIRE(ctx, ctx->has_deal, SCOPA_ESTATE, "scopa_tree_export: no deal set");
    SC_HIP(ctx, hipSetDevice(ctx->device));
    std::vector<scopa_state> st(kNodes);
    std::vector<uint16_t> inf(kDecision);
    std::vector<int8_t> pay(kTerminal);
    std::vector<uint64_t> keys((size_t)ctx->n_infosets);
    SC_HIP(ctx, hipMemcpyAsync(st.data(), ctx->d_states, sizeof(scopa_state) * kNodes, hipMemcpyDeviceToHost, ctx->stream));
    SC_HIP(ctx, hipMemcpyAsync(inf.data(), ctx->d_infoset, sizeof(uint16_t) * kDecision, hipMemcpyDeviceToHost, ctx->stream));
    SC_HIP(ctx, hipMemcpyAsync(pay.data(), ctx->d_payoff, kTerminal, hipMemcpyDeviceToHost, ctx->stream));
    SC_HIP(ctx, hipMemcpyAsync(keys.data(), ctx->d_key, sizeof(uint64_t) * keys.size(), hipMemcpyDeviceToHost, ctx->stream));
    SC_HIP(ctx, hipStreamSynchronize(ctx->stream));
    for (int d = 0; d <= kPlies; d++) {
        for (int j = 0; j < level_width(d); j++) {
            int dfs = 0, jj = j;
            for (int k = d - 1; k >= 0; k--) { const int n = nlegal_at(k); dfs += 1 + (jj % n) * subtree_size(k + 1); jj /= n; }
            const int bfs = level_offset(d) + j;
            if (h_states) h_states[dfs] = st[(size_t)bfs];
            if (h_infoset) h_infoset[dfs] = d < kPlies ? (int32_t)inf[(size_t)bfs] : -1;
            if (h_r2) {
                const int r0 = d < kPlies ? 0 : pay[(size_t)j];
                h_r2[dfs * 2] = (int8_t)r0;
                h_r2[dfs * 2 + 1] = (int8_t)-r0;
            }
        }
    }
    for (int i = 0; i < ctx->n_infosets; i++) {
        const uint64_t k = keys[(size_t)i];
        if (h_infoset_key) h_infoset_key[i] = k;
        const int n = (int)((k >> 1) & 7);
        if (h_infoset_nlegal) h_infoset_nlegal[i] = (int8_t)n;
        if (h_infoset_legal)
            for (int c = 0; c < 4; c++) h_infoset_legal[i * 4 + c] = (int8_t)(c < n ? (int)((k >> (4 + 4 * c)) & 15) : -1);
    }
    return SCOPA_OK;
}

}
```

Measured before the change: 136.8 billion.

## Renumber infosets so multi-choice rows come first and shrink LDS tables

Adds a walk-order permutation that places infosets with two or more legal actions first, and remaps the tree's infoset ids to this order. The traverse kernel then keeps sigma/CDF rows and regret deltas in LDS only for choice infosets, which cuts shared-memory footprint and load volume. Apply, fold and prepare kernels translate between the reference and walk orderings using the permutation maps and a popcount rank structure passed by value. This adds indirection in the update kernels and a new one-block kernel at deal setup.

```diff
diff --git a/include/scopa.h b/include/scopa.h
--- a/include/scopa.h
+++ b/include/scopa.h
@@ -99,6 +99,7 @@
 int32_t scopa_mccfr_iteration_counter(scopa_ctx *ctx, uint32_t *iteration);
 int32_t scopa_mccfr_graph_mode(scopa_ctx *ctx, int32_t on);
 int32_t scopa_debug_lds_limit(scopa_ctx *ctx, int32_t bytes);
+int32_t scopa_debug_walk_order(scopa_ctx *ctx, int32_t *n_choice, uint16_t *h_walk_to_ref);
 
 int32_t scopa_sdcfr_frontier_width(int32_t traverser, int32_t ply);
 int32_t scopa_sdcfr_features(scopa_ctx *ctx, int32_t ply, int64_t n, const int32_t *d_idx, float *d_feats, float *d_mask);
diff --git a/scopa_amd/_lib.py b/scopa_amd/_lib.py
--- a/scopa_amd/_lib.py
+++ b/scopa_amd/_lib.py
@@ -19,7 +19,7 @@
     "scopa_tree_counts", "scopa_tree_export", "scopa_tables_reset", "scopa_tables_get", "scopa_tables_set",
     "scopa_visited_get", "scopa_cfr_exact_iterate", "scopa_cfr_exact_traverse", "scopa_cfr_exact_mode", "scopa_cfr_exact_last_route", "scopa_cfr_exact_traverse_from", "scopa_mccfr_replay", "scopa_mccfr_seed",
     "scopa_mccfr_iterate", "scopa_mccfr_traverse", "scopa_mccfr_delta_buffer", "scopa_mccfr_bind_delta", "scopa_mccfr_delta_get", "scopa_mccfr_delta_set", "scopa_mccfr_apply",
-    "scopa_mccfr_iteration_counter", "scopa_mccfr_graph_mode", "scopa_debug_lds_limit", "scopa_sdcfr_frontier_width", "scopa_sdcfr_features", "scopa_sdcfr_expand",
+    "scopa_mccfr_iteration_counter", "scopa_mccfr_graph_mode", "scopa_debug_lds_limit", "scopa_debug_walk_order", "scopa_sdcfr_frontier_width", "scopa_sdcfr_features", "scopa_sdcfr_expand",
     "scopa_sdcfr_terminal_values", "scopa_sdcfr_backward", "scopa_sdcfr_visits", "scopa_sdcfr_policy_get", "scopa_sdcfr_traverse_fused", "scopa_sdcfr_image_floats", "scopa_sdcfr_pack_weights", "scopa_sdcfr_tuning", "scopa_sdcfr_mode", "scopa_sdcfr_train_params", "scopa_sdcfr_train_step", "scopa_sdcfr_train_steps", "scopa_sdcfr_average_policy", "scopa_features_from_states",
     "scopa_eval_init_states", "scopa_eval_step", "scopa_eval_tabular_step", "scopa_eval_tabular_prepare", "scopa_eval_tabular_match", "scopa_cfr_sync_iterate", "scopa_cfr_sync_iterate_weighted", "scopa_multi_create", "scopa_multi_destroy",
     "scopa_multi_deal_py_seeds", "scopa_multi_set_perms", "scopa_multi_perms_get", "scopa_multi_build", "scopa_multi_cfr_exact_iterate",
@@ -126,6 +126,7 @@
         "scopa_mccfr_iteration_counter": (i32, [vp, C.POINTER(u32)]),
         "scopa_mccfr_graph_mode": (i32, [vp, i32]),
         "scopa_debug_lds_limit": (i32, [vp, i32]),
+        "scopa_debug_walk_order": (i32, [vp, vp, vp]),
         "scopa_exploitability": (i32, [vp, vp, vp, vp]),
         "scopa_sdcfr_frontier_width": (i32, [i32, i32]),
         "scopa_sdcfr_features": (i32, [vp, i32, i64, vp, vp, vp]),
@@ -452,6 +453,12 @@
     def debug_lds_limit(self, nbytes):
         self._ck(self._L.scopa_debug_lds_limit(self._h, int(nbytes)), "scopa_debug_lds_limit")
 
+    def debug_walk_order(self):
+        c = C.c_int32()
+        w2r = np.zeros(self.n_infosets, np.uint16)
+        self._ck(self._L.scopa_debug_walk_order(self._h, C.byref(c), _ptr(w2r)), "scopa_debug_walk_order")
+        return c.value, w2r
+
     def mccfr_iteration(self):
         v = C.c_uint32()
         self._ck(self._L.scopa_mccfr_iteration_counter(self._h, C.byref(v)), "scopa_mccfr_iteration_counter")
diff --git a/scopa_amd/csrc/scopa_ctx.h b/scopa_amd/csrc/scopa_ctx.h
--- a/scopa_amd/csrc/scopa_ctx.h
+++ b/scopa_amd/csrc/scopa_ctx.h
@@ -8,6 +8,12 @@
 #include "../../include/scopa.h"
 #include "scopa_rules.h"
 
+namespace scopa {
+struct WalkRank {
+    uint64_t choice[26];
+    uint32_t before[26];
+};
+}
 struct scopa_p2p;
 struct scopa_team_solver;
 
@@ -34,6 +40,10 @@
     double *d_scratch = nullptr;
     double *d_sigcdf = nullptr;
     bool sigcdf_valid = false;
+    int n_choice = 0;
+    uint16_t *d_walk_inf = nullptr;
+    uint16_t *d_walk2ref = nullptr, *d_ref2walk = nullptr;
+    scopa::WalkRank walk_rank;
     bool mccfr_all_seen = false;
     uint32_t mccfr_seen_wait = 0;
     double *d_groups = nullptr;
@@ -108,6 +118,13 @@
     return (size_t)k * kGroupRows + (size_t)r;
 #endif
 }
+constexpr int kWalkMapStride = 1664;
+__device__ __forceinline__ int walk_id(const WalkRank &wr, int word, int r, int n_choice) {
+    const uint64_t m = wr.choice[word];
+    const int bit = r & 63;
+    const int below = (int)wr.before[word] + __popcll(m & ((1ull << bit) - 1ull));
+    return ((m >> bit) & 1ull) ? below : n_choice + (r - below);
+}
 constexpr int kClockSamples = 2048, kClockStride = 2048;
 
 inline int32_t fail(scopa_ctx *ctx, int32_t code, const char *what, hipError_t e = hipSuccess) {
diff --git a/scopa_amd/csrc/scopa_host.hip b/scopa_amd/csrc/scopa_host.hip
--- a/scopa_amd/csrc/scopa_host.hip
+++ b/scopa_amd/csrc/scopa_host.hip
@@ -128,6 +128,7 @@
               hipMalloc(&ctx->d_meta, sizeof(int32_t) * 8) == hipSuccess &&
               hipMalloc(&ctx->d_visit, sizeof(uint32_t) * kDecision) == hipSuccess &&
               hipMalloc(&ctx->d_sigcdf, (size_t)kDecision * 6 * sizeof(double)) == hipSuccess &&
+              hipMalloc(&ctx->d_walk_inf, (size_t)3 * scopa::kWalkMapStride * sizeof(uint16_t)) == hipSuccess &&
               hipMalloc(&ctx->d_groups, scopa::kDeltaGroups * scopa::kDeltaTable * sizeof(double)) == hipSuccess &&
               hipMalloc(&ctx->d_regret, rows * 4 * sizeof(double)) == hipSuccess &&
               hipMalloc(&ctx->d_strat, rows * 4 * sizeof(double)) == hipSuccess &&
@@ -135,8 +136,10 @@
               hipMalloc(&ctx->d_delta_own, rows * 5 * sizeof(double)) == hipSuccess &&
               hipMalloc(&ctx->d_counters, (8 + 2 * 1024) * sizeof(unsigned long long)) == hipSuccess;
     ctx->d_delta = ctx->d_delta_own;
+    if (ok) { ctx->d_walk2ref = ctx->d_walk_inf + scopa::kWalkMapStride; ctx->d_ref2walk = ctx->d_walk_inf + 2 * scopa::kWalkMapStride; }
     if (ok) ok = hipMemsetAsync(ctx->d_counters, 0, (8 + 2 * 1024) * sizeof(unsigned long long), ctx->stream) == hipSuccess &&
                  hipMemsetAsync(ctx->d_delta, 0, rows * 5 * sizeof(double), ctx->stream) == hipSuccess &&
+                 hipMemsetAsync(ctx->d_walk_inf, 0, (size_t)3 * scopa::kWalkMapStride * sizeof(uint16_t), ctx->stream) == hipSuccess &&
                  hipMemsetAsync(ctx->d_groups, 0, scopa::kDeltaGroups * scopa::kDeltaTable * sizeof(double), ctx->stream) == hipSuccess;
     if (!ok) { scopa_ctx_destroy(ctx); return SCOPA_ENOMEM; }
     *out = ctx;
@@ -152,7 +155,7 @@
     scopa::mccfr_graphs_clear(ctx);
     for (hipEvent_t e : ctx->ev_pool) (void)hipEventDestroy(e);
     void *bufs[] = {ctx->d_states, ctx->d_infoset, ctx->d_payoff, ctx->d_key, ctx->d_meta, ctx->d_regret, ctx->d_strat,
-                    ctx->d_local, ctx->d_delta_own, ctx->d_scratch, ctx->d_counters, ctx->d_visit, ctx->d_sigcdf, ctx->d_groups, ctx->d_clock, ctx->d_sched, ctx->d_lane_tab, ctx->d_sdnode, ctx->d_sdpol, ctx->d_train_partial, ctx->d_eval_thr, ctx->d_pair_thr, ctx->d_sdavg};
+                    ctx->d_local, ctx->d_delta_own, ctx->d_scratch, ctx->d_counters, ctx->d_visit, ctx->d_sigcdf, ctx->d_walk_inf, ctx->d_groups, ctx->d_clock, ctx->d_sched, ctx->d_lane_tab, ctx->d_sdnode, ctx->d_sdpol, ctx->d_train_partial, ctx->d_eval_thr, ctx->d_pair_thr, ctx->d_sdavg};
     for (void *b : bufs) if (b) (void)hipFree(b);
     if (ctx->own_stream) (void)hipStreamDestroy(ctx->stream);
     delete ctx;
@@ -167,6 +170,17 @@
     ctx->lds_limit = bytes ? bytes : (int)prop.sharedMemPerBlock;
     ctx->lds_attr_done = 0;
     scopa::mccfr_graphs_clear(ctx);
+    return SCOPA_OK;
+}
+
+int32_t scopa_debug_walk_order(scopa_ctx *ctx, int32_t *n_choice, uint16_t *h_walk_to_ref) {
+    if (!ctx) return SCOPA_EINVAL;
+    SC_REQUIRE(ctx, ctx->has_deal, SCOPA_ESTATE, "scopa_debug_walk_order: no deal set");
+    if (n_choice) *n_choice = ctx->n_choice;
+    if (h_walk_to_ref) {
+        SC_HIP(ctx, hipMemcpyAsync(h_walk_to_ref, ctx->d_walk2ref, (size_t)ctx->n_infosets * sizeof(uint16_t), hipMemcpyDeviceToHost, ctx->stream));
+        SC_HIP(ctx, hipStreamSynchronize(ctx->stream));
+    }
     return SCOPA_OK;
 }
 
diff --git a/scopa_amd/csrc/scopa_mccfr.hip b/scopa_amd/csrc/scopa_mccfr.hip
--- a/scopa_amd/csrc/scopa_mccfr.hip
+++ b/scopa_amd/csrc/scopa_mccfr.hip
@@ -48,7 +48,8 @@
 }
 
 __global__ void __launch_bounds__(256)
-k_mccfr_prepare(const uint64_t *__restrict__ g_key, const double *__restrict__ g_regret, double *__restrict__ g_sigcdf, int n_infosets) {
+k_mccfr_prepare(const uint64_t *__restrict__ g_key, const double *__restrict__ g_regret, double *__restrict__ g_sigcdf, int n_infosets,
+                const uint16_t *__restrict__ g_ref2walk) {
     const int r = blockIdx.x * blockDim.x + threadIdx.x;
     if (r >= n_infosets) return;
     const int n = (int)((g_key[r] >> 1) & 7);
@@ -57,7 +58,7 @@
     for (int c = 0; c < 4; c++) R[c] = g_regret[r * 4 + c];
     mc_sigma(R, n, sg);
     choice_cdf(sg, n, thr);
-    row_store(g_sigcdf + r * kRow, sg, thr);
+    row_store(g_sigcdf + (size_t)g_ref2walk[r] * kRow, sg, thr);
 }
 
 constexpr int kIdentSlot = 166;
@@ -187,6 +188,7 @@
 template <int D, int NP>
 __device__ __forceinline__ void ply_step(const WalkEnv &e, int lane, NodeRegs (&st)[NP]) {
     constexpr int n = 4 - (D >> 1);
+    static_assert(D <= 5 && n >= 2, "ply_step walks the plies whose nodes have a choice");
     constexpr int c0 = task_nodes(0, D), c1 = task_nodes(1, D);
     constexpr int NR = c0 + c1 > 64 ? 2 : 1;
     struct Pre {
@@ -378,19 +380,20 @@
     for (int i = 0; i < kLaneSlotVecs; i++) g_tab[i * 64 + lane] = row.v[i];
 }
 
-__device__ __forceinline__ void wave_scratch_init(WaveScratch *ws, int n_scratch, int lane, int n_infosets) {
+__device__ __forceinline__ void wave_scratch_init(WaveScratch *ws, int n_scratch, int lane, int ident_row) {
     if (lane == 0)
-        for (int i = 0; i < n_scratch; i++) ws[i].npk[kIdentSlot] = (uint32_t)n_infosets << 10;
+        for (int i = 0; i < n_scratch; i++) ws[i].npk[kIdentSlot] = (uint32_t)ident_row << 10;
 }
 
 __device__ __forceinline__ int group_of(unsigned int b) { return (int)((b >> 3) % kDeltaGroups); }
 
 __global__ void __launch_bounds__(1024)
-k_mccfr_traverse(const uint16_t *__restrict__ g_infoset, const int8_t *__restrict__ g_payoff,
+k_mccfr_traverse(const uint16_t *__restrict__ g_infoset , const int8_t *__restrict__ g_payoff,
                  const double *__restrict__ g_sigcdf, double *__restrict__ g_groups,
-                 int n_infosets, uint32_t seed_lo, uint32_t seed_hi, uint32_t iteration, uint32_t b0, uint32_t nb,
+                 int n_infosets, int n_choice, uint32_t seed_lo, uint32_t seed_hi, uint32_t iteration, uint32_t b0, uint32_t nb,
                  unsigned long long *__restrict__ g_wg_counts, uint32_t *__restrict__ g_visit, unsigned long long *__restrict__ g_clock,
-                 const uint4 *__restrict__ g_lane_tab, const uint32_t *__restrict__ g_iter, uint32_t track_seen) {
+                 const uint4 *__restrict__ g_lane_tab, const uint32_t *__restrict__ g_iter, uint32_t track_seen,
+                 const uint16_t *__restrict__ g_walk2ref) {
     extern __shared__ __align__(16) unsigned char smem[];
     __shared__ unsigned int s_vis[2];
     if (g_iter) iteration = *g_iter;
@@ -401,10 +404,10 @@
 #ifdef SCOPA_WALK_STAMPS
     const unsigned long long c_entry_ = clock64();
 #endif
-    const int I = n_infosets;
+    const int I = n_infosets, C = n_choice;
     double *s_sigcdf = reinterpret_cast<double *>(smem);
-    double *s_dR = s_sigcdf + (size_t)(I + 1) * kRow;
-    WaveScratch *s_wave = reinterpret_cast<WaveScratch *>(s_dR + (size_t)I * 4);
+    double *s_dR = s_sigcdf + (size_t)(C + 1) * kRow;
+    WaveScratch *s_wave = reinterpret_cast<WaveScratch *>(s_dR + (size_t)C * 4);
     unsigned int *s_cnt = reinterpret_cast<unsigned int *>(s_wave + 2 * (blockDim.x >> 6));
     uint16_t *s_inf = reinterpret_cast<uint16_t *>(reinterpret_cast<unsigned char *>(s_cnt) + (((size_t)I * 4 + 15) & ~(size_t)15));
     int8_t *s_pay = reinterpret_cast<int8_t *>(s_inf + 1656);
@@ -428,21 +431,21 @@
 #pragma unroll
         for (int j = 0; j < kSig; j++) {
             const int idx = tid + j * nthr;
-            v[j] = idx < I * 3 ? g2[idx] : make_double2(0.0, 0.0);
+            v[j] = idx < C * 3 ? g2[idx] : make_double2(0.0, 0.0);
         }
         const uint32_t wi = tid < kDecision / 2 ? gi[tid] : 0u;
         const uint32_t wp = tid < kTerminal / 4 ? gp[tid] : 0u;
         const uint16_t last_inf = g_infoset[kDecision - 1];
-        for (int i = tid; i < I * 2; i += nthr) reinterpret_cast<double2 *>(s_dR)[i] = make_double2(0.0, 0.0);
+        for (int i = tid; i < C * 2; i += nthr) reinterpret_cast<double2 *>(s_dR)[i] = make_double2(0.0, 0.0);
         for (int r = tid; r < I; r += nthr) s_cnt[r] = 0u;
         if (track_seen) for (int r = tid; r < I; r += nthr) s_seen[r] = 0;
-        if (tid < 4) s_sigcdf[(size_t)I * kRow + tid] = 1.0;
+        if (tid < 4) s_sigcdf[(size_t)C * kRow + tid] = 1.0;
 #pragma unroll
         for (int j = 0; j < kSig; j++) {
             const int idx = tid + j * nthr;
-            if (idx < I * 3) s2[idx] = v[j];
-        }
-        for (int idx = tid + kSig * nthr; idx < I * 3; idx += nthr) s2[idx] = g2[idx];
+            if (idx < C * 3) s2[idx] = v[j];
+        }
+        for (int idx = tid + kSig * nthr; idx < C * 3; idx += nthr) s2[idx] = g2[idx];
         if (tid < kLaneSlotVecs * 64) s_lane_tab[tid] = lane_piece;
         if (tid < kDecision / 2) reinterpret_cast<uint32_t *>(s_inf)[tid] = wi;
         if (tid == 0) s_inf[kDecision - 1] = last_inf;
@@ -459,7 +462,7 @@
 #endif
 
     WaveScratch *ws = s_wave + 2 * wave;
-    wave_scratch_init(ws, 2, lane, I);
+    wave_scratch_init(ws, 2, lane, C);
     WalkEnv env;
     env.wsb = lds_addr(ws); env.tab = lds_addr(s_lane_tab) + 16u * (uint32_t)lane;
     env.s_inf = s_inf; env.s_pay = s_pay; env.s_sigcdf = s_sigcdf; env.s_dR = s_dR; env.s_seen = track_seen ? s_seen : nullptr; env.s_cnt = s_cnt;
@@ -504,10 +507,12 @@
             const int per = (I + W - 1) / W, r0 = (W - 1 - (int)sl) * per, r1 = r0 + per < I ? r0 + per : I;
             double *tab = g_groups + (size_t)group_of(blockIdx.x) * kDeltaTable;
             for (int r = r0 + lane; r < r1; r += 64) {
-#pragma unroll
-                for (int k = 0; k < 4; k++) {
-                    const double v = __longlong_as_double((long long)atomicExch(reinterpret_cast<unsigned long long *>(&s_dR[r * 4 + k]), 0ull));
-                    if (v != 0.0) atomicAdd(&tab[group_cell(k, r)], v);
+                if (r < C) {
+#pragma unroll
+                    for (int k = 0; k < 4; k++) {
+                        const double v = __longlong_as_double((long long)atomicExch(reinterpret_cast<unsigned long long *>(&s_dR[r * 4 + k]), 0ull));
+                        if (v != 0.0) atomicAdd(&tab[group_cell(k, r)], v);
+                    }
                 }
                 const unsigned int c = atomicExch(&s_cnt[r], 0u);
                 if (c != 0u) { atomicAdd(&tab[group_cell(4, r)], (double)c); if (track_seen) s_seen[r] = 1; }
@@ -518,11 +523,13 @@
 
     const unsigned long long t_walk = wall_clock64();
     {
-        const bool first0 = track_seen && tid < I && (s_seen[tid] || s_cnt[tid]) && g_visit[tid] == 0u;
-        const bool first1 = track_seen && tid + nthr < I && (s_seen[tid + nthr] || s_cnt[tid + nthr]) && g_visit[tid + nthr] == 0u;
+        const int ref0 = track_seen && tid < I ? (int)g_walk2ref[tid] : 0, ref1 = track_seen && tid + nthr < I ? (int)g_walk2ref[tid + nthr] : 0;
+        const bool first0 = track_seen && tid < I && (s_seen[tid] || s_cnt[tid]) && g_visit[ref0] == 0u;
+        const bool first1 = track_seen && tid + nthr < I && (s_seen[tid + nthr] || s_cnt[tid + nthr]) && g_visit[ref1] == 0u;
         double *tab = g_groups + (size_t)group_of(blockIdx.x) * kDeltaTable;
         for (int r = tid; r < I; r += nthr) {
-            const double2 a = reinterpret_cast<const double2 *>(s_dR)[r * 2], b = reinterpret_cast<const double2 *>(s_dR)[r * 2 + 1];
+            const double2 zero = make_double2(0.0, 0.0);
+            const double2 a = r < C ? reinterpret_cast<const double2 *>(s_dR)[r * 2] : zero, b = r < C ? reinterpret_cast<const double2 *>(s_dR)[r * 2 + 1] : zero;
             const unsigned int c = s_cnt[r];
             if (a.x != 0.0) atomicAdd(&tab[group_cell(0, r)], a.x);
             if (a.y != 0.0) atomicAdd(&tab[group_cell(1, r)], a.y);
@@ -530,11 +537,13 @@
             if (b.y != 0.0) atomicAdd(&tab[group_cell(3, r)], b.y);
             if (c != 0u) atomicAdd(&tab[group_cell(4, r)], (double)c);
         }
-        if (first0) g_visit[tid] = 0x40000000u + (uint32_t)tid;
-        if (first1) g_visit[tid + nthr] = 0x40000000u + (uint32_t)(tid + nthr);
+        if (first0) g_visit[ref0] = 0x40000000u + (uint32_t)ref0;
+        if (first1) g_visit[ref1] = 0x40000000u + (uint32_t)ref1;
         if (track_seen)
-            for (int r = tid + 2 * nthr; r < I; r += nthr)
-                if ((s_seen[r] || s_cnt[r]) && g_visit[r] == 0u) g_visit[r] = 0x40000000u + (uint32_t)r;
+            for (int r = tid + 2 * nthr; r < I; r += nthr) {
+                const int ref = (int)g_walk2ref[r];
+                if ((s_seen[r] || s_cnt[r]) && g_visit[ref] == 0u) g_visit[ref] = 0x40000000u + (uint32_t)ref;
+            }
     }
     if (lane == 0) { atomicAdd(&s_vis[0], my_pairs * kPairDecisionVisits); atomicAdd(&s_vis[1], my_pairs * kPairTerminalVisits); }
     __syncthreads();
@@ -683,13 +692,14 @@
 }
 
 __global__ void __launch_bounds__(256)
-k_mccfr_fold(double *__restrict__ g_groups, double *__restrict__ g_delta, int n_infosets) {
+k_mccfr_fold(double *__restrict__ g_groups, double *__restrict__ g_delta, int n_infosets, const uint16_t *__restrict__ g_ref2walk) {
     const int r = blockIdx.x * blockDim.x + threadIdx.x;
     if (r >= n_infosets) return;
+    const int w = (int)g_ref2walk[r];
     double d[5] = {0.0, 0.0, 0.0, 0.0, 0.0};
     for (int g = 0; g < kDeltaGroups; g++)
         for (int k = 0; k < 5; k++) {
-            double *q = g_groups + (size_t)g * kDeltaTable + group_cell(k, r);
+            double *q = g_groups + (size_t)g * kDeltaTable + group_cell(k, w);
             d[k] += *q;
             *q = 0.0;
         }
@@ -698,12 +708,12 @@
 
 struct ApplyRow { double R[4], S[4], sg[4]; int n; };
 
-__device__ __forceinline__ ApplyRow apply_row_load(int r, const uint64_t *__restrict__ g_key, const double *__restrict__ g_regret,
+__device__ __forceinline__ ApplyRow apply_row_load(int r, int w, const uint64_t *__restrict__ g_key, const double *__restrict__ g_regret,
                                                    const double *__restrict__ g_strat, const double *__restrict__ g_sigcdf) {
     ApplyRow a;
     const double2 r0 = *reinterpret_cast<const double2 *>(g_regret + r * 4), r1 = *reinterpret_cast<const double2 *>(g_regret + r * 4 + 2);
     const double2 s0 = *reinterpret_cast<const double2 *>(g_strat + r * 4), s1 = *reinterpret_cast<const double2 *>(g_strat + r * 4 + 2);
-    const double2 g0 = *reinterpret_cast<const double2 *>(g_sigcdf + r * kRow), g1 = *reinterpret_cast<const double2 *>(g_sigcdf + r * kRow + 2);
+    const double2 g0 = *reinterpret_cast<const double2 *>(g_sigcdf + w * kRow), g1 = *reinterpret_cast<const double2 *>(g_sigcdf + w * kRow + 2);
     a.n = (int)((g_key[r] >> 1) & 7);
     a.R[0] = r0.x; a.R[1] = r0.y; a.R[2] = r1.x; a.R[3] = r1.y;
     a.S[0] = s0.x; a.S[1] = s0.y; a.S[2] = s1.x; a.S[3] = s1.y;
@@ -711,7 +721,7 @@
     return a;
 }
 
-__device__ __forceinline__ void apply_row_store(int r, ApplyRow &a, const double (&d)[5], double *__restrict__ g_regret,
+__device__ __forceinline__ void apply_row_store(int r, int w, ApplyRow &a, const double (&d)[5], double *__restrict__ g_regret,
                                                 double *__restrict__ g_strat, double *__restrict__ g_sigcdf) {
 #pragma unroll
     for (int c = 0; c < 4; c++)
@@ -724,13 +734,20 @@
     uint32_t thr[4];
     mc_sigma(a.R, a.n, sg);
     choice_cdf(sg, a.n, thr);
-    row_store(g_sigcdf + r * kRow, sg, thr);
-}
-
-__device__ __forceinline__ double groups_cell_take(double *__restrict__ g_groups, int r, int k) {
-    double v[kDeltaGroups];
+    row_store(g_sigcdf + w * kRow, sg, thr);
+}
+
+__device__ __forceinline__ void apply_single_row(int r, double R0, double S0, double sg0, double d0, double count, double *__restrict__ g_regret,
+                                                 double *__restrict__ g_strat) {
+    g_regret[r * 4] = R0 + d0;
+    g_strat[r * 4] = S0 + count * sg0;
+}
+
+__device__ __forceinline__ void groups_cell_fetch(const double *__restrict__ g_groups, int r, int k, double (&v)[kDeltaGroups]) {
 #pragma unroll
     for (int g = 0; g < kDeltaGroups; g++) v[g] = g_groups[(size_t)g * kDeltaTable + group_cell(k, r)];
+}
+__device__ __forceinline__ double groups_cell_sum(double *__restrict__ g_groups, int r, int k, const double (&v)[kDeltaGroups]) {
     double d = 0.0;
 #pragma unroll
     for (int g = 0; g < kDeltaGroups; g++) {
@@ -739,52 +756,72 @@
     }
     return d;
 }
+__device__ __forceinline__ double groups_cell_take(double *__restrict__ g_groups, int r, int k) {
+    double v[kDeltaGroups];
+    groups_cell_fetch(g_groups, r, k, v);
+    return groups_cell_sum(g_groups, r, k, v);
+}
 
 constexpr int kApplyLanes = 8, kApplyThreads = 64;
 
 __global__ void __launch_bounds__(kApplyThreads)
 k_mccfr_apply_groups(const uint64_t *__restrict__ g_key, double *__restrict__ g_regret, double *__restrict__ g_strat,
-                     double *__restrict__ g_groups, int n_infosets, double *__restrict__ g_sigcdf, uint32_t *__restrict__ g_iter) {
+                     double *__restrict__ g_groups, int n_infosets, int n_choice, double *__restrict__ g_sigcdf, uint32_t *__restrict__ g_iter,
+                     const scopa::WalkRank wr) {
+    const int lane = threadIdx.x & 63, k = lane & (kApplyLanes - 1);
+    const int r = (int)(blockIdx.x * kApplyThreads + threadIdx.x) / kApplyLanes;
+    const bool valid = r < n_infosets;
+    static_assert(64 % (kApplyThreads / kApplyLanes) == 0, "a workgroup's rows share a word of WalkRank");
+    const int w = walk_id(wr, __builtin_amdgcn_readfirstlane(r >> 6), r, n_choice);
+    const bool choice = w < n_choice;
+    const bool fetches = valid && (choice ? k < 5 : k == 4);
+    double v[kDeltaGroups];
+    groups_cell_fetch(g_groups, valid ? w : 0, k < 5 ? k : 4, v);
+    ApplyRow a{};
+    if (valid && k == 0) a = apply_row_load(r, w, g_key, g_regret, g_strat, g_sigcdf);
+    const double mine = fetches ? groups_cell_sum(g_groups, w, k, v) : 0.0;
+    double d[5];
+#pragma unroll
+    for (int j = 0; j < 5; j++) d[j] = __shfl(mine, (lane & ~(kApplyLanes - 1)) + j);
+    if (valid && k == 0) {
+        if (choice) apply_row_store(r, w, a, d, g_regret, g_strat, g_sigcdf);
+        else apply_single_row(r, a.R[0], a.S[0], a.sg[0], d[0], d[4], g_regret, g_strat);
+    }
     if (g_iter && blockIdx.x == 0 && threadIdx.x == 0) *g_iter += 1u;
-    const int lane = threadIdx.x & 63, k = lane & (kApplyLanes - 1);
-    const int r = (int)(blockIdx.x * blockDim.x + threadIdx.x) / kApplyLanes;
-    const bool valid = r < n_infosets;
-    ApplyRow a{};
-    if (valid && k == 0) a = apply_row_load(r, g_key, g_regret, g_strat, g_sigcdf);
-    const double mine = (valid && k < 5) ? groups_cell_take(g_groups, r, k) : 0.0;
-    double d[5];
-#pragma unroll
-    for (int j = 0; j < 5; j++) d[j] = __shfl(mine, (lane & ~(kApplyLanes - 1)) + j);
-    if (valid && k == 0) apply_row_store(r, a, d, g_regret, g_strat, g_sigcdf);
 }
 
 __global__ void __launch_bounds__(64)
 k_mccfr_apply(const uint64_t *__restrict__ g_key, double *__restrict__ g_regret, double *__restrict__ g_strat,
-              double *__restrict__ g_delta, int n_infosets, double *__restrict__ g_sigcdf) {
+              double *__restrict__ g_delta, int n_infosets, double *__restrict__ g_sigcdf, const uint16_t *__restrict__ g_ref2walk) {
     const int r = blockIdx.x * blockDim.x + threadIdx.x;
     if (r >= n_infosets) return;
+    const int w = (int)g_ref2walk[r];
     double d[5];
     for (int k = 0; k < 5; k++) d[k] = g_delta[r * 5 + k];
-    ApplyRow a = apply_row_load(r, g_key, g_regret, g_strat, g_sigcdf);
+    ApplyRow a = apply_row_load(r, w, g_key, g_regret, g_strat, g_sigcdf);
     for (int k = 0; k < 5; k++) g_delta[r * 5 + k] = 0.0;
-    apply_row_store(r, a, d, g_regret, g_strat, g_sigcdf);
+    apply_row_store(r, w, a, d, g_regret, g_strat, g_sigcdf);
 }
 
 __global__ void __launch_bounds__(64)
 k_mccfr_exchange_apply(scopa::P2PArgs xa, double *__restrict__ g_groups, const uint64_t *__restrict__ g_key, double *__restrict__ g_regret,
-                       double *__restrict__ g_strat, double *__restrict__ g_sigcdf, int n_infosets) {
+                       double *__restrict__ g_strat, double *__restrict__ g_sigcdf, int n_infosets, int n_choice, const scopa::WalkRank wr) {
     __shared__ double xch[4][scopa::kP2PMaxWorld][5];
     const int rl = threadIdx.x >> 4, q = threadIdx.x & 15;
     const int r = blockIdx.x * 4 + rl;
     const bool valid = r < n_infosets;
-    const double mine = (valid && q < 5) ? groups_cell_take(g_groups, r, q) : 0.0;
+    const int w = walk_id(wr, __builtin_amdgcn_readfirstlane(r >> 6), r, n_choice);
+    const double mine = (valid && q < 5) ? groups_cell_take(g_groups, w, q) : 0.0;
     double d[5];
 #pragma unroll
     for (int j = 0; j < 5; j++) d[j] = __shfl(mine, (int)(threadIdx.x & ~15u) + j);
     ApplyRow a{};
-    if (valid && q == 0) a = apply_row_load(r, g_key, g_regret, g_strat, g_sigcdf);
+    if (valid && q == 0) a = apply_row_load(r, w, g_key, g_regret, g_strat, g_sigcdf);
     scopa::p2p_exchange_wave4(xa, r, valid, q, d, xch[rl]);
-    if (valid && q == 0) apply_row_store(r, a, d, g_regret, g_strat, g_sigcdf);
+    if (valid && q == 0) {
+        if (w < n_choice) apply_row_store(r, w, a, d, g_regret, g_strat, g_sigcdf);
+        else apply_single_row(r, a.R[0], a.S[0], a.sg[0], d[0], d[4], g_regret, g_strat);
+    }
 }
 
 namespace {
@@ -878,8 +915,8 @@
 }
 
 
-static size_t traverse_lds_bytes(int n_infosets, int waves) {
-    size_t b = ((size_t)(n_infosets + 1) * kRow + (size_t)n_infosets * 4) * sizeof(double);
+static size_t traverse_lds_bytes(int n_infosets, int n_choice, int waves) {
+    size_t b = ((size_t)(n_choice + 1) * kRow + (size_t)n_choice * 4) * sizeof(double);
     b += (size_t)waves * 2 * sizeof(WaveScratch);
     b += (((size_t)n_infosets * 4 + 15) & ~(size_t)15);
     b += 1656 * 2 + 576;
@@ -912,9 +949,9 @@
 
 static int32_t prepare_traverse(scopa_ctx *ctx, uint32_t nb, TraverseGeom *g) {
     int waves = 16;
-    while (waves > 1 && traverse_lds_bytes(ctx->n_infosets, waves) + kStaticLds > (size_t)ctx->lds_limit) waves = waves > 2 ? waves - 2 : 1;
+    while (waves > 1 && traverse_lds_bytes(ctx->n_infosets, ctx->n_choice, waves) + kStaticLds > (size_t)ctx->lds_limit) waves = waves > 2 ? waves - 2 : 1;
     g->threads = waves * 64;
-    g->lds = traverse_lds_bytes(ctx->n_infosets, waves);
+    g->lds = traverse_lds_bytes(ctx->n_infosets, ctx->n_choice, waves);
     SC_REQUIRE(ctx, g->lds + kStaticLds <= (size_t)ctx->lds_limit, SCOPA_ELIMIT, "mccfr traverse: infoset tables do not fit in LDS");
     SC_LDS_ATTR(ctx, scopa::kLdsTraverse, k_mccfr_traverse, ctx->lds_limit - kStaticLds);
     const uint32_t n_passes = (nb + waves - 1) / waves;
@@ -925,7 +962,7 @@
     if (int32_t rc = refresh_all_seen(ctx, false)) return rc;
     if (!ctx->sigcdf_valid) {
         hipLaunchKernelGGL(k_mccfr_prepare, dim3((ctx->n_infosets + 255) / 256), dim3(256), 0, ctx->stream, ctx->d_key,
-                           ctx->d_regret, ctx->d_sigcdf, ctx->n_infosets);
+                           ctx->d_regret, ctx->d_sigcdf, ctx->n_infosets, (const uint16_t *)ctx->d_ref2walk);
         SC_HIP(ctx, hipGetLastError());
         ctx->sigcdf_valid = true;
     }
@@ -943,15 +980,15 @@
     unsigned long long *clock = sampled && ctx->d_clock && grid <= 512u ? ctx->d_clock + (size_t)((ctx->prof_launches - 1) % kClockSamples) * kClockStride : nullptr;
     if (sampled) ctx->clock_grid[(ctx->prof_launches - 1) % kClockSamples] = clock ? (uint16_t)grid : (uint16_t)0;
     if (sampled)
-        hipExtLaunchKernelGGL(k_mccfr_traverse, dim3(grid), dim3(threads), lds, ctx->stream, ev0, ev1, 0, ctx->d_infoset, ctx->d_payoff,
-                              ctx->d_sigcdf, ctx->d_groups, ctx->n_infosets, (uint32_t)ctx->seed, (uint32_t)(ctx->seed >> 32),
+        hipExtLaunchKernelGGL(k_mccfr_traverse, dim3(grid), dim3(threads), lds, ctx->stream, ev0, ev1, 0, (const uint16_t *)ctx->d_walk_inf, ctx->d_payoff,
+                              ctx->d_sigcdf, ctx->d_groups, ctx->n_infosets, ctx->n_choice, (uint32_t)ctx->seed, (uint32_t)(ctx->seed >> 32),
                               iteration, b0, nb, ctx->d_counters + 8, ctx->d_visit, clock, (const uint4 *)ctx->d_lane_tab, (const uint32_t *)nullptr,
-                              ctx->mccfr_all_seen ? 0u : 1u);
+                              ctx->mccfr_all_seen ? 0u : 1u, (const uint16_t *)ctx->d_walk2ref);
     else
-        hipLaunchKernelGGL(k_mccfr_traverse, dim3(grid), dim3(threads), lds, ctx->stream, ctx->d_infoset, ctx->d_payoff,
-                           ctx->d_sigcdf, ctx->d_groups, ctx->n_infosets, (uint32_t)ctx->seed, (uint32_t)(ctx->seed >> 32),
+        hipLaunchKernelGGL(k_mccfr_traverse, dim3(grid), dim3(threads), lds, ctx->stream, (const uint16_t *)ctx->d_walk_inf, ctx->d_payoff,
+                           ctx->d_sigcdf, ctx->d_groups, ctx->n_infosets, ctx->n_choice, (uint32_t)ctx->seed, (uint32_t)(ctx->seed >> 32),
                            iteration, b0, nb, ctx->d_counters + 8, ctx->d_visit, clock, (const uint4 *)ctx->d_lane_tab, (const uint32_t *)nullptr,
-                           ctx->mccfr_all_seen ? 0u : 1u);
+                           ctx->mccfr_all_seen ? 0u : 1u, (const uint16_t *)ctx->d_walk2ref);
     SC_HIP(ctx, hipGetLastError());
     return SCOPA_OK;
 }
@@ -971,11 +1008,12 @@
     hipGraph_t graph = nullptr;
     SC_HIP(ctx, hipStreamBeginCapture(ctx->stream, hipStreamCaptureModeThreadLocal));
     for (uint32_t i = 0; i < k; i++) {
-        hipLaunchKernelGGL(k_mccfr_traverse, dim3(g.grid), dim3(g.threads), g.lds, ctx->stream, ctx->d_infoset, ctx->d_payoff,
-                           ctx->d_sigcdf, ctx->d_groups, ctx->n_infosets, (uint32_t)ctx->seed, (uint32_t)(ctx->seed >> 32),
-                           0u, 0u, batch, ctx->d_counters + 8, ctx->d_visit, (unsigned long long *)nullptr, (const uint4 *)ctx->d_lane_tab, (const uint32_t *)d_iter, track);
+        hipLaunchKernelGGL(k_mccfr_traverse, dim3(g.grid), dim3(g.threads), g.lds, ctx->stream, (const uint16_t *)ctx->d_walk_inf, ctx->d_payoff,
+                           ctx->d_sigcdf, ctx->d_groups, ctx->n_infosets, ctx->n_choice, (uint32_t)ctx->seed, (uint32_t)(ctx->seed >> 32),
+                           0u, 0u, batch, ctx->d_counters + 8, ctx->d_visit, (unsigned long long *)nullptr, (const uint4 *)ctx->d_lane_tab, (const uint32_t *)d_iter, track,
+                           (const uint16_t *)ctx->d_walk2ref);
         hipLaunchKernelGGL(k_mccfr_apply_groups, dim3((ctx->n_infosets * kApplyLanes + kApplyThreads - 1) / kApplyThreads), dim3(kApplyThreads), 0, ctx->stream, ctx->d_key,
-                           ctx->d_regret, ctx->d_strat, ctx->d_groups, ctx->n_infosets, ctx->d_sigcdf, d_iter);
+                           ctx->d_regret, ctx->d_strat, ctx->d_groups, ctx->n_infosets, ctx->n_choice, ctx->d_sigcdf, d_iter, ctx->walk_rank);
     }
     const hipError_t e_end = hipStreamEndCapture(ctx->stream, &graph);
     if (e_end != hipSuccess || !graph) return scopa::fail(ctx, SCOPA_EHIP, "mccfr graph: stream capture", e_end);
@@ -1044,7 +1082,8 @@
     scopa::Range r("scopa mccfr traverse (split path)");
     const int32_t rc = launch_traverse(ctx, iteration, b0, nb);
     if (rc != SCOPA_OK) return rc;
-    hipLaunchKernelGGL(k_mccfr_fold, dim3((ctx->n_infosets + 255) / 256), dim3(256), 0, ctx->stream, ctx->d_groups, ctx->d_delta, ctx->n_infosets);
+    hipLaunchKernelGGL(k_mccfr_fold, dim3((ctx->n_infosets + 255) / 256), dim3(256), 0, ctx->stream, ctx->d_groups, ctx->d_delta, ctx->n_infosets,
+                       (const uint16_t *)ctx->d_ref2walk);
     SC_HIP(ctx, hipGetLastError());
     return SCOPA_OK;
 }
@@ -1096,11 +1135,11 @@
     scopa::Range r("scopa mccfr apply (split path)");
     if (!ctx->sigcdf_valid) {
         hipLaunchKernelGGL(k_mccfr_prepare, dim3((ctx->n_infosets + 255) / 256), dim3(256), 0, ctx->stream, ctx->d_key,
-                           ctx->d_regret, ctx->d_sigcdf, ctx->n_infosets);
+                           ctx->d_regret, ctx->d_sigcdf, ctx->n_infosets, (const uint16_t *)ctx->d_ref2walk);
         SC_HIP(ctx, hipGetLastError());
     }
     hipLaunchKernelGGL(k_mccfr_apply, dim3((ctx->n_infosets + 63) / 64), dim3(64), 0, ctx->stream, ctx->d_key,
-                       ctx->d_regret, ctx->d_strat, ctx->d_delta, ctx->n_infosets, ctx->d_sigcdf);
+                       ctx->d_regret, ctx->d_strat, ctx->d_delta, ctx->n_infosets, ctx->d_sigcdf, (const uint16_t *)ctx->d_ref2walk);
     SC_HIP(ctx, hipGetLastError());
     ctx->sigcdf_valid = true;
     ctx->iteration++;
@@ -1140,7 +1179,7 @@
         if (rc != SCOPA_OK) return rc;
         scopa::Range r("scopa mccfr apply");
         hipLaunchKernelGGL(k_mccfr_apply_groups, dim3((ctx->n_infosets * kApplyLanes + kApplyThreads - 1) / kApplyThreads), dim3(kApplyThreads), 0, ctx->stream, ctx->d_key,
-                           ctx->d_regret, ctx->d_strat, ctx->d_groups, ctx->n_infosets, ctx->d_sigcdf, (uint32_t *)nullptr);
+                           ctx->d_regret, ctx->d_strat, ctx->d_groups, ctx->n_infosets, ctx->n_choice, ctx->d_sigcdf, (uint32_t *)nullptr, ctx->walk_rank);
         SC_HIP(ctx, hipGetLastError());
         ctx->sigcdf_valid = true;
         ctx->iteration++;
@@ -1168,7 +1207,7 @@
         if (rc != SCOPA_OK) return rc;
         scopa::Range r("scopa mccfr exchange + apply");
         hipLaunchKernelGGL(k_mccfr_exchange_apply, dim3((ctx->n_infosets + 3) / 4), dim3(64), 0, ctx->stream, xa, ctx->d_groups, ctx->d_key,
-                           ctx->d_regret, ctx->d_strat, ctx->d_sigcdf, ctx->n_infosets);
+                           ctx->d_regret, ctx->d_strat, ctx->d_sigcdf, ctx->n_infosets, ctx->n_choice, ctx->walk_rank);
         SC_HIP(ctx, hipGetLastError());
         ctx->sigcdf_valid = true;
         ctx->iteration++;
diff --git a/scopa_amd/csrc/scopa_tree.hip b/scopa_amd/csrc/scopa_tree.hip
--- a/scopa_amd/csrc/scopa_tree.hip
+++ b/scopa_amd/csrc/scopa_tree.hip
@@ -126,6 +126,41 @@
             if (first == dfs_index(d, j)) key_of_infoset[id] = infoset_key(states[off + j], d & 1);
         }
     }
+}
+
+__global__ void __launch_bounds__(1024) k_walk_order(const uint16_t *__restrict__ infoset_of, const uint64_t *__restrict__ key_of_infoset,
+                                                      int32_t *__restrict__ meta, uint16_t *__restrict__ walk_inf,
+                                                      uint16_t *__restrict__ walk2ref, uint16_t *__restrict__ ref2walk) {
+    __shared__ int s_wsum[16], s_total;
+    __shared__ uint16_t s_r2w[kDecision];
+    const int tid = threadIdx.x, lane = tid & 63, wave = tid >> 6, I = meta[0] < kDecision ? meta[0] : kDecision;
+    int f[2], sum = 0;
+    for (int q = 0; q < 2; q++) { const int r = tid * 2 + q; f[q] = r < I && (int)((key_of_infoset[r] >> 1) & 7) >= 2 ? 1 : 0; sum += f[q]; }
+    int x = sum;
+    for (int o = 1; o < 64; o <<= 1) { const int y = __shfl_up(x, o); if (lane >= o) x += y; }
+    if (lane == 63) s_wsum[wave] = x;
+    __syncthreads();
+    if (tid == 0) {
+        int acc = 0;
+        for (int w = 0; w < 16; w++) { const int t = s_wsum[w]; s_wsum[w] = acc; acc += t; }
+        s_total = acc;
+        meta[3] = acc;
+    }
+    __syncthreads();
+    const int C = s_total;
+    int before = x - sum + s_wsum[wave];
+    for (int q = 0; q < 2; q++) {
+        const int r = tid * 2 + q;
+        if (r < I) {
+            const int w = f[q] ? before : C + (r - before);
+            s_r2w[r] = (uint16_t)w;
+            ref2walk[r] = (uint16_t)w;
+            walk2ref[w] = (uint16_t)r;
+        }
+        before += f[q];
+    }
+    __syncthreads();
+    for (int i = tid; i < kDecision; i += blockDim.x) walk_inf[i] = s_r2w[infoset_of[i]];
 }
 
 __global__ void k_tables_reset(double *regret, double *strat, double *local, const uint64_t *key_of_infoset,
@@ -219,11 +254,29 @@
     hipLaunchKernelGGL(k_tree_build, dim3(1), dim3(1024), 0, ctx->stream, (const uint8_t *)ctx->d_scratch, ctx->d_states,
                        ctx->d_infoset, ctx->d_payoff, ctx->d_key, ctx->d_meta);
     SC_HIP(ctx, hipGetLastError());
-    int32_t n_inf = 0;
-    SC_HIP(ctx, hipMemcpyAsync(&n_inf, ctx->d_meta, sizeof n_inf, hipMemcpyDeviceToHost, ctx->stream));
+    hipLaunchKernelGGL(k_walk_order, dim3(1), dim3(1024), 0, ctx->stream, (const uint16_t *)ctx->d_infoset, (const uint64_t *)ctx->d_key, ctx->d_meta,
+                       ctx->d_walk_inf, ctx->d_walk2ref, ctx->d_ref2walk);
+    SC_HIP(ctx, hipGetLastError());
+    int32_t h_meta[4] = {0, 0, 0, 0};
+    SC_HIP(ctx, hipMemcpyAsync(h_meta, ctx->d_meta, sizeof h_meta, hipMemcpyDeviceToHost, ctx->stream));
+    uint16_t h_w2r[kWalkMapStride];
+    SC_HIP(ctx, hipMemcpyAsync(h_w2r, ctx->d_walk2ref, sizeof h_w2r, hipMemcpyDeviceToHost, ctx->stream));
     SC_HIP(ctx, hipStreamSynchronize(ctx->stream));
+    const int32_t n_inf = h_meta[0];
     SC_REQUIRE(ctx, n_inf > 0 && n_inf <= kDecision, SCOPA_EHIP, "scopa_set_deal: tree build produced a bad infoset count");
+    SC_REQUIRE(ctx, h_meta[3] > 0 && h_meta[3] <= n_inf, SCOPA_EHIP, "scopa_set_deal: walk order produced a bad choice count");
     ctx->n_infosets = n_inf;
+    ctx->n_choice = h_meta[3];
+    {
+        scopa::WalkRank wr{};
+        for (int w = 0; w < ctx->n_choice; w++) {
+            SC_REQUIRE(ctx, h_w2r[w] < n_inf && (w == 0 || h_w2r[w] > h_w2r[w - 1]), SCOPA_EHIP, "scopa_set_deal: walk order is not increasing");
+            wr.choice[h_w2r[w] >> 6] |= 1ull << (h_w2r[w] & 63);
+        }
+        for (int b = 1; b < 26; b++) wr.before[b] = wr.before[b - 1] + (uint32_t)__builtin_popcountll(wr.choice[b - 1]);
+        ctx->walk_rank = wr;
+    }
+    ctx->sigcdf_valid = false;
     ctx->has_deal = true;
     ctx->d_delta = ctx->d_delta_own;
     ctx->sched_valid = false;
```

Measured after the change: 133.7 billion. 0.977x the previous value.
